# sisl/NeRFSafetyValidation

Measured on AMD Instinct MI355X. Metric: rendered_samples_per_sec, higher is better.
Workload: dtype f16; 1 GPU; Stonehenge 800x800 synthetic, hashgrid L=16 F=2 T=2^19 + ffmlp(64,2)/(64,3), fp16, occupancy-grid ray marching (run_cuda eval path, BASELINE configs[1]); rays_per_frame=640000, bound=2, cascade=2, frames_in_flight=3, fused_reference_rounding=True, parallelism=single GPU, rccl_ranks=1

## Files before the change

### include/ngp_hip.h

```cpp
#ifndef NGP_HIP_H
#define NGP_HIP_H

#include <stddef.h>
#include <stdint.h>

#ifdef __cplusplus
extern "C" {
#endif

#define NGP_OK 0
#define NGP_EINVAL (-1)
#define NGP_ELAUNCH (-2)
#define NGP_EWORKSPACE (-3)
#define NGP_ENODEVICE (-4)

#define NGP_F32 0
#define NGP_F16 1

typedef void* ngp_stream_t;

#if defined(NGP_BUILD)
#define NGP_API __attribute__((visibility("default")))
#else
#define NGP_API
#endif

NGP_API const char* ngp_last_error(void);
NGP_API int ngp_version(void);
NGP_API int ngp_device_count(void);


NGP_API int ngp_near_far_from_aabb(const float* rays_o, const float* rays_d, const float* aabb, uint32_t N, float min_near,
                           float* nears, float* fars, ngp_stream_t stream);
NGP_API int ngp_finish_rays(float* image, float* depth, const float* weights_sum, const float* nears, const float* fars,
                    const float* bg_color3_host, uint32_t N, ngp_stream_t stream);
NGP_API int ngp_sph_from_ray(const float* rays_o, const float* rays_d, float radius, uint32_t N, float* coords,
                     ngp_stream_t stream);
NGP_API int ngp_morton3D(const int32_t* coords, uint32_t N, int32_t* indices, ngp_stream_t stream);
NGP_API int ngp_morton3D_invert(const int32_t* indices, uint32_t N, int32_t* coords, ngp_stream_t stream);
NGP_API int ngp_packbits(const float* grid, uint32_t N, float density_thresh, uint8_t* bitfield, ngp_stream_t stream);

NGP_API size_t ngp_march_rays_train_workspace(uint32_t N);
NGP_API int ngp_march_rays_train(const float* rays_o, const float* rays_d, const uint8_t* grid, float bound, float dt_gamma,
                         uint32_t max_steps, uint32_t N, uint32_t C, uint32_t H, uint32_t M, const float* nears,
                         const float* fars, float* xyzs, float* dirs, float* deltas, int32_t* rays, int32_t* counter,
                         uint32_t perturb, void* workspace, size_t workspace_bytes, ngp_stream_t stream);
NGP_API int ngp_composite_rays_train_forward(const float* sigmas, const float* rgbs, const float* deltas, const int32_t* rays,
                                     uint32_t M, uint32_t N, float* weights_sum, float* depth, float* image,
                                     ngp_stream_t stream);
NGP_API int ngp_composite_rays_train_backward(const float* grad_weights_sum, const float* grad_image, const float* sigmas,
                                      const float* rgbs, const float* deltas, const int32_t* rays,
                                      const float* weights_sum, const float* image, uint32_t M, uint32_t N,
                                      float* grad_sigmas, float* grad_rgbs, ngp_stream_t stream);
NGP_API int ngp_march_rays(uint32_t n_alive, uint32_t n_step, const int32_t* rays_alive, const float* rays_t,
                   const float* rays_o, const float* rays_d, float bound, float dt_gamma, uint32_t max_steps,
                   uint32_t C, uint32_t H, const uint8_t* grid, const float* nears, const float* fars, float* xyzs,
                   float* dirs, float* deltas, uint32_t perturb, uint32_t M_padded, ngp_stream_t stream);
NGP_API size_t ngp_occupancy_lin_bytes(uint32_t C, uint32_t H);
NGP_API int ngp_build_occupancy_lin(const uint8_t* grid, uint32_t C, uint32_t H, void* out, size_t out_bytes, ngp_stream_t stream);
NGP_API int ngp_march_rays_lin(uint32_t n_alive, uint32_t n_step, const int32_t* rays_alive, const float* rays_t,
                   const float* rays_o, const float* rays_d, float bound, float dt_gamma, uint32_t max_steps,
                   uint32_t C, uint32_t H, const uint8_t* grid, const float* nears, const float* fars, float* xyzs,
                   float* dirs, float* deltas, uint32_t perturb, uint32_t M_padded, const void* occupancy_lin,
                   ngp_stream_t stream);
NGP_API int ngp_composite_rays(uint32_t n_alive, uint32_t n_step, int32_t* rays_alive, float* rays_t, const float* sigmas,
                       const float* rgbs, const float* deltas, float* weights_sum, float* depth, float* image,
                       ngp_stream_t stream);


NGP_API int ngp_grid_encode_forward(const float* inputs, const void* embeddings, const int32_t* offsets_host, void* outputs,
                            uint32_t B, uint32_t D, uint32_t C, uint32_t L, float S, uint32_t H,
                            int calc_grad_inputs, void* dy_dx, uint32_t gridtype, int align_corners, int dtype,
                            const void* cell_tables, uint32_t cell_levels, ngp_stream_t stream);
NGP_API int ngp_grid_encode_backward(const void* grad, const float* inputs, const void* embeddings,
                             const int32_t* offsets_host, void* grad_embeddings, uint32_t B, uint32_t D, uint32_t C,
                             uint32_t L, float S, uint32_t H, int calc_grad_inputs, const void* dy_dx,
                             void* grad_inputs, uint32_t gridtype, int align_corners, int dtype, void* workspace,
                             size_t workspace_bytes, ngp_stream_t stream);
NGP_API int ngp_grid_encode_forward_strided(const float* inputs, const void* embeddings, const int32_t* offsets_host, void* outputs,
                                    uint32_t B, uint32_t D, uint32_t C, uint32_t L, float S, uint32_t H,
                                    int calc_grad_inputs, void* dy_dx, uint32_t gridtype, int align_corners, int dtype,
                                    const void* cell_tables, uint32_t cell_levels, uint32_t level_stride, uint32_t point_stride,
                                    ngp_stream_t stream);
NGP_API int ngp_grid_encode_backward_strided(const void* grad, const float* inputs, const void* embeddings,
                                     const int32_t* offsets_host, void* grad_embeddings, uint32_t B, uint32_t D, uint32_t C,
                                     uint32_t L, float S, uint32_t H, int calc_grad_inputs, const void* dy_dx,
                                     void* grad_inputs, uint32_t gridtype, int align_corners, int dtype, void* workspace,
                                     size_t workspace_bytes, uint32_t level_stride, uint32_t point_stride, ngp_stream_t stream);
NGP_API size_t ngp_grid_encode_backward_workspace(uint32_t B, uint32_t D, uint32_t C, uint32_t L, int dtype);


NGP_API int ngp_sh_encode_forward(const float* inputs, float* outputs, uint32_t B, uint32_t D, uint32_t C,
                          int calc_grad_inputs, float* dy_dx, ngp_stream_t stream);
NGP_API int ngp_sh_encode_backward(const float* grad, const float* inputs, uint32_t B, uint32_t D, uint32_t C,
                           const float* dy_dx, float* grad_inputs, ngp_stream_t stream);


NGP_API int ngp_freq_encode_forward(const float* inputs, float* outputs, uint32_t B, uint32_t D, uint32_t deg, ngp_stream_t stream);
NGP_API int ngp_freq_encode_backward(const float* grad, const float* inputs, uint32_t B, uint32_t D, uint32_t deg, float* grad_inputs,
                             ngp_stream_t stream);

NGP_API int ngp_ff_sigma_color_input(const uint16_t* h, const float* dirs, uint32_t B, uint32_t B_pad, float* sigma, uint16_t* color_input,
                             ngp_stream_t stream);
NGP_API int ngp_ff_sigma_color_input_backward(const uint16_t* h, const float* grad_sigma, const uint16_t* grad_color_input, uint32_t B,
                                      uint32_t B_pad, uint16_t* grad_h, ngp_stream_t stream);
NGP_API int ngp_ff_rgb(const uint16_t* outputs16, uint32_t B, uint16_t* rgb, ngp_stream_t stream);
NGP_API int ngp_ff_rgb_backward(const uint16_t* grad_rgb, const uint16_t* rgb, uint32_t B, uint32_t B_pad, uint16_t* grad_outputs16,
                        ngp_stream_t stream);


NGP_API int ngp_ffmlp_forward(const uint16_t* inputs, const uint16_t* weights, uint32_t B, uint32_t input_dim,
                      uint32_t output_dim, uint32_t hidden_dim, uint32_t num_layers, uint32_t activation,
                      uint32_t output_activation, uint16_t* forward_buffer, uint16_t* outputs, ngp_stream_t stream);
NGP_API int ngp_ffmlp_forward_planes(const uint16_t* inputs, const uint16_t* weights, uint32_t B, uint32_t input_dim,
                             uint32_t output_dim, uint32_t hidden_dim, uint32_t num_layers, uint32_t activation,
                             uint32_t output_activation, uint16_t* forward_buffer, uint16_t* outputs, ngp_stream_t stream);
NGP_API int ngp_ffmlp_backward_planes(const uint16_t* grad, const uint16_t* inputs, const uint16_t* weights, const uint16_t* forward_buffer,
                              uint32_t B, uint32_t input_dim, uint32_t output_dim, uint32_t hidden_dim, uint32_t num_layers,
                              uint32_t activation, uint32_t output_activation, int calc_grad_inputs, uint16_t* backward_buffer,
                              uint16_t* grad_inputs, uint16_t* grad_weights, void* workspace, size_t workspace_bytes,
                              ngp_stream_t stream);
NGP_API int ngp_ffmlp_backward_recomputes(uint32_t input_dim, uint32_t hidden_dim, uint32_t num_layers);
NGP_API int ngp_ffmlp_inference(const uint16_t* inputs, const uint16_t* weights, uint32_t B, uint32_t input_dim,
                        uint32_t output_dim, uint32_t hidden_dim, uint32_t num_layers, uint32_t activation,
                        uint32_t output_activation, uint16_t* inference_buffer, uint16_t* outputs,
                        ngp_stream_t stream);
NGP_API int ngp_ffmlp_backward(const uint16_t* grad, const uint16_t* inputs, const uint16_t* weights,
                       const uint16_t* forward_buffer, uint32_t B, uint32_t input_dim, uint32_t output_dim,
                       uint32_t hidden_dim, uint32_t num_layers, uint32_t activation, uint32_t output_activation,
                       int calc_grad_inputs, uint16_t* backward_buffer, uint16_t* grad_inputs,
                       uint16_t* grad_weights, void* workspace, size_t workspace_bytes, ngp_stream_t stream);
NGP_API size_t ngp_ffmlp_backward_workspace(uint32_t B, uint32_t input_dim, uint32_t hidden_dim, uint32_t num_layers);
NGP_API size_t ngp_ffmlp_backward_buffer_bytes(uint32_t B, uint32_t input_dim, uint32_t hidden_dim, uint32_t num_layers);
NGP_API int ngp_ffmlp_allocate_splitk(size_t n);
NGP_API int ngp_ffmlp_free_splitk(void);


NGP_API int ngp_get_rays(const float* poses, uint32_t Bc, float fx, float fy, float cx, float cy, uint32_t H, uint32_t W,
                 const int32_t* pixel_inds, uint32_t n_pix, float* rays_o, float* rays_d, ngp_stream_t stream);
NGP_API int ngp_get_rays_backward(const float* grad_rays_o, const float* grad_rays_d, uint32_t Bc, float fx, float fy, float cx, float cy,
                          uint32_t H, uint32_t W, const int32_t* pixel_inds, uint32_t n_pix, float* grad_poses,
                          ngp_stream_t stream);


typedef struct ngp_model {
    const uint16_t* embeddings;
    const int32_t* offsets_host;
    uint32_t L;
    float S;
    uint32_t H_base;
    uint32_t gridtype;
    int align_corners;
    const uint16_t* sigma_weights;
    uint32_t sigma_hidden_mm;
    const uint16_t* color_weights;
    uint32_t color_hidden_mm;
    float bound;
    float density_scale;
    const uint8_t* density_bitfield;
    uint32_t cascade;
    uint32_t grid_size;
    const void* cell_tables;
    uint32_t cell_levels;
    const void* packed_weights;
    uint32_t precision;
} ngp_model;
#define NGP_PREC_F16 0u
#define NGP_PREC_F32 1u
#define NGP_PREC_F16_REF 2u

NGP_API size_t ngp_packed_weights_bytes(void);
NGP_API int ngp_pack_weights(const ngp_model* model, void* out, ngp_stream_t stream);

NGP_API size_t ngp_cell_tables_bytes(const ngp_model* model, uint32_t n_levels);
NGP_API int ngp_build_cell_tables(const ngp_model* model, uint32_t n_levels, void* out, ngp_stream_t stream);

typedef struct ngp_render_stats {
    uint64_t samples_marched;
    uint64_t samples_slots;
    uint32_t iterations;
    uint32_t rays;
    uint32_t last_n_alive;
    uint32_t last_n_step;
    uint32_t launches;
    uint32_t replayed;
} ngp_render_stats;

typedef struct ngp_render_ctx ngp_render_ctx;

NGP_API int ngp_render_ctx_create(uint32_t max_rays, ngp_render_ctx** out);
NGP_API int ngp_render_ctx_destroy(ngp_render_ctx* ctx);

NGP_API int ngp_render_ctx_set_frame_width(ngp_render_ctx* ctx, uint32_t width);

NGP_API int ngp_render_rays(ngp_render_ctx* ctx, const ngp_model* model, const float* rays_o, const float* rays_d,
                    const float* nears, const float* fars, uint32_t N, float dt_gamma, uint32_t max_steps,
                    uint32_t perturb, float* weights_sum, float* depth, float* image, float* last_sigmas,
                    float* last_rgbs, const float* pad_value_host, ngp_render_stats* stats_host, int sync,
                    ngp_stream_t stream);

NGP_API int ngp_network_forward(const ngp_model* model, const float* xyzs, const float* dirs, uint32_t M, float* sigmas,
                        float* rgbs, ngp_stream_t stream);

NGP_API int ngp_network_density(const ngp_model* model, const float* xyzs, uint32_t M, float* sigmas, float* geo_feat, ngp_stream_t stream);
NGP_API int ngp_network_density_backward(const ngp_model* model, const void* packed_weights_bwd, const float* xyzs, uint32_t M,
                                 const float* grad_sigmas, const float* grad_geo_feat, float* grad_xyzs, ngp_stream_t stream);

NGP_API int ngp_planner_collision(const ngp_model* model, const float* rot_matrix, const float* pos, const float* body, const float* rot,
                                  uint32_t S, uint32_t B, float* out, ngp_stream_t stream);
NGP_API int ngp_planner_collision_backward(const ngp_model* model, const void* packed_weights_bwd, const float* rot_matrix, const float* pos,
                                           const float* body, const float* rot, uint32_t S, uint32_t B, const float* grad_out,
                                           float* grad_pos, float* grad_rot_matrix, ngp_stream_t stream);

NGP_API int ngp_cell_max_density(const ngp_model* model, const float* start_host, float granularity, uint32_t X, uint32_t Y, uint32_t Z,
                                 uint32_t s, const float* rot_host, float* out_max_sigma, ngp_stream_t stream);

#define NGP_EDT_INF 0x7fffffff
NGP_API size_t ngp_edt_sq_workspace(uint32_t X, uint32_t Y, uint32_t Z);
NGP_API int ngp_edt_sq(const uint8_t* occupied, uint32_t X, uint32_t Y, uint32_t Z, int32_t* d2, void* workspace, size_t workspace_bytes,
                       ngp_stream_t stream);

NGP_API size_t ngp_isosurface_workspace(uint32_t X, uint32_t Y, uint32_t Z);
NGP_API int ngp_isosurface_count(const float* u, uint32_t X, uint32_t Y, uint32_t Z, float threshold, void* workspace, size_t workspace_bytes,
                                 uint64_t* totals, ngp_stream_t stream);
NGP_API int ngp_isosurface_emit(const float* u, uint32_t X, uint32_t Y, uint32_t Z, float threshold, const void* workspace,
                                size_t workspace_bytes, uint64_t V, uint64_t F, float* vertices, int32_t* faces, ngp_stream_t stream);

typedef struct ngp_raycast_grid {
    float lo[3], cell[3], inv_cell[3], grow[3];
    float reach;
    uint32_t n[3];
} ngp_raycast_grid;
NGP_API int ngp_raycast_bin_count(const float* tri_data, uint32_t F, const ngp_raycast_grid* grid, int32_t* counts, ngp_stream_t stream);
NGP_API int ngp_raycast_bin_emit(const float* tri_data, uint32_t F, const ngp_raycast_grid* grid, const int64_t* offsets, uint64_t P,
                                 int32_t* pair_cell, int32_t* pair_tri, ngp_stream_t stream);
NGP_API int ngp_raycast(const float* rays_o, const float* rays_d, uint64_t N, const ngp_raycast_grid* grid, const int32_t* cell_start,
                        const int32_t* pair_tri, uint64_t P, const float* tri_data, uint32_t F, float t_min, float t_max,
                        uint32_t frame_width, float* t, int32_t* prim, float* u, float* v, ngp_stream_t stream);
NGP_API int ngp_raycast_shade(const float* rays_d, const int32_t* prim, const float* u, const float* v, uint64_t N, const float* tri_data,
                              const int32_t* faces, uint32_t F, const float* colors, uint32_t V, float ambient,
                              const float* bg_color3_host, float* image, uint8_t* image_u8, ngp_stream_t stream);

typedef struct ngp_voxel_box {
    double start[3];
    double granularity;
    uint32_t shape[3];
    int32_t axis[3], sign[3];
} ngp_voxel_box;
NGP_API int ngp_voxelize_count(const float* vertices, uint32_t V, const int32_t* faces, uint32_t F, const ngp_voxel_box* box, uint8_t* map,
                               int32_t* counts, ngp_stream_t stream);
NGP_API int ngp_voxelize_mark(const float* vertices, uint32_t V, const int32_t* faces, uint32_t F, const ngp_voxel_box* box,
                              const int64_t* ends, uint64_t pair_base, uint64_t n_pairs, uint8_t* map, ngp_stream_t stream);

NGP_API int ngp_overlay_cast(const float* rays_o, const float* rays_d, uint64_t N, const float* prims_host, const float* prims, uint32_t P,
                             float t_min, const float* t_max, uint32_t frame_width, float* t, int32_t* prim, float* normal,
                             ngp_stream_t stream);
NGP_API int ngp_overlay_shade(const float* rays_d, const int32_t* prim, const float* normal, uint64_t N, const float* colors, uint32_t P,
                              float ambient, float* image, uint8_t* image_u8, ngp_stream_t stream);

#define NGP_DISTANCE_STATS_MAX_THRESHOLDS 8
NGP_API int ngp_closest_point(const float* points, uint64_t N, const ngp_raycast_grid* grid, const int32_t* cell_start,
                              const int32_t* pair_tri, uint64_t P, const float* tri_verts, uint32_t F, float max_distance, float* distance,
                              int32_t* prim, float* point, uint32_t* tested, ngp_stream_t stream);
NGP_API size_t ngp_distance_stats_state_bytes(void);
NGP_API size_t ngp_distance_stats_workspace(uint64_t n);
NGP_API int ngp_distance_stats(const float* distance, uint64_t n, uint64_t seen, const float* thresholds_host, uint32_t K, void* state,
                               double* stats, void* workspace, size_t workspace_bytes, ngp_stream_t stream);

NGP_API int ngp_render_uniform(const ngp_model* model, const float* rays_o, const float* rays_d, const float* nears,
                       const float* fars, uint32_t N, uint32_t T, const float* lin, float* weights_sum, float* depth,
                       float* image, float* aggregated_density, uint32_t dump_begin, float* sigmas, float* rgbs,
                       uint32_t frame_width, ngp_stream_t stream);

NGP_API int ngp_render_upsample(const ngp_model* model, const float* rays_o, const float* rays_d, const float* nears,
                        const float* fars, uint32_t N, uint32_t T, uint32_t U, const float* lin, const float* u,
                        float* weights_sum, float* depth, float* image, float* aggregated_density, uint32_t dump_begin,
                        float* sigmas, float* rgbs, uint32_t frame_width, void* workspace, size_t workspace_bytes,
                        ngp_stream_t stream);
NGP_API size_t ngp_render_upsample_workspace(uint32_t N, uint32_t T, uint32_t U);

NGP_API size_t ngp_packed_weights_bwd_bytes(void);
NGP_API int ngp_pack_weights_bwd(const ngp_model* model, void* out, ngp_stream_t stream);
NGP_API size_t ngp_render_uniform_backward_lds(const ngp_model* model, uint32_t T);
NGP_API int ngp_render_uniform_backward(const ngp_model* model, const void* packed_weights_bwd, const float* rays_o, const float* rays_d,
                                const float* nears, const float* fars, uint32_t N, uint32_t T, const float* lin, const float* grad_image,
                                const float* grad_depth, const float* grad_weights_sum, const float* grad_aggregated_density,
                                float* grad_rays_o, float* grad_rays_d, ngp_stream_t stream);


NGP_API int ngp_uniform_samples(const float* rays_o, const float* rays_d, const float* nears, const float* fars, uint32_t N, uint32_t T,
                        uint32_t steps_for_dist, const float* lin, const float* noise, const float* z_in, const float* aabb_host,
                        float* z_vals, float* xyzs, ngp_stream_t stream);
NGP_API int ngp_uniform_samples_backward(const float* grad_xyzs, const float* rays_o, const float* rays_d, const float* z_vals, uint32_t N,
                                 uint32_t T, const float* aabb_host, float* grad_rays_o, float* grad_rays_d, ngp_stream_t stream);
NGP_API int ngp_transmittance_weights(const float* z_vals, const float* sigmas, const float* sample_dist, uint32_t N, uint32_t T,
                              float density_scale, float* weights, ngp_stream_t stream);
NGP_API int ngp_transmittance_weights_backward(const float* grad_weights, const float* z_vals, const float* sigmas, const float* sample_dist,
                                       uint32_t N, uint32_t T, float density_scale, float* grad_sigmas, ngp_stream_t stream);
NGP_API int ngp_sample_pdf(const float* bins, const float* weights, uint32_t N, uint32_t n_bins, const float* u, int u_per_ray,
                   uint32_t n_samples, float* samples, ngp_stream_t stream);
NGP_API int ngp_merge_sorted(const float* z_a, const float* z_b, uint32_t N, uint32_t Ta, uint32_t Tb, float* z, int64_t* index,
                     ngp_stream_t stream);


NGP_API int ngp_mark_untrained_grid(const float* poses, uint32_t n_cams, float fx, float fy, float cx, float cy, float bound, uint32_t cascade,
                            uint32_t H, float* density_grid, void* workspace, size_t workspace_bytes, ngp_stream_t stream);
NGP_API int ngp_density_grid_points(const int32_t* coords, uint32_t n, uint32_t H, float cascade_bound, const float* noise, float* xyzs,
                            int32_t* indices, ngp_stream_t stream);
NGP_API size_t ngp_density_grid_workspace(uint32_t cascade, uint32_t H);
NGP_API int ngp_density_grid_update(float* density_grid, uint32_t cascade, uint32_t H, uint32_t cas, const int32_t* indices, const float* sigmas,
                            uint32_t n, float density_scale, float decay, void* workspace, size_t workspace_bytes, ngp_stream_t stream);
NGP_API int ngp_density_grid_finish(const float* density_grid, uint32_t cascade, uint32_t H, float density_thresh, float* mean_thresh,
                            uint8_t* bitfield, void* workspace, size_t workspace_bytes, ngp_stream_t stream);


NGP_API size_t ngp_uq_stats_workspace(void);
NGP_API int ngp_uq_stats(const void* c, int c_dtype, const float* d, uint64_t n, const float* r, uint64_t m, double* stats,
                 void* workspace, size_t workspace_bytes, ngp_stream_t stream);


NGP_API size_t ngp_sigma_fit_workspace(uint32_t n, uint32_t max_workgroups);
NGP_API int ngp_sigma_fit_eval(const float* features, const float* y, uint32_t n, const float* theta, float prior_mean, double prior_var,
                       int mode, uint32_t max_workgroups, void* workspace, size_t workspace_bytes, double* loss, float* grad,
                       ngp_stream_t stream);
NGP_API int ngp_sigma_fit_step(const float* features, const float* y, uint32_t n, float* theta, float prior_mean, double prior_var, int mode,
                       uint32_t max_workgroups, void* workspace, size_t workspace_bytes, float* grad, float* exp_avg, float* exp_avg_sq,
                       float lr, uint32_t step, float* min_loss, int32_t* improved, float* history, uint32_t history_index,
                       ngp_stream_t stream);


NGP_API int ngp_adam_step(float* param, const float* grad, float* exp_avg, float* exp_avg_sq, uint64_t n, float lr, float beta1,
                  float beta2, float eps, uint32_t step, float grad_scale, ngp_stream_t stream);

NGP_API int ngp_adam_advance_step(float* step_dev, const float* found_inf_dev, ngp_stream_t stream);
NGP_API int ngp_adam_step_dev(float* param, const float* grad, float* exp_avg, float* exp_avg_sq, uint64_t n, float lr, float beta1,
                      float beta2, float eps, const float* step_dev, const float* grad_scale_dev, const float* found_inf_dev,
                      ngp_stream_t stream);


NGP_API int ngp_train_targets(const void* store, int store_dtype, uint32_t C, uint64_t frame_base, uint32_t n_pix, const int64_t* inds,
                      uint32_t N, const float* bg, const float* table, int round_half, float* gt_rgb, ngp_stream_t stream);

NGP_API size_t ngp_photo_loss_workspace(uint32_t N);
NGP_API int ngp_photo_loss_forward(const void* pred, int pred_dtype, const float* gt, uint32_t N, float* per_ray, float* mean, float* error_row,
                           uint32_t map_len, const int64_t* inds_coarse, void* workspace, size_t workspace_bytes, ngp_stream_t stream);
NGP_API int ngp_photo_loss_backward(const void* pred, int pred_dtype, const float* gt, uint32_t N, const float* g, void* grad_pred,
// ... 59 lines not shown
```

### nerfsafetyvalidation_amd/_fused.py

```python
import ctypes as C
import os
import threading

import numpy as np
import torch

from . import _lib


CACHE_LOCK = threading.Lock()


class RunUniform(torch.autograd.Function):

    @staticmethod
    def forward(ctx, fm, rays_o, rays_d, nears, fars, num_steps, dump_begin, frame_width=0, bg=None):
        rays_o, rays_d = rays_o.float().contiguous(), rays_d.float().contiguous()
        ws, depth, image, agg, sigmas, rgbs = fm.render_uniform(rays_o, rays_d, nears, fars, num_steps, dump_begin, frame_width)
        ctx.fm, ctx.num_steps = fm, num_steps
        ctx.bg = None
        if bg is not None:
            ctx.bg = torch.tensor(bg, dtype=torch.float32, device=image.device) if isinstance(bg, (tuple, list)) else float(bg)
            image = image + (1 - ws).unsqueeze(-1) * ctx.bg
        ctx.save_for_backward(rays_o, rays_d, nears, fars)
# ... 126 lines not shown
            raise RuntimeError("fused renderer needs 64-wide MLPs and geo_feat_dim == 15")
        watched = [net.encoder.embeddings] + [l.weight for l in net.sigma_net] + [l.weight for l in net.color_net]
        if f32 and (len(net.sigma_net) - 2 > 1 or len(net.color_net) - 2 > 2):
            raise RuntimeError("fp32 fused model: at most 3 sigma and 4 colour layers (the backward kernels keep that many activations)")
        return cls(net, blob(net.sigma_net, 32), len(net.sigma_net) - 2, blob(net.color_net, 32), len(net.color_net) - 2, watched, f32=f32)

    def valid_for(self, net):
        return (_versions(self._watched) == self._snapshot and self.density_scale == float(net.density_scale)
                and self.bound == float(net.bound) and self.emb16.device == net.encoder.embeddings.device
                and (self.f32 or self.ref_rounding == bool(getattr(net, "fused_reference_rounding", False))))

    def _struct(self, bitfield):
        m = _lib.ModelStruct()
        m.embeddings = _lib.ptr(self.emb16)
        m.offsets_host = C.cast(self.offsets_host, C.c_void_p)
        m.L, m.S, m.H_base, m.gridtype, m.align_corners = 16, self.S, self.H_base, self.gridtype, self.align_corners
        m.sigma_weights, m.sigma_hidden_mm = _lib.ptr(self.sigma_blob), self.sigma_mm
        m.color_weights, m.color_hidden_mm = _lib.ptr(self.color_blob), self.color_mm
        m.bound, m.density_scale = self.bound, self.density_scale
        m.density_bitfield = _lib.ptr(bitfield) if bitfield is not None else None
        m.cascade, m.grid_size = self.cascade, self.grid_size
        m.cell_tables = _lib.ptr(self._cells) if self._cells is not None else None
        m.cell_levels = self._cell_levels
        m.packed_weights = _lib.ptr(self._packed) if self._packed is not None else None
        m.precision = _lib.NGP_PREC_F32 if self.f32 else (_lib.NGP_PREC_F16_REF if self.ref_rounding else _lib.NGP_PREC_F16)
        return m

    def _ensure_packed(self):
        if self._packed is not None:
            return
        with self._ctx_lock:
            if self._packed is not None:
                return
            lib = _lib.lib()
            m = self._struct(None)
            packed = torch.empty(lib.ngp_packed_weights_bytes(), dtype=torch.uint8, device=self.device)
            _lib.check(lib.ngp_pack_weights(C.byref(m), _lib.ptr(packed), _lib.stream()), "pack_weights")
            torch.cuda.current_stream(self.device).synchronize()
            self._packed = packed

    def _ensure_cells(self):
        self._ensure_packed()
        if self._tables is not None:
            self._tables.table_for_current_stream()
        if self._cells_ready:
            return
        if self.cell_table_gb > 0 and not self.f32:
            self._cells, self._cell_levels = self._tables.ensure_cells(self.offsets_host, self.S, self.H_base, self.gridtype, self.align_corners,
                                                                       self.cell_table_gb)
        self._cells_ready = True

    def network_forward(self, xyzs, dirs):
        xyzs, dirs = xyzs.float().contiguous(), dirs.float().contiguous()
        self._ensure_cells()
        M = xyzs.shape[0]
        sigmas = torch.empty(M, dtype=torch.float32, device=xyzs.device)
        rgbs = torch.empty(M, 3, dtype=torch.float32, device=xyzs.device)
        m = self._struct(None)
        lib = _lib.lib()
        _lib.check(lib.ngp_network_forward(C.byref(m), _lib.ptr(xyzs), _lib.ptr(dirs), M, _lib.ptr(sigmas), _lib.ptr(rgbs), _lib.stream()),
                   "network_forward")
        return sigmas, rgbs

    def network_density(self, xyzs, want_geo=False):
        xyzs = xyzs.float().contiguous()
        self._ensure_packed()
        M = xyzs.shape[0]
        sigmas = torch.empty(M, dtype=torch.float32, device=xyzs.device)
        geo = torch.empty(M, 15, dtype=torch.float32, device=xyzs.device) if want_geo else None
        m = self._struct(None)
        _lib.check(_lib.lib().ngp_network_density(C.byref(m), _lib.ptr(xyzs), M, _lib.ptr(sigmas), _lib.ptr(geo), _lib.stream()), "network_density")
        return (sigmas, geo) if want_geo else sigmas

    def cell_max_density(self, start, granularity, shape, samples_per_axis, rot):
        self._ensure_packed()
        X, Y, Z = (int(n) for n in shape)
        out = torch.empty(X, Y, Z, dtype=torch.float32, device=self.device)
        st = (C.c_float * 3)(*[float(v) for v in start])
        r = (C.c_float * 9)(*[float(v) for v in torch.as_tensor(rot, dtype=torch.float32).reshape(9).tolist()])
        _lib.check(_lib.lib().ngp_cell_max_density(C.byref(self._struct(None)), st, float(granularity), X, Y, Z, int(samples_per_axis), r,
                                                   _lib.ptr(out), _lib.stream()), "cell_max_density")
        return out

    def _ensure_packed_bwd(self):
        if self._packed_bwd is None:
            lib = _lib.lib()
            with self._ctx_lock:
                if self._packed_bwd is None:
                    buf = torch.empty(lib.ngp_packed_weights_bwd_bytes(), dtype=torch.uint8, device=self.device)
                    _lib.check(lib.ngp_pack_weights_bwd(C.byref(self._struct(None)), _lib.ptr(buf), _lib.stream()), "pack_weights_bwd")
                    torch.cuda.current_stream(self.device).synchronize()
                    self._packed_bwd = buf
        return self._packed_bwd

    def network_density_backward(self, xyzs, g_sigma=None, g_geo=None):
        self._ensure_packed()
        packed_bwd = self._ensure_packed_bwd()
        xyzs = xyzs.float().contiguous()
        M = xyzs.shape[0]
        f32 = lambda t: None if t is None else t.float().contiguous()
        gx = torch.empty(M, 3, dtype=torch.float32, device=xyzs.device)
        m = self._struct(None)
        _lib.check(_lib.lib().ngp_network_density_backward(C.byref(m), _lib.ptr(packed_bwd), _lib.ptr(xyzs), M, _lib.ptr(f32(g_sigma)),
                                                           _lib.ptr(f32(g_geo)), _lib.ptr(gx), _lib.stream()), "network_density_backward")
        return gx

    def planner_collision(self, rot_matrix, pos, body, rot):
        self._ensure_packed()
        S, B = rot_matrix.shape[0], body.shape[0]
        out = torch.empty(S, dtype=torch.float32, device=rot_matrix.device)
        _lib.check(_lib.lib().ngp_planner_collision(C.byref(self._struct(None)), _lib.ptr(rot_matrix), _lib.ptr(pos), _lib.ptr(body),
                                                    _lib.ptr(rot), S, B, _lib.ptr(out), _lib.stream()), "planner_collision")
        return out

    def planner_collision_backward(self, rot_matrix, pos, body, rot, g):
        self._ensure_packed()
        packed_bwd = self._ensure_packed_bwd()
        S, B = rot_matrix.shape[0], body.shape[0]
        g = g.float().contiguous()
        g_pos = torch.empty(S, 3, dtype=torch.float32, device=rot_matrix.device)
        g_rot = torch.empty(S, 3, 3, dtype=torch.float32, device=rot_matrix.device)
        _lib.check(_lib.lib().ngp_planner_collision_backward(C.byref(self._struct(None)), _lib.ptr(packed_bwd), _lib.ptr(rot_matrix), _lib.ptr(pos),
                                                             _lib.ptr(body), _lib.ptr(rot), S, B, _lib.ptr(g), _lib.ptr(g_pos), _lib.ptr(g_rot),
                                                             _lib.stream()), "planner_collision_backward")
        return g_pos, g_rot

    def _pad_value(self):
        if self._pad is None:
            z = torch.zeros(16, 3, device=self.device)
            s, c = self.network_forward(z, z)
            sig = np.float32(float(s[0])) * np.float32(self.density_scale)
            self._pad = (C.c_float * 4)(float(sig), float(c[0, 0]), float(c[0, 1]), float(c[0, 2]))
        return self._pad

    @property
    def last_stats(self):
        return getattr(self._tls, "stats", None)

    def _context(self, N):
        lib = _lib.lib()
        key = threading.get_ident()
        with self._ctx_lock:
            ent = self._ctxs.get(key)
        if ent is None or ent[1] < N:
            if ent is not None:
                lib.ngp_render_ctx_destroy(ent[0])
            h = C.c_void_p()
            _lib.check(lib.ngp_render_ctx_create(N, C.byref(h)), "render_ctx_create")
            ent = [h, N]
            with self._ctx_lock:
                self._ctxs[key] = ent
        return ent[0]

    def render(self, net_bitfield_owner, rays_o, rays_d, nears, fars, dt_gamma, max_steps, perturb, want_last=True, want_stats=True,
               frame_width=0):
        bitfield = net_bitfield_owner.density_bitfield
        self._ensure_cells()
        N = rays_o.shape[0]
        dev = rays_o.device
        weights_sum = torch.empty(N, dtype=torch.float32, device=dev)
        depth = torch.empty(N, dtype=torch.float32, device=dev)
        image = torch.empty(N, 3, dtype=torch.float32, device=dev)
        last_s = torch.empty(N + 128, dtype=torch.float32, device=dev) if want_last else None
        last_c = torch.empty(N + 128, 3, dtype=torch.float32, device=dev) if want_last else None
        stats = _lib.RenderStats()
        m = self._struct(bitfield)
        lib = _lib.lib()
        ctx = self._context(N)
        need_stats = want_stats or want_last
        _lib.check(lib.ngp_render_ctx_set_frame_width(ctx, int(frame_width or 0)), "render_ctx_set_frame_width")
        if self.debug is not None:
            flags, stamps, hashes = self.debug
            _lib.check(lib.ngp_render_ctx_set_debug(ctx, 1, int(flags), _lib.ptr(stamps), _lib.ptr(hashes)), "render_ctx_set_debug")
        _lib.check(lib.ngp_render_rays(ctx, C.byref(m), _lib.ptr(rays_o), _lib.ptr(rays_d), _lib.ptr(nears.contiguous()),
                                       _lib.ptr(fars.contiguous()), N, float(dt_gamma), int(max_steps), int(perturb), _lib.ptr(weights_sum),
                                       _lib.ptr(depth), _lib.ptr(image), _lib.ptr(last_s), _lib.ptr(last_c),
                                       self._pad_value() if want_last else None, C.byref(stats) if need_stats else None, 0, _lib.stream()),
                   "render_rays")
        sigmas = rgbs = None
        if need_stats:
            self._tls.stats = {"samples_marched": int(stats.samples_marched), "samples_slots": int(stats.samples_slots),
                               "iterations": int(stats.iterations), "rays": int(stats.rays), "launches": int(stats.launches),
                               "replayed": int(stats.replayed)}
        if want_last and stats.iterations > 0:
            M = stats.last_n_alive * stats.last_n_step
            M += 128 - (M % 128)
            sigmas, rgbs = last_s[:M], last_c[:M]
        return weights_sum, depth, image, sigmas, rgbs

    def render_uniform(self, rays_o, rays_d, nears, fars, num_steps, dump_begin, frame_width=0):
        self._ensure_cells()
        N, T, dev = rays_o.shape[0], int(num_steps), rays_o.device
        lin = self._linspace(0.0, 1.0, T)
        out = [torch.empty(N, dtype=torch.float32, device=dev), torch.empty(N, dtype=torch.float32, device=dev),
               torch.empty(N, 3, dtype=torch.float32, device=dev), torch.empty(N, dtype=torch.float32, device=dev)]
        n_dump = N - dump_begin
        sigmas = torch.empty(n_dump * T, 1, dtype=torch.float32, device=dev)
        rgbs = torch.empty(n_dump, T, 3, dtype=torch.float32, device=dev)
        m = self._struct(None)
        lib = _lib.lib()
        _lib.check(lib.ngp_render_uniform(C.byref(m), _lib.ptr(rays_o), _lib.ptr(rays_d), _lib.ptr(nears.contiguous()), _lib.ptr(fars.contiguous()),
                                          N, T, _lib.ptr(lin), _lib.ptr(out[0]), _lib.ptr(out[1]), _lib.ptr(out[2]), _lib.ptr(out[3]),
                                          dump_begin, _lib.ptr(sigmas), _lib.ptr(rgbs), int(frame_width or 0), _lib.stream()), "render_uniform")
        return out[0], out[1], out[2], out[3], sigmas, rgbs

    def _linspace(self, lo, hi, n):
        key = (float(lo), float(hi), int(n))
        t = self._lin_cache.get(key)
        if t is None:
            t = torch.linspace(lo, hi, n, device=self.device)
            torch.cuda.current_stream(self.device).synchronize()
            self._lin_cache[key] = t
        return t

    def upsample_fits(self, num_steps, upsample_steps):
        if self.f32:
            return False
        weights = 2 * ((2048 + self.sigma_mm * 4096 + 1024) + (2048 + self.color_mm * 4096 + 1024))
        return num_steps >= 3 and upsample_steps >= 1 and weights + 2048 + 4 * (5 * num_steps + 4 * upsample_steps) <= 159 * 1024

    def render_upsample(self, rays_o, rays_d, nears, fars, num_steps, upsample_steps, dump_begin, frame_width=0):
        self._ensure_cells()
        N, T, U, dev = rays_o.shape[0], int(num_steps), int(upsample_steps), rays_o.device
        lin = self._linspace(0.0, 1.0, T)
        u = self._linspace(0.0 + 0.5 / U, 1.0 - 0.5 / U, U)
        out = [torch.empty(N, dtype=torch.float32, device=dev), torch.empty(N, dtype=torch.float32, device=dev),
               torch.empty(N, 3, dtype=torch.float32, device=dev), torch.empty(N, dtype=torch.float32, device=dev)]
        n_dump = N - dump_begin
        sigmas = torch.empty(n_dump * (T + U), 1, dtype=torch.float32, device=dev)
        rgbs = torch.empty(n_dump, T + U, 3, dtype=torch.float32, device=dev)
        m = self._struct(None)
        lib = _lib.lib()
        wbytes = lib.ngp_render_upsample_workspace(N, T, U)
        work = torch.empty((wbytes + 3) // 4, dtype=torch.float32, device=dev) if wbytes else None
        _lib.check(lib.ngp_render_upsample(C.byref(m), _lib.ptr(rays_o), _lib.ptr(rays_d), _lib.ptr(nears.contiguous()), _lib.ptr(fars.contiguous()),
                                           N, T, U, _lib.ptr(lin), _lib.ptr(u), _lib.ptr(out[0]), _lib.ptr(out[1]), _lib.ptr(out[2]),
                                           _lib.ptr(out[3]), dump_begin, _lib.ptr(sigmas), _lib.ptr(rgbs), int(frame_width or 0), _lib.ptr(work), wbytes,
                                           _lib.stream()), "render_upsample")
        return out[0], out[1], out[2], out[3], sigmas, rgbs

    def render_uniform_backward(self, rays_o, rays_d, nears, fars, num_steps, g_image, g_depth=None, g_ws=None, g_agg=None):
        self._ensure_cells()
        lib = _lib.lib()
        self._ensure_packed_bwd()
        N, T, dev = rays_o.shape[0], int(num_steps), rays_o.device
        lin = self._linspace(0.0, 1.0, T)
        f32 = lambda t: None if t is None else t.float().contiguous()
        go = torch.empty(N, 3, dtype=torch.float32, device=dev)
        gd = torch.empty(N, 3, dtype=torch.float32, device=dev)
        m = self._struct(None)
        _lib.check(lib.ngp_render_uniform_backward(C.byref(m), _lib.ptr(self._packed_bwd), _lib.ptr(rays_o), _lib.ptr(rays_d), _lib.ptr(nears.contiguous()),
                                                   _lib.ptr(fars.contiguous()), N, T, _lib.ptr(lin), _lib.ptr(f32(g_image)), _lib.ptr(f32(g_depth)),
                                                   _lib.ptr(f32(g_ws)), _lib.ptr(f32(g_agg)), _lib.ptr(go), _lib.ptr(gd), _lib.stream()),
                   "render_uniform_backward")
        return go, gd

    def uniform_backward_fits(self, num_steps):
        need = _lib.lib().ngp_render_uniform_backward_lds(C.byref(self._struct(None)), int(num_steps))
        return num_steps <= 1024 and need <= 160 * 1024

    def __del__(self):
        try:
            for ent in self._ctxs.values():
                _lib.lib().ngp_render_ctx_destroy(ent[0])
        except Exception:
            pass
```

### nerfsafetyvalidation_amd/_lib.py

```python
import ctypes as C
import os

import torch

_HERE = os.path.dirname(os.path.abspath(__file__))
SO_PATH = os.environ.get("NGP_HIP_LIB", os.path.join(_HERE, "libngp_hip.so"))

NGP_F32, NGP_F16 = 0, 1
NGP_PREC_F16, NGP_PREC_F32, NGP_PREC_F16_REF = 0, 1, 2
NGP_DBG_NO_BLOCK_JUMP, NGP_DBG_NO_COARSE, NGP_DBG_NO_SLOW_SORT, NGP_DBG_NO_LIN = 1 << 0, 1 << 1, 1 << 2, 1 << 3
NGP_DBG_ONE_ITER_PER_LAUNCH, NGP_DBG_NO_TILES = 1 << 8, 1 << 13
NGP_DBG_NO_PRE_VERDICT, NGP_DBG_WIDE_ITEMS, NGP_DBG_REPLAY_ONE_ITER = 1 << 14, 1 << 15, 1 << 16
NGP_DBG_LANE_MARCH, NGP_DBG_PROBE_PER_SAMPLE = 1 << 17, 1 << 18
NGP_EDT_INF = 0x7FFFFFFF

_vp, _u32, _f32, _int, _sz = C.c_void_p, C.c_uint32, C.c_float, C.c_int, C.c_size_t


class ModelStruct(C.Structure):
    _fields_ = [
        ("embeddings", _vp), ("offsets_host", _vp), ("L", _u32), ("S", _f32), ("H_base", _u32), ("gridtype", _u32),
        ("align_corners", _int), ("sigma_weights", _vp), ("sigma_hidden_mm", _u32), ("color_weights", _vp),
        ("color_hidden_mm", _u32), ("bound", _f32), ("density_scale", _f32), ("density_bitfield", _vp),
        ("cascade", _u32), ("grid_size", _u32), ("cell_tables", _vp), ("cell_levels", _u32), ("packed_weights", _vp),
        ("precision", _u32),
    ]


class RenderStats(C.Structure):
    _fields_ = [("samples_marched", C.c_uint64), ("samples_slots", C.c_uint64), ("iterations", _u32), ("rays", _u32),
                ("last_n_alive", _u32), ("last_n_step", _u32), ("launches", _u32), ("replayed", _u32)]


class RaycastGrid(C.Structure):
    _fields_ = [("lo", _f32 * 3), ("cell", _f32 * 3), ("inv_cell", _f32 * 3), ("grow", _f32 * 3), ("reach", _f32), ("n", _u32 * 3)]


class VoxelBox(C.Structure):
    _fields_ = [("start", C.c_double * 3), ("granularity", C.c_double), ("shape", _u32 * 3), ("axis", C.c_int32 * 3), ("sign", C.c_int32 * 3)]


SIGNATURES = {
    "ngp_last_error": [],
    "ngp_version": [],
    "ngp_device_count": [],
    "ngp_finish_rays": [_vp, _vp, _vp, _vp, _vp, C.POINTER(C.c_float), _u32, _vp],
    "ngp_near_far_from_aabb": [_vp, _vp, _vp, _u32, _f32, _vp, _vp, _vp],
    "ngp_sph_from_ray": [_vp, _vp, _f32, _u32, _vp, _vp],
    "ngp_morton3D": [_vp, _u32, _vp, _vp],
    "ngp_morton3D_invert": [_vp, _u32, _vp, _vp],
    "ngp_packbits": [_vp, _u32, _f32, _vp, _vp],
    "ngp_march_rays_train_workspace": [_u32],
    "ngp_march_rays_train": [_vp, _vp, _vp, _f32, _f32, _u32, _u32, _u32, _u32, _u32, _vp, _vp, _vp, _vp, _vp, _vp, _vp,
                             _u32, _vp, _sz, _vp],
    "ngp_composite_rays_train_forward": [_vp, _vp, _vp, _vp, _u32, _u32, _vp, _vp, _vp, _vp],
    "ngp_composite_rays_train_backward": [_vp, _vp, _vp, _vp, _vp, _vp, _vp, _vp, _u32, _u32, _vp, _vp, _vp],
    "ngp_march_rays": [_u32, _u32, _vp, _vp, _vp, _vp, _f32, _f32, _u32, _u32, _u32, _vp, _vp, _vp, _vp, _vp, _vp, _u32,
                       _u32, _vp],
    "ngp_occupancy_lin_bytes": [_u32, _u32],
    "ngp_build_occupancy_lin": [_vp, _u32, _u32, _vp, _sz, _vp],
    "ngp_march_rays_lin": [_u32, _u32, _vp, _vp, _vp, _vp, _f32, _f32, _u32, _u32, _u32, _vp, _vp, _vp, _vp, _vp, _vp, _u32,
                           _u32, _vp, _vp],
    "ngp_composite_rays": [_u32, _u32, _vp, _vp, _vp, _vp, _vp, _vp, _vp, _vp, _vp],
    "ngp_grid_encode_forward": [_vp, _vp, _vp, _vp, _u32, _u32, _u32, _u32, _f32, _u32, _int, _vp, _u32, _int, _int, _vp, _u32, _vp],
    "ngp_grid_encode_backward": [_vp, _vp, _vp, _vp, _vp, _u32, _u32, _u32, _u32, _f32, _u32, _int, _vp, _vp, _u32, _int,
                                 _int, _vp, _sz, _vp],
    "ngp_grid_encode_forward_strided": [_vp, _vp, _vp, _vp, _u32, _u32, _u32, _u32, _f32, _u32, _int, _vp, _u32, _int, _int, _vp, _u32,
                                        _u32, _u32, _vp],
    "ngp_grid_encode_backward_strided": [_vp, _vp, _vp, _vp, _vp, _u32, _u32, _u32, _u32, _f32, _u32, _int, _vp, _vp, _u32, _int,
                                         _int, _vp, _sz, _u32, _u32, _vp],
    "ngp_grid_encode_backward_workspace": [_u32, _u32, _u32, _u32, _int],
    "ngp_sh_encode_forward": [_vp, _vp, _u32, _u32, _u32, _int, _vp, _vp],
    "ngp_sh_encode_backward": [_vp, _vp, _u32, _u32, _u32, _vp, _vp, _vp],
    "ngp_freq_encode_forward": [_vp, _vp, _u32, _u32, _u32, _vp],
    "ngp_freq_encode_backward": [_vp, _vp, _u32, _u32, _u32, _vp, _vp],
    "ngp_ff_sigma_color_input": [_vp, _vp, _u32, _u32, _vp, _vp, _vp],
    "ngp_ff_sigma_color_input_backward": [_vp, _vp, _vp, _u32, _u32, _vp, _vp],
    "ngp_ff_rgb": [_vp, _u32, _vp, _vp],
    "ngp_ff_rgb_backward": [_vp, _vp, _u32, _u32, _vp, _vp],
    "ngp_ffmlp_forward": [_vp, _vp, _u32, _u32, _u32, _u32, _u32, _u32, _u32, _vp, _vp, _vp],
    "ngp_ffmlp_inference": [_vp, _vp, _u32, _u32, _u32, _u32, _u32, _u32, _u32, _vp, _vp, _vp],
    "ngp_ffmlp_backward": [_vp, _vp, _vp, _vp, _u32, _u32, _u32, _u32, _u32, _u32, _u32, _int, _vp, _vp, _vp, _vp, _sz, _vp],
    "ngp_ffmlp_forward_planes": [_vp, _vp, _u32, _u32, _u32, _u32, _u32, _u32, _u32, _vp, _vp, _vp],
    "ngp_ffmlp_backward_planes": [_vp, _vp, _vp, _vp, _u32, _u32, _u32, _u32, _u32, _u32, _u32, _int, _vp, _vp, _vp, _vp, _sz, _vp],
    "ngp_ffmlp_backward_recomputes": [_u32, _u32, _u32],
    "ngp_ffmlp_backward_workspace": [_u32, _u32, _u32, _u32],
    "ngp_ffmlp_backward_buffer_bytes": [_u32, _u32, _u32, _u32],
    "ngp_ffmlp_allocate_splitk": [_sz],
    "ngp_ffmlp_free_splitk": [],
    "ngp_get_rays": [_vp, _u32, _f32, _f32, _f32, _f32, _u32, _u32, _vp, _u32, _vp, _vp, _vp],
    "ngp_get_rays_backward": [_vp, _vp, _u32, _f32, _f32, _f32, _f32, _u32, _u32, _vp, _u32, _vp, _vp],
    "ngp_uq_stats_workspace": [],
    "ngp_uq_stats": [_vp, _int, _vp, C.c_uint64, _vp, C.c_uint64, _vp, _vp, _sz, _vp],
    "ngp_sigma_fit_workspace": [_u32, _u32],
    "ngp_sigma_fit_eval": [_vp, _vp, _u32, _vp, _f32, C.c_double, _int, _u32, _vp, _sz, _vp, _vp, _vp],
    "ngp_sigma_fit_step": [_vp, _vp, _u32, _vp, _f32, C.c_double, _int, _u32, _vp, _sz, _vp, _vp, _vp, _f32, _u32, _vp, _vp, _vp, _u32, _vp],
    "ngp_adam_step": [_vp, _vp, _vp, _vp, C.c_uint64, _f32, _f32, _f32, _f32, _u32, _f32, _vp],
    "ngp_adam_advance_step": [_vp, _vp, _vp],
    "ngp_adam_step_dev": [_vp, _vp, _vp, _vp, C.c_uint64, _f32, _f32, _f32, _f32, _vp, _vp, _vp, _vp],
    "ngp_train_targets": [_vp, _int, _u32, C.c_uint64, _u32, _vp, _u32, _vp, _vp, _int, _vp, _vp],
    "ngp_photo_loss_workspace": [_u32],
    "ngp_photo_loss_forward": [_vp, _int, _vp, _u32, _vp, _vp, _vp, _u32, _vp, _vp, _sz, _vp],
    "ngp_photo_loss_backward": [_vp, _int, _vp, _u32, _vp, _vp, _vp],
    "ngp_distortion_workspace": [_u32],
    "ngp_distortion_train_forward": [_vp, _vp, _vp, _vp, _u32, _u32, _vp, _vp, _vp, _vp, _sz, _vp],
    "ngp_distortion_train_backward": [_vp, _vp, _vp, _vp, _vp, _vp, _u32, _u32, _vp, _vp],
    "ngp_distortion_forward": [_vp, _vp, _vp, _f32, _vp, _u32, _u32, _vp, _vp, _vp, _vp, _sz, _vp],
    "ngp_distortion_backward": [_vp, _vp, _vp, _vp, _f32, _vp, _vp, _u32, _u32, _vp, _vp],
    "ngp_image_quality_workspace": [_u32, _u32, _u32],
    "ngp_image_quality": [_vp, _vp, _vp, _u32, _u32, _u32, C.c_int64, C.c_int64, C.c_int64, C.c_int64, _f32, _vp, _vp, _vp, _sz, _vp],
    "ngp_cell_tables_bytes": [C.POINTER(ModelStruct), _u32],
    "ngp_build_cell_tables": [C.POINTER(ModelStruct), _u32, _vp, _vp],
    "ngp_packed_weights_bytes": [],
    "ngp_pack_weights": [C.POINTER(ModelStruct), _vp, _vp],
    "ngp_render_ctx_create": [_u32, C.POINTER(_vp)],
    "ngp_render_ctx_destroy": [_vp],
    "ngp_render_ctx_set_frame_width": [_vp, _u32],
    "ngp_render_rays": [_vp, C.POINTER(ModelStruct), _vp, _vp, _vp, _vp, _u32, _f32, _u32, _u32, _vp, _vp, _vp, _vp, _vp,
                        C.POINTER(C.c_float), C.POINTER(RenderStats), _int, _vp],
    "ngp_network_forward": [C.POINTER(ModelStruct), _vp, _vp, _u32, _vp, _vp, _vp],
    "ngp_network_density": [C.POINTER(ModelStruct), _vp, _u32, _vp, _vp, _vp],
    "ngp_network_density_backward": [C.POINTER(ModelStruct), _vp, _vp, _u32, _vp, _vp, _vp, _vp],
    "ngp_planner_collision": [C.POINTER(ModelStruct), _vp, _vp, _vp, _vp, _u32, _u32, _vp, _vp],
    "ngp_planner_collision_backward": [C.POINTER(ModelStruct), _vp, _vp, _vp, _vp, _vp, _u32, _u32, _vp, _vp, _vp, _vp],
    "ngp_cell_max_density": [C.POINTER(ModelStruct), _vp, C.c_float, _u32, _u32, _u32, _u32, _vp, _vp, _vp],
    "ngp_edt_sq_workspace": [_u32, _u32, _u32],
    "ngp_edt_sq": [_vp, _u32, _u32, _u32, _vp, _vp, _sz, _vp],
    "ngp_isosurface_workspace": [_u32, _u32, _u32],
    "ngp_isosurface_count": [_vp, _u32, _u32, _u32, _f32, _vp, _sz, _vp, _vp],
    "ngp_isosurface_emit": [_vp, _u32, _u32, _u32, _f32, _vp, _sz, C.c_uint64, C.c_uint64, _vp, _vp, _vp],
    "ngp_raycast_bin_count": [_vp, _u32, C.POINTER(RaycastGrid), _vp, _vp],
    "ngp_raycast_bin_emit": [_vp, _u32, C.POINTER(RaycastGrid), _vp, C.c_uint64, _vp, _vp, _vp],
    "ngp_raycast": [_vp, _vp, C.c_uint64, C.POINTER(RaycastGrid), _vp, _vp, C.c_uint64, _vp, _u32, _f32, _f32, _u32, _vp, _vp, _vp, _vp, _vp],
    "ngp_raycast_shade": [_vp, _vp, _vp, _vp, C.c_uint64, _vp, _vp, _u32, _vp, _u32, _f32, C.POINTER(C.c_float), _vp, _vp, _vp],
    "ngp_voxelize_count": [_vp, _u32, _vp, _u32, C.POINTER(VoxelBox), _vp, _vp, _vp],
    "ngp_voxelize_mark": [_vp, _u32, _vp, _u32, C.POINTER(VoxelBox), _vp, C.c_uint64, C.c_uint64, _vp, _vp],
    "ngp_overlay_cast": [_vp, _vp, C.c_uint64, _vp, _vp, _u32, _f32, _vp, _u32, _vp, _vp, _vp, _vp],
    "ngp_overlay_shade": [_vp, _vp, _vp, C.c_uint64, _vp, _u32, _f32, _vp, _vp, _vp],
    "ngp_closest_point": [_vp, C.c_uint64, C.POINTER(RaycastGrid), _vp, _vp, C.c_uint64, _vp, _u32, _f32, _vp, _vp, _vp, _vp, _vp],
    "ngp_distance_stats_state_bytes": [],
    "ngp_distance_stats_workspace": [C.c_uint64],
    "ngp_distance_stats": [_vp, C.c_uint64, C.c_uint64, C.POINTER(C.c_float), _u32, _vp, _vp, _vp, _sz, _vp],
    "ngp_sift_workspace": [_u32, _u32],
    "ngp_sift_layer_offset": [_u32, _u32, _int, _int],
    "ngp_sift_octaves": [_u32, _u32],
    "ngp_sift_interest_mask": [_vp, _u32, _u32, _u32, _u32, _vp, _vp, _vp, _vp, _sz, _vp],
    "ngp_render_uniform_backward_lds": [C.POINTER(ModelStruct), _u32],
    "ngp_packed_weights_bwd_bytes": [],
    "ngp_pack_weights_bwd": [C.POINTER(ModelStruct), _vp, _vp],
    "ngp_render_uniform_backward": [C.POINTER(ModelStruct), _vp, _vp, _vp, _vp, _vp, _u32, _u32, _vp, _vp, _vp, _vp, _vp, _vp, _vp, _vp],
    "ngp_uniform_samples": [_vp, _vp, _vp, _vp, _u32, _u32, _u32, _vp, _vp, _vp, C.POINTER(C.c_float), _vp, _vp, _vp],
    "ngp_uniform_samples_backward": [_vp, _vp, _vp, _vp, _u32, _u32, C.POINTER(C.c_float), _vp, _vp, _vp],
    "ngp_transmittance_weights": [_vp, _vp, _vp, _u32, _u32, _f32, _vp, _vp],
    "ngp_transmittance_weights_backward": [_vp, _vp, _vp, _vp, _u32, _u32, _f32, _vp, _vp],
    "ngp_sample_pdf": [_vp, _vp, _u32, _u32, _vp, _int, _u32, _vp, _vp],
    "ngp_merge_sorted": [_vp, _vp, _u32, _u32, _u32, _vp, _vp, _vp],
    "ngp_mark_untrained_grid": [_vp, _u32, _f32, _f32, _f32, _f32, _f32, _u32, _u32, _vp, _vp, _sz, _vp],
    "ngp_density_grid_points": [_vp, _u32, _u32, _f32, _vp, _vp, _vp, _vp],
    "ngp_density_grid_workspace": [_u32, _u32],
    "ngp_density_grid_update": [_vp, _u32, _u32, _u32, _vp, _vp, _u32, _f32, _f32, _vp, _sz, _vp],
    "ngp_density_grid_finish": [_vp, _u32, _u32, _f32, _vp, _vp, _vp, _sz, _vp],
    "ngp_render_uniform": [C.POINTER(ModelStruct), _vp, _vp, _vp, _vp, _u32, _u32, _vp, _vp, _vp, _vp, _vp, _u32, _vp, _vp, _u32, _vp],
    "ngp_render_upsample": [C.POINTER(ModelStruct), _vp, _vp, _vp, _vp, _u32, _u32, _u32, _vp, _vp, _vp, _vp, _vp, _vp, _u32, _vp, _vp, _u32, _vp, _sz, _vp],
    "ngp_render_upsample_workspace": [_u32, _u32, _u32],
    "ngp_debug_set_stamps": [_vp],
    "ngp_debug_set_sample_hash": [_vp],
    "ngp_debug_disable_march_queue": [_int],
    "ngp_render_ctx_set_debug": [_vp, _int, _int, _vp, _vp],
    "ngp_debug_set_grad_dump": [_vp],
    "ngp_debug_fused_features": [C.POINTER(ModelStruct), _vp, _u32, _int, _vp, _vp],
    "ngp_prof_enable": [_int],
    "ngp_prof_reset": [],
    "ngp_prof_read": [C.c_char_p, C.POINTER(C.c_double), C.POINTER(C.c_uint64), C.POINTER(C.c_double)],
}
_RESTYPES = {"ngp_render_uniform_backward_lds": _sz, "ngp_cell_tables_bytes": _sz, "ngp_packed_weights_bytes": _sz, "ngp_packed_weights_bwd_bytes": _sz, "ngp_grid_encode_backward_workspace": _sz,
             "ngp_ffmlp_backward_workspace": _sz, "ngp_ffmlp_backward_buffer_bytes": _sz, "ngp_render_upsample_workspace": _sz, "ngp_density_grid_workspace": _sz, "ngp_last_error": C.c_char_p, "ngp_march_rays_train_workspace": _sz, "ngp_uq_stats_workspace": _sz, "ngp_sigma_fit_workspace": _sz, "ngp_occupancy_lin_bytes": _sz, "ngp_edt_sq_workspace": _sz, "ngp_isosurface_workspace": _sz, "ngp_sift_workspace": _sz, "ngp_sift_layer_offset": _sz, "ngp_photo_loss_workspace": _sz, "ngp_image_quality_workspace": _sz, "ngp_distortion_workspace": _sz, "ngp_distance_stats_state_bytes": _sz, "ngp_distance_stats_workspace": _sz}

_lib = None


def lib():
    global _lib
    if _lib is None:
        if not os.path.exists(SO_PATH):
            raise RuntimeError(
                f"{SO_PATH} not found: build it with `python -c 'import __graft_entry__ as g; g.build()'` "
                "(hipcc --offload-arch=gfx950).  There is no fallback implementation.")
        handle = C.CDLL(SO_PATH)
        for name, argtypes in SIGNATURES.items():
            fn = getattr(handle, name)
            fn.argtypes = argtypes
            fn.restype = _RESTYPES.get(name, C.c_int)
        _lib = handle
    return _lib


def check(rc, what=""):
    if rc != 0:
        msg = lib().ngp_last_error()
        raise RuntimeError(f"libngp_hip {what} failed (code {rc}): {msg.decode() if msg else ''}")


def ptr(t):
    if t is None:
        return None
    if not t.is_cuda:
        raise RuntimeError("libngp_hip operators need tensors on a HIP device; got a CPU tensor (no CPU fallback)")
    if not t.is_contiguous():
        raise RuntimeError("libngp_hip operators need contiguous tensors")
    return t.data_ptr()


_raw_stream = getattr(torch._C, "_cuda_getCurrentRawStream", None)


def stream():
    if _raw_stream is not None:
        return _raw_stream(torch.cuda.current_device())
    return torch.cuda.current_stream().cuda_stream


def dtype_code(t):
    if t.dtype == torch.float32:
        return NGP_F32
    if t.dtype == torch.float16:
        return NGP_F16
    raise RuntimeError(f"unsupported dtype {t.dtype}: the grid encoder supports float32 and float16")


def host_i32(t):
    cached = getattr(t, "_ngp_host_i32", None)
    if cached is not None and cached[0] == t._version and cached[1] == t.data_ptr():
        return cached[2]
    vals = t.detach().to("cpu", torch.int32).tolist()
    arr = (C.c_int32 * len(vals))(*vals)
    try:
        t._ngp_host_i32 = (t._version, t.data_ptr(), arr)
    except AttributeError:
        pass
    return arr
```

### nerfsafetyvalidation_amd/csrc/capi.hip

```cpp
#include <math.h>
#include <stdarg.h>
#include <stdlib.h>
#include <string.h>

#include <mutex>
#include <vector>

#include "ngp_common.hpp"
#include "wave_ops.hpp"

namespace ngp {

static thread_local char g_err[512] = "";

void set_error(const char* fmt, ...) {
    va_list ap;
    va_start(ap, fmt);
    vsnprintf(g_err, sizeof(g_err), fmt, ap);
    va_end(ap);
}

int check_launch(const char* what) {
    const hipError_t e = hipGetLastError();
    if (e != hipSuccess) {
        set_error("%s: %s", what, hipGetErrorString(e));
        return NGP_ELAUNCH;
    }
    return NGP_OK;
}

bool env_set(const char* name) { return getenv(name) != nullptr; }
uint32_t env_u32(const char* name, uint32_t dflt) {
    const char* e = getenv(name);
    return e ? (uint32_t)atoll(e) : dflt;
}

static std::mutex g_attr_mu;
static std::vector<std::pair<int, const void*>> g_attr_done;

void ensure_dynamic_lds(const void* func, int bytes) {
    int dev = 0;
    (void)hipGetDevice(&dev);
    std::lock_guard<std::mutex> lk(g_attr_mu);
    for (const auto& e : g_attr_done)
        if (e.first == dev && e.second == func) return;
    (void)hipFuncSetAttribute(func, hipFuncAttributeMaxDynamicSharedMemorySize, bytes);
    g_attr_done.emplace_back(dev, func);
}

struct ProfEntry {
    std::string name;
    std::vector<std::pair<hipEvent_t, hipEvent_t>> events;
    double total_ms = 0;
    uint64_t launches = 0;
    double units = 0;
};
static bool g_prof_on = false;
static std::mutex g_prof_mu;
static std::vector<ProfEntry> g_prof;

static int prof_slot(const char* name) {
    for (size_t i = 0; i < g_prof.size(); i++)
        if (g_prof[i].name == name) return (int)i;
    g_prof.emplace_back();
    g_prof.back().name = name;
    return (int)g_prof.size() - 1;
}

ProfScope::ProfScope(const char* name, hipStream_t s, double units) : slot(-1), stream(s) {
    if (!g_prof_on) return;
    std::lock_guard<std::mutex> lk(g_prof_mu);
    slot = prof_slot(name);
    hipEvent_t a, b;
    (void)hipEventCreate(&a);
    (void)hipEventCreate(&b);
    (void)hipEventRecord(a, s);
    g_prof[slot].events.emplace_back(a, b);
    g_prof[slot].units += units;
}
ProfScope::~ProfScope() {
    if (slot < 0) return;
    std::lock_guard<std::mutex> lk(g_prof_mu);
    (void)hipEventRecord(g_prof[slot].events.back().second, stream);
}

bool prof_enabled() { return g_prof_on; }
void prof_add_units(const char* name, double units) {
    if (!g_prof_on) return;
    std::lock_guard<std::mutex> lk(g_prof_mu);
    g_prof[prof_slot(name)].units += units;
}

static void prof_collect(ProfEntry& e) {
    for (auto& p : e.events) {
        (void)hipEventSynchronize(p.second);
        float ms = 0;
        if (hipEventElapsedTime(&ms, p.first, p.second) == hipSuccess) {
            e.total_ms += ms;
            e.launches++;
        }
        (void)hipEventDestroy(p.first);
        (void)hipEventDestroy(p.second);
    }
    e.events.clear();
}

constexpr uint32_t kUqBlocks = 512, kUqThreads = 256;

template <typename CT>
__global__ void __launch_bounds__(kUqThreads) k_uq_partial(const CT* __restrict__ c, const float* __restrict__ d, uint64_t n,
                                                           const float* __restrict__ r, uint64_t m, double* __restrict__ partial) {
    __shared__ double red[5][kUqThreads / 64];
    double acc[5] = {0, 0, 0, 0, 0};
    const uint64_t stride = (uint64_t)gridDim.x * kUqThreads, t0 = (uint64_t)blockIdx.x * kUqThreads + threadIdx.x;
    for (uint64_t i = t0; i < n; i += stride) {
        const double dv = (double)d[i];
        double sc = 0, sc2 = 0;
#pragma unroll
        for (int k = 0; k < 3; k++) {
            const double cv = (double)(float)c[i * 3 + k];
            sc += cv;
            sc2 += cv * cv;
        }
        acc[0] += sc2 * dv * dv;
        acc[1] += sc * dv;
        acc[3] += dv;
        acc[4] += dv * dv;
    }
    for (uint64_t i = t0; i < m; i += stride) acc[2] += (double)r[i];
#pragma unroll
    for (int k = 0; k < 5; k++) {
        const double v = wave_sum_lane0(acc[k]);
        if ((threadIdx.x & 63) == 0) red[k][threadIdx.x >> 6] = v;
    }
    __syncthreads();
    if (threadIdx.x < 5) {
        double v = 0;
        for (uint32_t w = 0; w < kUqThreads / 64; w++) v += red[threadIdx.x][w];
        partial[(size_t)blockIdx.x * 5 + threadIdx.x] = v;
    }
}

__global__ void k_uq_final(const double* __restrict__ partial, uint32_t blocks, uint64_t n, uint64_t m, double* __restrict__ stats) {
    const uint32_t k = threadIdx.x;
    if (k >= 5) return;
    double v = 0;
    for (uint32_t b = 0; b < blocks; b++) v += partial[(size_t)b * 5 + k];
    const int slot[5] = {0, 1, 2, 4, 5};
    stats[slot[k]] = v;
    if (k == 0) {
        stats[3] = (double)m;
        stats[6] = (double)n;
        stats[7] = 0;
    }
}

__global__ void __launch_bounds__(256) k_adam_step(float* __restrict__ p, const float* __restrict__ g, float* __restrict__ m,
                                                   float* __restrict__ v, uint64_t n, float beta1, float beta2, float eps, float step_size,
                                                   float rsqrt_bc2_inv, float grad_scale_inv) {
    const uint64_t i0 = ((uint64_t)blockIdx.x * 256 + threadIdx.x) * 4;
    if (i0 >= n) return;
    const bool vec = i0 + 4 <= n && (((uintptr_t)p | (uintptr_t)g | (uintptr_t)m | (uintptr_t)v) & 15) == 0;
    float pv[4], gv[4], mv[4], vv[4];
    const uint32_t cnt = (uint32_t)(n - i0 < 4 ? n - i0 : 4);
    if (vec) {
        *reinterpret_cast<float4*>(pv) = *reinterpret_cast<const float4*>(p + i0);
        *reinterpret_cast<float4*>(gv) = *reinterpret_cast<const float4*>(g + i0);
        *reinterpret_cast<float4*>(mv) = *reinterpret_cast<const float4*>(m + i0);
        *reinterpret_cast<float4*>(vv) = *reinterpret_cast<const float4*>(v + i0);
    } else {
        for (uint32_t k = 0; k < cnt; k++) { pv[k] = p[i0 + k]; gv[k] = g[i0 + k]; mv[k] = m[i0 + k]; vv[k] = v[i0 + k]; }
    }
#pragma unroll
    for (uint32_t k = 0; k < 4; k++) {
        if (k < cnt) {
            const float gr = gv[k] * grad_scale_inv;
            mv[k] = mv[k] + (1.0f - beta1) * (gr - mv[k]);
            vv[k] = beta2 * vv[k] + (1.0f - beta2) * gr * gr;
            const float denom = sqrtf(vv[k]) / rsqrt_bc2_inv + eps;
            pv[k] = pv[k] - step_size * (mv[k] / denom);
        }
    }
    if (vec) {
        *reinterpret_cast<float4*>(p + i0) = *reinterpret_cast<float4*>(pv);
        *reinterpret_cast<float4*>(m + i0) = *reinterpret_cast<float4*>(mv);
        *reinterpret_cast<float4*>(v + i0) = *reinterpret_cast<float4*>(vv);
    } else {
        for (uint32_t k = 0; k < cnt; k++) { p[i0 + k] = pv[k]; m[i0 + k] = mv[k]; v[i0 + k] = vv[k]; }
    }
}

__global__ void k_adam_advance(float* __restrict__ step, const float* __restrict__ found_inf) {
    if (threadIdx.x == 0 && blockIdx.x == 0 && !(found_inf && *found_inf != 0.0f)) *step += 1.0f;
}
__global__ void __launch_bounds__(256) k_adam_step_dev(float* __restrict__ p, const float* __restrict__ g, float* __restrict__ m,
                                                       float* __restrict__ v, uint64_t n, float beta1, float beta2, float eps, float lr,
                                                       const float* __restrict__ step, const float* __restrict__ grad_scale,
                                                       const float* __restrict__ found_inf) {
    if (found_inf && *found_inf != 0.0f) return;
    __shared__ float s_step_size, s_sqrt_bc2, s_inv;
    if (threadIdx.x == 0) {
        const double st = (double)*step;
        const double bc1 = 1.0 - pow((double)beta1, st), bc2 = 1.0 - pow((double)beta2, st);
        s_step_size = (float)((double)lr / bc1);
        s_sqrt_bc2 = (float)sqrt(bc2);
        s_inv = grad_scale ? 1.0f / *grad_scale : 1.0f;
    }
    __syncthreads();
    const float step_size = s_step_size, rsqrt_bc2_inv = s_sqrt_bc2, grad_scale_inv = s_inv;
    const uint64_t i0 = ((uint64_t)blockIdx.x * 256 + threadIdx.x) * 4;
    if (i0 >= n) return;
    const bool vec = i0 + 4 <= n && (((uintptr_t)p | (uintptr_t)g | (uintptr_t)m | (uintptr_t)v) & 15) == 0;
    float pv[4], gv[4], mv[4], vv[4];
    const uint32_t cnt = (uint32_t)(n - i0 < 4 ? n - i0 : 4);
    if (vec) {
        *reinterpret_cast<float4*>(pv) = *reinterpret_cast<const float4*>(p + i0);
        *reinterpret_cast<float4*>(gv) = *reinterpret_cast<const float4*>(g + i0);
        *reinterpret_cast<float4*>(mv) = *reinterpret_cast<const float4*>(m + i0);
        *reinterpret_cast<float4*>(vv) = *reinterpret_cast<const float4*>(v + i0);
    } else {
        for (uint32_t k = 0; k < cnt; k++) { pv[k] = p[i0 + k]; gv[k] = g[i0 + k]; mv[k] = m[i0 + k]; vv[k] = v[i0 + k]; }
    }
#pragma unroll
    for (uint32_t k = 0; k < 4; k++) {
        if (k < cnt) {
            const float gr = gv[k] * grad_scale_inv;
            mv[k] = mv[k] + (1.0f - beta1) * (gr - mv[k]);
            vv[k] = beta2 * vv[k] + (1.0f - beta2) * gr * gr;
            const float denom = sqrtf(vv[k]) / rsqrt_bc2_inv + eps;
            pv[k] = pv[k] - step_size * (mv[k] / denom);
        }
    }
    if (vec) {
        *reinterpret_cast<float4*>(p + i0) = *reinterpret_cast<float4*>(pv);
        *reinterpret_cast<float4*>(m + i0) = *reinterpret_cast<float4*>(mv);
        *reinterpret_cast<float4*>(v + i0) = *reinterpret_cast<float4*>(vv);
    } else {
        for (uint32_t k = 0; k < cnt; k++) { p[i0 + k] = pv[k]; m[i0 + k] = mv[k]; v[i0 + k] = vv[k]; }
    }
}

}

using namespace ngp;

extern "C" {

const char* ngp_last_error(void) { return g_err; }
int ngp_version(void) { return 100; }

int ngp_device_count(void) {
    int n = 0;
    if (hipGetDeviceCount(&n) != hipSuccess) return 0;
    return n;
}

size_t ngp_uq_stats_workspace(void) { return (size_t)kUqBlocks * 5 * sizeof(double); }

int ngp_uq_stats(const void* c, int c_dtype, const float* d, uint64_t n, const float* r, uint64_t m, double* stats, void* workspace,
                 size_t workspace_bytes, ngp_stream_t stream) {
    NGP_REQUIRE(stats && workspace, "uq_stats: null pointer");
    NGP_REQUIRE((c && d) || n == 0, "uq_stats: null sample buffers");
    NGP_REQUIRE(r || m == 0, "uq_stats: null rendered-colour buffer");
    NGP_REQUIRE(workspace_bytes >= ngp_uq_stats_workspace(), "uq_stats: workspace too small (%zu < %zu bytes)", workspace_bytes,
                ngp_uq_stats_workspace());
    NGP_REQUIRE(c_dtype == 0 || c_dtype == 1, "uq_stats: colour dtype must be 0 (f32) or 1 (f16)");
    hipStream_t s = (hipStream_t)stream;
    const uint64_t work = n > m ? n : m;
    uint32_t blocks = (uint32_t)((work + kUqThreads - 1) / kUqThreads);
    blocks = blocks < 1 ? 1 : blocks > kUqBlocks ? kUqBlocks : blocks;
    ProfScope prof("uq_stats", s, (double)work);
    if (c_dtype == 0)
        k_uq_partial<float><<<blocks, kUqThreads, 0, s>>>((const float*)c, d, n, r, m, (double*)workspace);
    else
        k_uq_partial<_Float16><<<blocks, kUqThreads, 0, s>>>((const _Float16*)c, d, n, r, m, (double*)workspace);
    int rc = check_launch("uq_stats");
    if (rc) return rc;
    k_uq_final<<<1, 64, 0, s>>>((const double*)workspace, blocks, n, m, stats);
    return check_launch("uq_stats (final)");
}

int ngp_adam_step(float* param, const float* grad, float* exp_avg, float* exp_avg_sq, uint64_t n, float lr, float beta1, float beta2, float eps,
                  uint32_t step, float grad_scale, ngp_stream_t stream) {
    if (n == 0) return NGP_OK;
    NGP_REQUIRE(param && grad && exp_avg && exp_avg_sq, "adam_step: null pointer");
    NGP_REQUIRE(step >= 1, "adam_step: step counts from 1");
    NGP_REQUIRE(grad_scale != 0.0f, "adam_step: grad_scale must be non-zero");
    const double bc1 = 1.0 - pow((double)beta1, (double)step), bc2 = 1.0 - pow((double)beta2, (double)step);
    const float step_size = (float)((double)lr / bc1);
    const float sqrt_bc2 = (float)sqrt(bc2);
    const uint64_t quads = (n + 3) / 4;
    ProfScope prof("adam_step", (hipStream_t)stream, (double)n);
    k_adam_step<<<(uint32_t)((quads + 255) / 256), 256, 0, (hipStream_t)stream>>>(param, grad, exp_avg, exp_avg_sq, n, beta1, beta2, eps, step_size,
                                                                                   sqrt_bc2, 1.0f / grad_scale);
    return check_launch("adam_step");
}

int ngp_adam_advance_step(float* step_dev, const float* found_inf_dev, ngp_stream_t stream) {
    NGP_REQUIRE(step_dev, "adam_advance_step: null pointer");
    k_adam_advance<<<1, 64, 0, (hipStream_t)stream>>>(step_dev, found_inf_dev);
    return check_launch("adam_advance_step");
}

int ngp_adam_step_dev(float* param, const float* grad, float* exp_avg, float* exp_avg_sq, uint64_t n, float lr, float beta1, float beta2,
                      float eps, const float* step_dev, const float* grad_scale_dev, const float* found_inf_dev, ngp_stream_t stream) {
    if (n == 0) return NGP_OK;
    NGP_REQUIRE(param && grad && exp_avg && exp_avg_sq && step_dev, "adam_step_dev: null pointer");
    const uint64_t quads = (n + 3) / 4;
    ProfScope prof("adam_step", (hipStream_t)stream, (double)n);
    k_adam_step_dev<<<(uint32_t)((quads + 255) / 256), 256, 0, (hipStream_t)stream>>>(param, grad, exp_avg, exp_avg_sq, n, beta1, beta2, eps, lr,
                                                                                       step_dev, grad_scale_dev, found_inf_dev);
    return check_launch("adam_step_dev");
}

int ngp_prof_enable(int on) {
    g_prof_on = on != 0;
    return NGP_OK;
}

int ngp_prof_reset(void) {
    std::lock_guard<std::mutex> lk(g_prof_mu);
    for (auto& e : g_prof) {
        prof_collect(e);
        e.total_ms = 0;
        e.launches = 0;
        e.units = 0;
    }
    return NGP_OK;
}

int ngp_prof_read(const char* name, double* total_ms, uint64_t* launches, double* units) {
    std::lock_guard<std::mutex> lk(g_prof_mu);
    for (auto& e : g_prof) {
        if (e.name == name) {
            prof_collect(e);
            if (total_ms) *total_ms = e.total_ms;
            if (launches) *launches = e.launches;
            if (units) *units = e.units;
            return NGP_OK;
        }
    }
    set_error("prof_read: no kernel named '%s' was recorded", name);
    return NGP_EINVAL;
}

}
```

### nerfsafetyvalidation_amd/csrc/density_grid.hip

```cpp
#include "ngp_common.hpp"
#include "wave_ops.hpp"

namespace ngp {

constexpr int kDgBlock = 256;
constexpr uint32_t kMaxCams = 2048;

__device__ __forceinline__ float cell_unit(uint32_t c, float Hm1) { return (2.0f * (float)c) / Hm1 - 1.0f; }

__global__ void __launch_bounds__(kDgBlock) k_mark_untrained(const float* __restrict__ poses, uint32_t n_cams, float kx, float ky, float bound,
                                                              uint32_t cascade, uint32_t H, float* __restrict__ grid,
                                                              uint32_t* __restrict__ seen_any, uint32_t first_batch, uint32_t last_batch) {
    extern __shared__ float cam[];
    for (uint32_t i = threadIdx.x; i < n_cams * 12; i += kDgBlock) {
        const uint32_t c = i / 12, e = i % 12;
        cam[i] = e < 9 ? poses[(size_t)c * 16 + (e / 3) * 4 + (e % 3)] : poses[(size_t)c * 16 + (e - 9) * 4 + 3];
    }
    __syncthreads();
    const uint32_t H3 = H * H * H;
    const uint32_t g = blockIdx.x * kDgBlock + threadIdx.x;
    if (g >= cascade * H3) return;
    const uint32_t cas = g / H3, cell = g % H3;
    const uint32_t x = cell / (H * H), y = (cell / H) % H, z = cell % H;
    const uint32_t m = morton3D_cell(x, y, z);
// ... 24 lines not shown
    uint32_t c[3];
    if (coords) { c[0] = (uint32_t)coords[(size_t)i * 3]; c[1] = (uint32_t)coords[(size_t)i * 3 + 1]; c[2] = (uint32_t)coords[(size_t)i * 3 + 2]; }
    else { c[0] = i / (H * H); c[1] = (i / H) % H; c[2] = i % H; }
    indices[i] = (int32_t)morton3D(c[0], c[1], c[2]);
    const float Hm1 = (float)(H - 1);
#pragma unroll
    for (int d = 0; d < 3; d++) {
        float v = cell_unit(c[d], Hm1) * span;
        if (noise) v = v + (noise[(size_t)i * 3 + d] * 2.0f - 1.0f) * hgs;
        xyzs[(size_t)i * 3 + d] = v;
    }
}

__global__ void __launch_bounds__(kDgBlock) k_grid_scatter(const int32_t* __restrict__ indices, const float* __restrict__ sigmas, uint32_t n,
                                                            float density_scale, unsigned long long* __restrict__ tmp, uint32_t H3) {
    const uint32_t i = blockIdx.x * kDgBlock + threadIdx.x;
    if (i >= n) return;
    const uint32_t cell = (uint32_t)indices[i];
    if (cell >= H3) return;
    const float v = sigmas[i] * density_scale;
    atomicMax(tmp + cell, ((unsigned long long)(i + 1) << 32) | (unsigned long long)__float_as_uint(v));
}

__global__ void __launch_bounds__(kDgBlock) k_grid_ema(float* __restrict__ grid, const unsigned long long* __restrict__ tmp, uint32_t H3, float decay) {
    const uint32_t i = blockIdx.x * kDgBlock + threadIdx.x;
    if (i >= H3) return;
    const unsigned long long t = tmp[i];
    if (t == 0ull) return;
    const float g = grid[i], v = __uint_as_float((uint32_t)t);
    if (g >= 0.0f && v >= 0.0f) grid[i] = fmaxf(g * decay, v);
}

__global__ void __launch_bounds__(kDgBlock) k_grid_possum(const float* __restrict__ grid, uint32_t n, double* __restrict__ partial) {
    __shared__ double wsum[kDgBlock / 64];
    const uint32_t i = blockIdx.x * kDgBlock + threadIdx.x;
    double pos = 0.0;
    if (i < n) { const float g = grid[i]; pos = g > 0.0f ? (double)g : 0.0; }
    pos = wave_sum_lane0(pos);
    if ((threadIdx.x & 63) == 0) wsum[threadIdx.x >> 6] = pos;
    __syncthreads();
    if (threadIdx.x == 0) partial[blockIdx.x] = wsum[0] + wsum[1] + wsum[2] + wsum[3];
}

__global__ void __launch_bounds__(1024) k_grid_mean_thresh(const double* __restrict__ partial, uint32_t n_partial, double n_cells, float density_thresh,
                                                            float* __restrict__ out) {
    __shared__ double s[1024];
    double a = 0.0;
    for (uint32_t i = threadIdx.x; i < n_partial; i += 1024) a += partial[i];
    s[threadIdx.x] = a;
    __syncthreads();
    for (uint32_t st = 512; st > 0; st >>= 1) {
        if (threadIdx.x < st) s[threadIdx.x] += s[threadIdx.x + st];
        __syncthreads();
    }
    if (threadIdx.x == 0) {
        const float mean = (float)(s[0] / n_cells);
        out[0] = mean;
        out[1] = fminf(mean, density_thresh);
    }
}

__global__ void __launch_bounds__(kDgBlock) k_packbits_dev(const float* __restrict__ grid, uint32_t n_bytes, const float* __restrict__ thresh_p,
                                                            uint8_t* __restrict__ bitfield) {
    const uint32_t w = blockIdx.x * kDgBlock + threadIdx.x;
    const uint32_t n0 = w * 4;
    if (n0 >= n_bytes) return;
    const float thresh = *thresh_p;
    for (uint32_t n = n0; n < n_bytes && n < n0 + 4; n++) {
        const float4 lo = reinterpret_cast<const float4*>(grid)[(size_t)n * 2], hi = reinterpret_cast<const float4*>(grid)[(size_t)n * 2 + 1];
        const uint32_t b = (lo.x > thresh ? 1u : 0u) | (lo.y > thresh ? 2u : 0u) | (lo.z > thresh ? 4u : 0u) | (lo.w > thresh ? 8u : 0u) |
                           (hi.x > thresh ? 16u : 0u) | (hi.y > thresh ? 32u : 0u) | (hi.z > thresh ? 64u : 0u) | (hi.w > thresh ? 128u : 0u);
        bitfield[n] = (uint8_t)b;
    }
}

static bool grid_dims_ok(uint32_t cascade, uint32_t H) {
    return cascade >= 1 && cascade <= 8 && H >= 2 && H <= 1024 && (H * H * H) % 8 == 0;
}

}

using namespace ngp;

extern "C" {

int ngp_mark_untrained_grid(const float* poses, uint32_t n_cams, float fx, float fy, float cx, float cy, float bound, uint32_t cascade, uint32_t H,
                            float* density_grid, void* workspace, size_t workspace_bytes, ngp_stream_t stream) {
    NGP_REQUIRE(density_grid && (poses || n_cams == 0), "mark_untrained_grid: null pointer");
    NGP_REQUIRE(grid_dims_ok(cascade, H), "mark_untrained_grid: unsupported cascade / grid size (%u, %u)", cascade, H);
    hipStream_t s = (hipStream_t)stream;
    const uint32_t H3 = H * H * H, cells = cascade * H3;
    const float kx = (float)((double)cx / (double)fx), ky = (float)((double)cy / (double)fy);
    const uint32_t n_batches = n_cams ? div_up(n_cams, kMaxCams) : 1;
    uint32_t* seen = nullptr;
    if (n_batches > 1) {
        NGP_REQUIRE(workspace && workspace_bytes >= (size_t)cells * 4, "mark_untrained_grid: %u cameras need a workspace of %zu bytes", n_cams,
                    (size_t)cells * 4);
        seen = reinterpret_cast<uint32_t*>(workspace);
    }
    ensure_dynamic_lds((const void*)k_mark_untrained, (int)(kMaxCams * 12 * sizeof(float)));
    for (uint32_t b = 0; b < n_batches; b++) {
        const uint32_t c0 = b * kMaxCams, nc = n_cams - c0 < kMaxCams ? n_cams - c0 : kMaxCams;
        k_mark_untrained<<<div_up(cells, kDgBlock), kDgBlock, (size_t)(nc ? nc : 1) * 12 * sizeof(float), s>>>(
            poses + (size_t)c0 * 16, n_cams ? nc : 0, kx, ky, bound, cascade, H, density_grid, seen, b == 0, b + 1 == n_batches);
    }
    return check_launch("mark_untrained_grid");
}

int ngp_density_grid_points(const int32_t* coords, uint32_t n, uint32_t H, float cascade_bound, const float* noise, float* xyzs, int32_t* indices,
                            ngp_stream_t stream) {
    if (n == 0) return NGP_OK;
    NGP_REQUIRE(xyzs && indices, "density_grid_points: null pointer");
    NGP_REQUIRE(H >= 2 && H <= 1024, "density_grid_points: unsupported grid size %u", H);
    NGP_REQUIRE(coords || n <= H * H * H, "density_grid_points: a full sweep has at most H^3 samples");
    const double hgs = (double)cascade_bound / (double)H;
    k_grid_points<<<div_up(n, kDgBlock), kDgBlock, 0, (hipStream_t)stream>>>(coords, n, H, (float)((double)cascade_bound - hgs), (float)hgs, noise, xyzs,
                                                                             indices);
    return check_launch("density_grid_points");
}

size_t ngp_density_grid_workspace(uint32_t cascade, uint32_t H) {
    const size_t H3 = (size_t)H * H * H;
    return H3 * 8 + (size_t)div_up((uint32_t)(cascade * H3), kDgBlock) * 8 + 64;
}

int ngp_density_grid_update(float* density_grid, uint32_t cascade, uint32_t H, uint32_t cas, const int32_t* indices, const float* sigmas, uint32_t n,
                            float density_scale, float decay, void* workspace, size_t workspace_bytes, ngp_stream_t stream) {
    NGP_REQUIRE(density_grid && workspace && (n == 0 || (indices && sigmas)), "density_grid_update: null pointer");
    NGP_REQUIRE(grid_dims_ok(cascade, H) && cas < cascade, "density_grid_update: unsupported cascade / grid size");
    NGP_REQUIRE(workspace_bytes >= ngp_density_grid_workspace(cascade, H) && ((uintptr_t)workspace & 7) == 0,
                "density_grid_update: workspace too small or misaligned (%zu < %zu bytes)", workspace_bytes, ngp_density_grid_workspace(cascade, H));
    hipStream_t s = (hipStream_t)stream;
    const uint32_t H3 = H * H * H;
    unsigned long long* tmp = reinterpret_cast<unsigned long long*>(workspace);
    if (hipMemsetAsync(tmp, 0, (size_t)H3 * 8, s) != hipSuccess) return check_launch("density_grid_update (memset)");
    if (n) k_grid_scatter<<<div_up(n, kDgBlock), kDgBlock, 0, s>>>(indices, sigmas, n, density_scale, tmp, H3);
    k_grid_ema<<<div_up(H3, kDgBlock), kDgBlock, 0, s>>>(density_grid + (size_t)cas * H3, tmp, H3, decay);
    return check_launch("density_grid_update");
}

int ngp_density_grid_finish(const float* density_grid, uint32_t cascade, uint32_t H, float density_thresh, float* mean_thresh, uint8_t* bitfield,
                            void* workspace, size_t workspace_bytes, ngp_stream_t stream) {
    NGP_REQUIRE(density_grid && mean_thresh && bitfield && workspace, "density_grid_finish: null pointer");
    NGP_REQUIRE(grid_dims_ok(cascade, H), "density_grid_finish: unsupported cascade / grid size");
    NGP_REQUIRE(workspace_bytes >= ngp_density_grid_workspace(cascade, H) && ((uintptr_t)workspace & 7) == 0, "density_grid_finish: workspace too small or misaligned");
    NGP_REQUIRE(((uintptr_t)density_grid & 15) == 0, "density_grid_finish: the density grid must be 16-byte aligned");
    hipStream_t s = (hipStream_t)stream;
    const uint32_t H3 = H * H * H, cells = cascade * H3;
    double* partial = reinterpret_cast<double*>(reinterpret_cast<unsigned long long*>(workspace) + H3);
    const uint32_t per = div_up(H3, kDgBlock);
    for (uint32_t c = 0; c < cascade; c++) k_grid_possum<<<per, kDgBlock, 0, s>>>(density_grid + (size_t)c * H3, H3, partial + (size_t)c * per);
    k_grid_mean_thresh<<<1, 1024, 0, s>>>(partial, cascade * per, (double)cells, density_thresh, mean_thresh);
    k_packbits_dev<<<div_up(div_up(cells / 8, 4), kDgBlock), kDgBlock, 0, s>>>(density_grid, cells / 8, mean_thresh + 1, bitfield);
    return check_launch("density_grid_finish");
}

}
```

### nerfsafetyvalidation_amd/csrc/ngp_common.hpp

```cpp
#pragma once
#include <hip/hip_runtime.h>
#include <stdint.h>
#include <stdio.h>
#include <string>

#include "../../include/ngp_hip.h"

namespace ngp {

void set_error(const char* fmt, ...);
int check_launch(const char* what);

#define NGP_REQUIRE(cond, ...)                 \
    do {                                       \
        if (!(cond)) {                         \
            ngp::set_error(__VA_ARGS__);       \
            return NGP_EINVAL;                 \
        }                                      \
    } while (0)

bool env_set(const char* name);
uint32_t env_u32(const char* name, uint32_t dflt);

struct ProfScope {
    ProfScope(const char* name, hipStream_t s, double units);
    ~ProfScope();
    int slot;
    hipStream_t stream;
};
bool prof_enabled();
void prof_add_units(const char* name, double units);

static inline uint32_t div_up(uint32_t a, uint32_t b) { return (a + b - 1) / b; }

constexpr uint32_t kMeanOneBlockRays = 16384;
constexpr uint32_t kMeanOneBlockThreads = 1024;
constexpr uint32_t kMeanGroupThreads = 256;
static inline size_t mean_workspace(uint32_t N) { return N <= kMeanOneBlockRays ? 0 : (size_t)div_up(N, 64) * sizeof(float); }
int mean_of_rays(const float* values, uint32_t N, float* mean, void* workspace, size_t workspace_bytes, hipStream_t s, const char* what);
int mean_of_groups(const float* groups, uint32_t N, float* mean, hipStream_t s, const char* what);

void ensure_dynamic_lds(const void* func, int bytes);

constexpr int kMaxLevels = 32;
struct GridLevels {
    float scale[kMaxLevels];
    uint32_t resolution[kMaxLevels];
    uint32_t offset[kMaxLevels + 1];
    uint32_t mul1[kMaxLevels], mul2[kMaxLevels];
    uint8_t hashed[kMaxLevels], mode[kMaxLevels];
};
void fill_levels(GridLevels& lv, const int32_t* offsets_host, uint32_t L, float S, uint32_t H, uint32_t D, uint32_t gridtype,
                 bool align_corners);

__device__ __forceinline__ _Float16 mul_round_f16(float w, _Float16 g) {
    float p = w * (float)g;
    asm volatile("" : "+v"(p));
    return (_Float16)p;
}
__device__ __forceinline__ float clampf(float x, float lo, float hi) { return fminf(hi, fmaxf(lo, x)); }
__device__ __forceinline__ float signf(float x) { return copysignf(1.0f, x); }

__device__ __forceinline__ uint32_t expand_bits(uint32_t v) {
    v = (v * 0x00010001u) & 0xFF0000FFu;
    v = (v * 0x00000101u) & 0x0F00F00Fu;
    v = (v * 0x00000011u) & 0xC30C30C3u;
    v = (v * 0x00000005u) & 0x49249249u;
    return v;
}
__device__ __forceinline__ uint32_t morton3D(uint32_t x, uint32_t y, uint32_t z) {
    return expand_bits(x) | (expand_bits(y) << 1) | (expand_bits(z) << 2);
}
__device__ __forceinline__ uint32_t expand_bits10(uint32_t v) {
    v = (v | (v << 16)) & 0xFF0000FFu;
    v = (v | (v << 8)) & 0x0F00F00Fu;
    v = (v | (v << 4)) & 0xC30C30C3u;
    v = (v | (v << 2)) & 0x49249249u;
    return v;
}
__device__ __forceinline__ uint32_t morton3D_cell(uint32_t x, uint32_t y, uint32_t z) {
    return expand_bits10(x) | (expand_bits10(y) << 1) | (expand_bits10(z) << 2);
}

}
```

### nerfsafetyvalidation_amd/csrc/raymarching.hip

```cpp
#include "occupancy.hpp"

namespace ngp {

constexpr int kBlock = 256;
typedef float f4u __attribute__((ext_vector_type(4), aligned(4)));

__global__ void __launch_bounds__(kBlock) k_near_far_from_aabb(const float* __restrict__ rays_o, const float* __restrict__ rays_d,
                                                               const float* __restrict__ aabb, uint32_t N, float min_near,
                                                               float* __restrict__ nears, float* __restrict__ fars) {
    const uint32_t n = blockIdx.x * kBlock + threadIdx.x;
    if (n >= N) return;
    const float ox = rays_o[n * 3], oy = rays_o[n * 3 + 1], oz = rays_o[n * 3 + 2];
    const float rdx = 1 / rays_d[n * 3], rdy = 1 / rays_d[n * 3 + 1], rdz = 1 / rays_d[n * 3 + 2];
    const float a0 = aabb[0], a1 = aabb[1], a2 = aabb[2], a3 = aabb[3], a4 = aabb[4], a5 = aabb[5];
    float near = (a0 - ox) * rdx, far = (a3 - ox) * rdx;
    if (near > far) { float c = near; near = far; far = c; }
    float near_y = (a1 - oy) * rdy, far_y = (a4 - oy) * rdy;
    if (near_y > far_y) { float c = near_y; near_y = far_y; far_y = c; }
    const float FMAX = 3.402823466e+38f;
    if (near > far_y || near_y > far) { nears[n] = fars[n] = FMAX; return; }
    if (near_y > near) near = near_y;
    if (far_y < far) far = far_y;
    float near_z = (a2 - oz) * rdz, far_z = (a5 - oz) * rdz;
    if (near_z > far_z) { float c = near_z; near_z = far_z; far_z = c; }
// ... 502 lines not shown
                                                           float* __restrict__ weights_sum, float* __restrict__ depth,
                                                           float* __restrict__ image) {
    const uint32_t n = blockIdx.x * kBlock + threadIdx.x;
    if (n >= n_alive) return;
    const int32_t index = rays_alive[n];
    const float* sg = sigmas + (size_t)n * n_step;
    const float* rg = rgbs + (size_t)n * n_step * 3;
    const float* dl = deltas + (size_t)n * n_step * 2;
    float t = rays_t[index];
    float weight_sum = weights_sum[index], d = depth[index];
    float r = image[index * 3], g = image[index * 3 + 1], b = image[index * 3 + 2];
    uint32_t step = 0;
    while (step < n_step) {
        if (dl[0] == 0) break;
        const float alpha = 1.0f - expf(-sg[0] * dl[0]);
        const float T = 1 - weight_sum;
        const float weight = alpha * T;
        weight_sum += weight;
        t += dl[1];
        d = fmaf(weight, t, d);
        r = fmaf(weight, rg[0], r); g = fmaf(weight, rg[1], g); b = fmaf(weight, rg[2], b);
        if ((double)T < 1e-4) break;
        sg++; rg += 3; dl += 2; step++;
    }
    if (step < n_step) rays_alive[n] = -1; else rays_t[index] = t;
    weights_sum[index] = weight_sum; depth[index] = d;
    image[index * 3] = r; image[index * 3 + 1] = g; image[index * 3 + 2] = b;
}

__global__ void __launch_bounds__(kBlock) k_get_rays(const float* __restrict__ poses, uint32_t Bc, float fx, float fy, float cx, float cy,
                                                     uint32_t H, uint32_t W, const int32_t* __restrict__ pixel_inds, uint32_t n_pix,
                                                     float* __restrict__ rays_o, float* __restrict__ rays_d) {
    const uint32_t p = blockIdx.x * kBlock + threadIdx.x;
    const uint32_t cam = blockIdx.y;
    if (p >= n_pix || cam >= Bc) return;
    const uint32_t pix = pixel_inds ? (uint32_t)pixel_inds[p] : p;
    const float* P = poses + (size_t)cam * 16;
    const float i = (float)(pix % W) + 0.5f, j = (float)(pix / W) + 0.5f;
    const float xs = (i - cx) / fx, ys = (j - cy) / fy, zs = 1.0f;
    const float nrm = sqrtf(xs * xs + ys * ys + zs * zs);
    const float ux = xs / nrm, uy = ys / nrm, uz = zs / nrm;
    const size_t o = ((size_t)cam * n_pix + p) * 3;
    rays_d[o + 0] = ux * P[0] + uy * P[1] + uz * P[2];
    rays_d[o + 1] = ux * P[4] + uy * P[5] + uz * P[6];
    rays_d[o + 2] = ux * P[8] + uy * P[9] + uz * P[10];
    rays_o[o + 0] = P[3];
    rays_o[o + 1] = P[7];
    rays_o[o + 2] = P[11];
}

__global__ void __launch_bounds__(1024) k_get_rays_backward(const float* __restrict__ grad_rays_o, const float* __restrict__ grad_rays_d,
                                                            float fx, float fy, float cx, float cy, uint32_t W,
                                                            const int32_t* __restrict__ pixel_inds, uint32_t n_pix,
                                                            float* __restrict__ grad_poses) {
    __shared__ float red[12][1024 / 64];
    const uint32_t cam = blockIdx.x;
    float acc[12];
#pragma unroll
    for (int k = 0; k < 12; k++) acc[k] = 0.0f;
    for (uint32_t p = threadIdx.x; p < n_pix; p += 1024) {
        const uint32_t pix = pixel_inds ? (uint32_t)pixel_inds[p] : p;
        const float i = (float)(pix % W) + 0.5f, j = (float)(pix / W) + 0.5f;
        const float xs = (i - cx) / fx, ys = (j - cy) / fy, zs = 1.0f;
        const float nrm = sqrtf(xs * xs + ys * ys + zs * zs);
        const float u[3] = {xs / nrm, ys / nrm, zs / nrm};
        const size_t o = ((size_t)cam * n_pix + p) * 3;
#pragma unroll
        for (int k = 0; k < 3; k++) {
            const float gd = grad_rays_d ? grad_rays_d[o + k] : 0.0f;
#pragma unroll
            for (int m = 0; m < 3; m++) acc[k * 4 + m] += gd * u[m];
            acc[k * 4 + 3] += grad_rays_o ? grad_rays_o[o + k] : 0.0f;
        }
    }
#pragma unroll
    for (int k = 0; k < 12; k++) {
        const float v = wave_sum_lane0(acc[k]);
        if ((threadIdx.x & 63) == 0) red[k][threadIdx.x >> 6] = v;
    }
    __syncthreads();
    if (threadIdx.x < 16) {
        float v = 0.0f;
        if (threadIdx.x < 12)
            for (int w = 0; w < 1024 / 64; w++) v += red[threadIdx.x][w];
        grad_poses[(size_t)cam * 16 + threadIdx.x] = v;
    }
}

}

using namespace ngp;

__global__ void __launch_bounds__(kBlock) k_finish_rays(float* __restrict__ image, float* __restrict__ depth, const float* __restrict__ weights_sum,
                                                        const float* __restrict__ nears, const float* __restrict__ fars, float bg_r, float bg_g,
                                                        float bg_b, uint32_t N) {
    const uint32_t n = blockIdx.x * kBlock + threadIdx.x;
    if (n >= N) return;
    const float t = 1.0f - weights_sum[n];
    image[(size_t)n * 3] = image[(size_t)n * 3] + t * bg_r;
    image[(size_t)n * 3 + 1] = image[(size_t)n * 3 + 1] + t * bg_g;
    image[(size_t)n * 3 + 2] = image[(size_t)n * 3 + 2] + t * bg_b;
    const float d = depth[n] - nears[n];
    depth[n] = (d != d ? d : fmaxf(d, 0.0f)) / (fars[n] - nears[n]);
}

extern "C" {

int ngp_finish_rays(float* image, float* depth, const float* weights_sum, const float* nears, const float* fars, const float* bg_color3,
                    uint32_t N, ngp_stream_t stream) {
    if (N == 0) return NGP_OK;
    NGP_REQUIRE(image && depth && weights_sum && nears && fars && bg_color3, "finish_rays: null pointer");
    k_finish_rays<<<div_up(N, kBlock), kBlock, 0, (hipStream_t)stream>>>(image, depth, weights_sum, nears, fars, bg_color3[0], bg_color3[1],
                                                                          bg_color3[2], N);
    return check_launch("finish_rays");
}

int ngp_near_far_from_aabb(const float* rays_o, const float* rays_d, const float* aabb, uint32_t N, float min_near, float* nears,
                           float* fars, ngp_stream_t stream) {
    if (N == 0) return NGP_OK;
    NGP_REQUIRE(rays_o && rays_d && aabb && nears && fars, "near_far_from_aabb: null pointer");
    hipStream_t s = (hipStream_t)stream;
    ProfScope prof("near_far_from_aabb", s, N);
    k_near_far_from_aabb<<<div_up(N, kBlock), kBlock, 0, s>>>(rays_o, rays_d, aabb, N, min_near, nears, fars);
    return check_launch("near_far_from_aabb");
}

int ngp_sph_from_ray(const float* rays_o, const float* rays_d, float radius, uint32_t N, float* coords, ngp_stream_t stream) {
    if (N == 0) return NGP_OK;
    NGP_REQUIRE(rays_o && rays_d && coords, "sph_from_ray: null pointer");
    k_sph_from_ray<<<div_up(N, kBlock), kBlock, 0, (hipStream_t)stream>>>(rays_o, rays_d, radius, N, coords);
    return check_launch("sph_from_ray");
}

int ngp_morton3D(const int32_t* coords, uint32_t N, int32_t* indices, ngp_stream_t stream) {
    if (N == 0) return NGP_OK;
    NGP_REQUIRE(coords && indices, "morton3D: null pointer");
    k_morton3D<<<div_up(N, kBlock), kBlock, 0, (hipStream_t)stream>>>(coords, N, indices);
    return check_launch("morton3D");
}

int ngp_morton3D_invert(const int32_t* indices, uint32_t N, int32_t* coords, ngp_stream_t stream) {
    if (N == 0) return NGP_OK;
    NGP_REQUIRE(coords && indices, "morton3D_invert: null pointer");
    k_morton3D_invert<<<div_up(N, kBlock), kBlock, 0, (hipStream_t)stream>>>(indices, N, coords);
    return check_launch("morton3D_invert");
}

int ngp_packbits(const float* grid, uint32_t N, float density_thresh, uint8_t* bitfield, ngp_stream_t stream) {
    if (N == 0) return NGP_OK;
    NGP_REQUIRE(grid && bitfield, "packbits: null pointer");
    hipStream_t s = (hipStream_t)stream;
    ProfScope prof("packbits", s, N);
    k_packbits<<<div_up(div_up(N, 4), kBlock), kBlock, 0, s>>>(grid, N, density_thresh, bitfield);
    return check_launch("packbits");
}

static size_t train_counts_bytes(uint32_t N) {
    const size_t nblocks = div_up(N ? N : 1, kBlock);
    return (((size_t)(N + nblocks + 4) * sizeof(uint32_t)) + 15) & ~(size_t)15;
}

constexpr uint32_t kTraceMaxRays = 16384, kTraceMaxSteps = 1024;
static size_t train_trace_bytes(uint32_t N) { return N <= kTraceMaxRays ? (size_t)N * kTraceMaxSteps * sizeof(float2) : 0; }

size_t ngp_march_rays_train_workspace(uint32_t N) {
    return train_counts_bytes(N) + kTrainLinBytes + kCoarseMaxBytes + train_trace_bytes(N);
}

int ngp_march_rays_train(const float* rays_o, const float* rays_d, const uint8_t* grid, float bound, float dt_gamma, uint32_t max_steps,
                         uint32_t N, uint32_t C, uint32_t H, uint32_t M, const float* nears, const float* fars, float* xyzs, float* dirs,
                         float* deltas, int32_t* rays, int32_t* counter, uint32_t perturb, void* workspace, size_t workspace_bytes,
                         ngp_stream_t stream) {
    if (N == 0) return NGP_OK;
    NGP_REQUIRE(rays_o && rays_d && grid && nears && fars && xyzs && dirs && deltas && rays && counter, "march_rays_train: null pointer");
    NGP_REQUIRE(C >= 1 && C <= 8 && H >= 2 && H <= 1024, "march_rays_train: unsupported cascade/grid size C=%u H=%u", C, H);
    if (!workspace || workspace_bytes < ngp_march_rays_train_workspace(N)) {
        set_error("march_rays_train: workspace of %zu bytes needed, %zu given", ngp_march_rays_train_workspace(N), workspace_bytes);
        return NGP_EWORKSPACE;
    }
    hipStream_t s = (hipStream_t)stream;
    const uint32_t nblocks = div_up(N, kBlock);
    uint32_t* counts = (uint32_t*)workspace;
    uint32_t* block_sums = counts + N;
    uint32_t* base = block_sums + nblocks;
    Pcg32 rng;
    rng.seed(42u);
    ProfScope prof("march_rays_train", s, N);
    OccupancyLin tl = {};
    const bool lin = N >= 1024 && occupancy_lin_fits(C, H, grid, kTrainLinBytes, kCoarseMaxBytes);
    char* extra = (char*)workspace + train_counts_bytes(N);
    float2* trace = nullptr;
    if (lin && train_trace_bytes(N) && max_steps <= kTraceMaxSteps) trace = (float2*)(extra + kTrainLinBytes + kCoarseMaxBytes);
    enum { kWave, kTraced, kLin, kPlain } const form = !lin ? kPlain : (!trace ? kLin : (dt_gamma == 0.0f ? kWave : kTraced));
    if (lin) tl = build_occupancy_lin(grid, C, H, extra, extra + kTrainLinBytes, s);
#define NGP_COUNT(LIN_, TRACE_)                                                                                                                   \
    k_march_train_count<LIN_, TRACE_><<<nblocks, kBlock, 0, s>>>(rays_o, rays_d, grid, bound, dt_gamma, max_steps, N, C, H, nears, fars, perturb, rng, \
                                                                 counts, block_sums, tl, trace)
#define NGP_WRITE(LIN_, TRACE_)                                                                                                                      \
    k_march_train_write<LIN_, TRACE_><<<nblocks, kBlock, 0, s>>>(rays_o, rays_d, grid, bound, dt_gamma, max_steps, N, C, H, M, nears, fars, perturb, rng, \
                                                                 counts, block_sums, base, xyzs, dirs, deltas, rays, tl, trace)
    switch (form) {
        case kWave:
            (void)hipMemsetAsync(block_sums, 0, (size_t)nblocks * sizeof(uint32_t), s);
            k_march_train_count_wave<<<div_up(N, kBlock / 64), kBlock, 0, s>>>(rays_o, rays_d, grid, bound, max_steps, N, C, H, nears, fars, perturb,
                                                                              rng, counts, block_sums, tl, trace);
            break;
        case kTraced: NGP_COUNT(true, true); break;
        case kLin: NGP_COUNT(true, false); break;
        case kPlain: NGP_COUNT(false, false); break;
    }
    k_march_train_scan<<<1, 1024, 0, s>>>(block_sums, nblocks, N, counter, base);
    switch (form) {
        case kWave:
            k_march_train_write_wave<<<div_up(N, kBlock / 64), kBlock, 0, s>>>(rays_o, rays_d, bound, max_steps, N, M, nears, perturb, rng, counts,
                                                                              block_sums, base, xyzs, dirs, deltas, rays, trace);
            break;
        case kTraced: NGP_WRITE(true, true); break;
        case kLin: NGP_WRITE(true, false); break;
        case kPlain: NGP_WRITE(false, false); break;
    }
#undef NGP_COUNT
#undef NGP_WRITE
    return check_launch("march_rays_train");
}

int ngp_composite_rays_train_forward(const float* sigmas, const float* rgbs, const float* deltas, const int32_t* rays, uint32_t M,
                                     uint32_t N, float* weights_sum, float* depth, float* image, ngp_stream_t stream) {
    if (N == 0) return NGP_OK;
    NGP_REQUIRE(sigmas && rgbs && deltas && rays && weights_sum && depth && image, "composite_rays_train_forward: null pointer");
    hipStream_t s = (hipStream_t)stream;
    ProfScope prof("composite_rays_train_forward", s, M);
    k_composite_train_fwd<<<div_up(N, kBlock), kBlock, 0, s>>>(sigmas, rgbs, deltas, rays, M, N, weights_sum, depth, image);
    return check_launch("composite_rays_train_forward");
}

int ngp_composite_rays_train_backward(const float* grad_weights_sum, const float* grad_image, const float* sigmas, const float* rgbs,
                                      const float* deltas, const int32_t* rays, const float* weights_sum, const float* image, uint32_t M,
                                      uint32_t N, float* grad_sigmas, float* grad_rgbs, ngp_stream_t stream) {
    if (N == 0) return NGP_OK;
    NGP_REQUIRE(grad_weights_sum && grad_image && sigmas && rgbs && deltas && rays && weights_sum && image && grad_sigmas && grad_rgbs,
                "composite_rays_train_backward: null pointer");
    ProfScope prof("composite_rays_train_backward", (hipStream_t)stream, M);
    k_composite_train_bwd<<<div_up(N, kBlock), kBlock, 0, (hipStream_t)stream>>>(grad_weights_sum, grad_image, sigmas, rgbs, deltas, rays,
                                                                                 weights_sum, image, M, N, grad_sigmas, grad_rgbs);
    return check_launch("composite_rays_train_backward");
}

static size_t lin_coarse_offset(uint32_t C, uint32_t H) { return ((size_t)C * H * H * H / 8 + 255) / 256 * 256; }
size_t ngp_occupancy_lin_bytes(uint32_t C, uint32_t H) {
    if (!occupancy_lin_fits(C, H, nullptr, kTrainLinBytes, kCoarseMaxBytes)) return 0;
    return lin_coarse_offset(C, H) + (size_t)C * H * H * H / 512;
}
int ngp_build_occupancy_lin(const uint8_t* grid, uint32_t C, uint32_t H, void* out, size_t out_bytes, ngp_stream_t stream) {
    NGP_REQUIRE(grid && out, "build_occupancy_lin: null pointer");
    const size_t need = ngp_occupancy_lin_bytes(C, H);
    NGP_REQUIRE(need && out_bytes >= need, "build_occupancy_lin: C=%u H=%u needs %zu bytes (0 = not supported), %zu given", C, H, need, out_bytes);
    NGP_REQUIRE(((uintptr_t)grid & 7) == 0 && ((uintptr_t)out & 255) == 0, "build_occupancy_lin: grid must be 8-byte aligned, out 256-byte aligned");
    build_occupancy_lin(grid, C, H, out, (char*)out + lin_coarse_offset(C, H), (hipStream_t)stream);
    return check_launch("build_occupancy_lin");
}

static int march_rays_impl(uint32_t n_alive, uint32_t n_step, const int32_t* rays_alive, const float* rays_t, const float* rays_o,
                           const float* rays_d, float bound, float dt_gamma, uint32_t max_steps, uint32_t C, uint32_t H, const uint8_t* grid,
                           const float* fars, float* xyzs, float* dirs, float* deltas, uint32_t perturb, uint32_t M_padded,
                           const void* occupancy_lin, ngp_stream_t stream) {
    if (M_padded == 0 || n_step == 0) return NGP_OK;
    NGP_REQUIRE(rays_alive && rays_t && rays_o && rays_d && grid && fars && xyzs && dirs && deltas, "march_rays: null pointer");
    NGP_REQUIRE((uint64_t)n_alive * n_step <= M_padded, "march_rays: M_padded=%u smaller than n_alive*n_step", M_padded);
    NGP_REQUIRE(C >= 1 && C <= 8 && H >= 2 && H <= 1024, "march_rays: unsupported cascade/grid size C=%u H=%u", C, H);
    hipStream_t s = (hipStream_t)stream;
    Pcg32 rng;
    rng.seed((uint64_t)perturb);
    const uint32_t n_rows = div_up(M_padded, n_step);
    ProfScope prof("march_rays", s, (double)n_alive * n_step);
    OccupancyLin tl = {};
    if (occupancy_lin) {
        NGP_REQUIRE(occupancy_lin_fits(C, H, nullptr, kTrainLinBytes, kCoarseMaxBytes), "march_rays_lin: C=%u H=%u has no derived occupancy copies (ngp_occupancy_lin_bytes is 0)", C, H);
        tl = occupancy_lin_view(C, H, occupancy_lin, (const char*)occupancy_lin + lin_coarse_offset(C, H));
        k_march_rays<true><<<div_up(n_rows, kBlock), kBlock, 0, s>>>(n_alive, n_step, rays_alive, rays_t, rays_o, rays_d, bound, dt_gamma, max_steps,
                                                                     C, H, grid, fars, xyzs, dirs, deltas, perturb, rng, n_rows, M_padded, tl);
    } else {
        k_march_rays<false><<<div_up(n_rows, kBlock), kBlock, 0, s>>>(n_alive, n_step, rays_alive, rays_t, rays_o, rays_d, bound, dt_gamma, max_steps,
                                                                      C, H, grid, fars, xyzs, dirs, deltas, perturb, rng, n_rows, M_padded, tl);
    }
    return check_launch("march_rays");
}

int ngp_march_rays_lin(uint32_t n_alive, uint32_t n_step, const int32_t* rays_alive, const float* rays_t, const float* rays_o,
                       const float* rays_d, float bound, float dt_gamma, uint32_t max_steps, uint32_t C, uint32_t H, const uint8_t* grid,
                       const float* nears, const float* fars, float* xyzs, float* dirs, float* deltas, uint32_t perturb, uint32_t M_padded,
                       const void* occupancy_lin, ngp_stream_t stream) {
    (void)nears;
    NGP_REQUIRE(occupancy_lin, "march_rays_lin: occupancy_lin is NULL (ngp_build_occupancy_lin fills it; ngp_march_rays needs none)");
    return march_rays_impl(n_alive, n_step, rays_alive, rays_t, rays_o, rays_d, bound, dt_gamma, max_steps, C, H, grid, fars, xyzs, dirs, deltas,
                           perturb, M_padded, occupancy_lin, stream);
}

int ngp_march_rays(uint32_t n_alive, uint32_t n_step, const int32_t* rays_alive, const float* rays_t, const float* rays_o,
                   const float* rays_d, float bound, float dt_gamma, uint32_t max_steps, uint32_t C, uint32_t H, const uint8_t* grid,
                   const float* nears, const float* fars, float* xyzs, float* dirs, float* deltas, uint32_t perturb, uint32_t M_padded,
                   ngp_stream_t stream) {
    (void)nears;
    return march_rays_impl(n_alive, n_step, rays_alive, rays_t, rays_o, rays_d, bound, dt_gamma, max_steps, C, H, grid, fars, xyzs, dirs, deltas,
                           perturb, M_padded, nullptr, stream);
}

// ... 34 lines not shown
```

### nerfsafetyvalidation_amd/csrc/render_fused.hip

```cpp
#include <hip/hip_fp16.h>
#include <math.h>
#include <string.h>

#include <atomic>

#include "fused_net.hpp"
#include "occupancy.hpp"

namespace ngp {

constexpr int kWaves = 8;
constexpr int kThreads = kWaves * 64;
constexpr int kWavesPerSimd = 4;
constexpr int kCh = 2;
constexpr int kSlots = 64 * kCh;
constexpr size_t kLinMaxBytes = 4u << 20;
constexpr int kLookahead = 4;
constexpr int kRing = 8;

struct Ctl {
    uint32_t n_alive, n_step, step, done;
    uint32_t iters, last_n_alive, last_n_step, pad;
    unsigned long long samples_marched, samples_slots;
    uint32_t spec, rollbacks, backoff, rsv;
};

constexpr uint32_t kSpecK = 8;
constexpr uint32_t kSpecMarginDiv = 16;
constexpr uint32_t kSpecMaxQ = 8;
constexpr uint32_t kSpecMaxSamples = 32;
constexpr uint32_t kSpecMidSamples = 8;
constexpr uint32_t kSpecSafetyX2 = 1;
constexpr int kDeathShards = 64;
constexpr uint32_t kDeathWords = 2u * kDeathShards * kSpecK;
struct QueueHeads { uint32_t head[8][32]; };

constexpr int kStatShards = 64;

struct RenderArgs {
    const float *rays_o, *rays_d, *fars;
    float* rays_t;
    float *weights_sum, *depth, *image;
    float *last_sigmas, *last_rgbs;
    float pad_sigma, pad_r, pad_g, pad_b;
    float4* dump_rec;
    uint32_t* dump_iter;
    const int32_t* alive_in;
    int32_t* staging;
    uint32_t* chunk_count;
    uint32_t sort_slow;
    Ctl* ctl;
    QueueHeads* heads;
    unsigned long long* stat_shards;
    uint32_t* death_shards;
    float4* backup;
    const uint8_t* bitfield;
    uint32_t cascade, grid_size, max_steps, perturb;
    float dt_gamma;
    Pcg32 rng;
    OccupancyLin occ;
    uint32_t block_jump;
    uint32_t* sample_hash;
    unsigned long long* stamps;
    float2* march_samples;
    uint8_t* march_counts;
    uint32_t wave_slots;
    uint32_t n_rays;
    uint32_t pre_verdict;
    uint32_t wave_march_max;
    uint32_t cell_runs;
};

__host__ __device__ __forceinline__ uint32_t item_width(uint32_t n_alive, uint32_t wave_slots) {
    return n_alive >= 64u * wave_slots ? 64u : (n_alive >= 32u * wave_slots ? 32u : 16u);
}
__device__ __forceinline__ void truncate_launch(Ctl& c, const uint32_t* exhausted, uint32_t N) {
    if (!c.spec) return;
    const uint32_t q = c.spec, K = c.n_step / q;
    uint32_t alive = c.n_alive, ok = K;
    for (uint32_t j = 0; j < K; j++) {
        if (alive == 0) break;
        const uint32_t want_q = N / alive;
        if (j > 0 && (want_q < 1 ? 1u : (want_q > 8 ? 8u : want_q)) != q) { ok = j; break; }
        alive -= exhausted[j] < alive ? exhausted[j] : alive;
    }
    if (ok < K) {
        if (ok <= 1) { c.spec = 0; c.n_step = q; }
        else c.n_step = ok * q;
        c.rsv += 1;
    }
}
static uint32_t items_bound(uint32_t ub, uint32_t wave_slots) {
    const uint32_t by64 = div_up(ub ? ub : 1, 64), narrow = div_up(ub ? ub : 1, 16);
    const uint32_t cap = 2u * wave_slots + 1u;
    return by64 > (narrow < cap ? narrow : cap) ? by64 : (narrow < cap ? narrow : cap);
}

struct WaveSlab {
    float t[kSlots], dt[kSlots], sig[kSlots];
    uint32_t rg[kSlots], b[kSlots];
    uint16_t list[kSlots];
    float od[64][6];
};

__device__ __forceinline__ void dump_row(const RenderArgs& ra, uint32_t entry, int32_t ray, uint32_t n_step, uint32_t k, float sg, float r,
                                         float g, float b) {
    if (ra.dump_rec) {
        ra.dump_rec[(size_t)ray * 8 + k] = make_float4(sg, r, g, b);
    } else {
        const size_t row = (size_t)entry * n_step + k;
        ra.last_sigmas[row] = sg;
        ra.last_rgbs[row * 3] = r; ra.last_rgbs[row * 3 + 1] = g; ra.last_rgbs[row * 3 + 2] = b;
    }
}

__device__ __forceinline__ void march_ahead_wave(const RenderArgs& ra, float bound, const Ctl& ctl, const uint32_t* coarse) {
    const uint32_t lane = threadIdx.x & 63u;
    const uint32_t entry = blockIdx.x * 4u + (threadIdx.x >> 6);
    if (entry >= ctl.n_alive) return;
    const uint32_t n_step = ctl.n_step, spec = ctl.spec;
    const int32_t ray = ra.alive_in[entry];
    Dda dda;
    const float t_c = ra.rays_t[ray], far = ra.fars[ray];
    float t_march = dda.start(ra.rays_o + (size_t)ray * 3, ra.rays_d + (size_t)ray * 3, ra.bitfield, bound, 0.0f, ra.max_steps, ra.cascade,
                              ra.grid_size, &ra.occ, ra.block_jump != 0, t_c, ra.perturb, ra.rng, entry);
    float last_m = t_march, geo_tc = t_c;
    uint32_t emitted = 0, rounds = 0;
    float2* out = ra.march_samples + ((size_t)(entry >> 6) * n_step) * 64 + (entry & 63u);
    while (t_march < far && emitted < n_step) {
        rounds++;
        const LatticeWindow w = probe_window(dda, t_march, far, lane, coarse);
        const uint32_t room = spec ? spec - emitted % spec : n_step - emitted;
        unsigned long long emit = 0ull;
        uint32_t cur = 0, cnt = 0;
        float t_next = t_march;
        for (int guard = 0; guard < 64; guard++) {
            const float to = __uint_as_float((uint32_t)__builtin_amdgcn_readlane((int)__float_as_uint(w.nxt), (int)cur));
            if ((w.omask >> cur) & 1ull) {
                emit |= 1ull << cur;
                const float d1 = to - last_m;
                last_m = to;
                geo_tc += d1;
                if (++cnt == room) { t_next = to; break; }
            }
            const uint32_t jn = (uint32_t)__builtin_amdgcn_readlane((int)w.j, (int)cur);
            if (jn >= 64u || !((w.vmask >> jn) & 1ull)) { t_next = to; break; }
            cur = jn;
        }
        if ((emit >> lane) & 1ull) out[(size_t)(emitted + (uint32_t)__popcll(emit & ((1ull << lane) - 1ull))) * 64] = make_float2(w.p, w.dt);
        emitted += cnt;
        t_march = t_next;
        if (spec && cnt == room) {
            t_march = geo_tc;
            last_m = geo_tc;
        }
    }
    if (lane != 0) return;
    if (ra.stamps) {
        atomicAdd(ra.stamps + 4, (unsigned long long)rounds);
        atomicAdd(ra.stamps + 5, (unsigned long long)rounds * 64ull);
        atomicAdd(ra.stamps + 6, 1ull);
        atomicMax(ra.stamps + 7, (unsigned long long)rounds);
    }
    if (spec && ra.pre_verdict && emitted < n_step)
        atomicAdd(ra.death_shards + (size_t)kDeathShards * kSpecK + (blockIdx.x % kDeathShards) * kSpecK + emitted / spec, 1u);
    bool slow = false;
    if (ra.sort_slow && emitted == n_step) slow = geo_tc < far && dda.coarse_empty_at_lin(geo_tc, coarse);
    ra.march_counts[entry] = (uint8_t)(emitted | (slow ? 128u : 0u));
}

template <bool LIN>
__global__ void __launch_bounds__(256) k_march_ahead(RenderArgs ra, float bound) {
    const Ctl ctl = *ra.ctl;
    if (ctl.done) return;
    const uint32_t n_alive = ctl.n_alive, n_step = ctl.n_step, spec = ctl.spec;
    const bool by_wave = LIN && n_alive <= ra.wave_march_max;
    if (blockIdx.x * (by_wave ? 4u : 256u) >= n_alive) return;
    __shared__ uint32_t coarse_lds[kCoarseMaxBytes / 4];
    stage_coarse(ra.occ, coarse_lds, blockDim.x);
    __syncthreads();
    const uint32_t* coarse = ra.occ.coarse_words ? coarse_lds : nullptr;
    if (LIN && by_wave) {
        march_ahead_wave(ra, bound, ctl, coarse);
        return;
    }
    const uint32_t entry = blockIdx.x * blockDim.x + threadIdx.x;
    if (entry >= n_alive) return;
    const int32_t ray = ra.alive_in[entry];
    Dda dda;
    const float t_c = ra.rays_t[ray], far = ra.fars[ray];
    float t_march = dda.start(ra.rays_o + (size_t)ray * 3, ra.rays_d + (size_t)ray * 3, ra.bitfield, bound, ra.dt_gamma, ra.max_steps, ra.cascade,
                              ra.grid_size, LIN ? &ra.occ : nullptr, ra.block_jump != 0, t_c, ra.perturb, ra.rng, entry);
    float last_m = t_march;
    float geo_tc = t_c;
    uint32_t emitted = 0;
    float2* out = ra.march_samples + ((size_t)(entry >> 6) * n_step) * 64 + (entry & 63u);
    float x, y, z, dt;
    uint32_t probes = 0, probes_coarse_empty = 0, probes_fine_empty = 0;
    const bool run_cells = LIN && dda.const_dt && ra.cell_runs != 0;
    float occ_until = 0.0f;
    while (t_march < far && emitted < n_step) {
        probes++;
        const bool diag_ce = LIN && ra.stamps && dda.coarse_empty_at_lin(t_march, coarse);
        const uint32_t emitted_before = emitted;
        if (LIN ? dda.probe_lin(t_march, x, y, z, dt, coarse, run_cells ? &occ_until : nullptr) : dda.probe(t_march, x, y, z, dt, coarse)) {
            do {
                out[(size_t)emitted * 64] = make_float2(t_march, dt);
                t_march += dt;
                const float d1 = t_march - last_m;
                last_m = t_march;
                geo_tc += d1;
                emitted++;
                if (spec && emitted % spec == 0) {
                    t_march = geo_tc;
                    last_m = geo_tc;
                }
            } while (run_cells && t_march < occ_until && t_march < far && emitted < n_step);
        }
        if (ra.stamps && emitted == emitted_before) { if (diag_ce) probes_coarse_empty++; else probes_fine_empty++; }
    }
    if (ra.stamps) {
        uint32_t mx = probes, sm = probes;
#pragma unroll
        for (int off = 32; off > 0; off >>= 1) {
            const uint32_t o = (uint32_t)__shfl_xor((int)mx, off, 64), p2 = (uint32_t)__shfl_xor((int)sm, off, 64);
            mx = mx > o ? mx : o;
            sm += p2;
        }
        if ((threadIdx.x & 63u) == (uint32_t)__builtin_ctzll(__ballot(true))) {
            atomicAdd(ra.stamps + 4, (unsigned long long)mx);
            atomicAdd(ra.stamps + 5, (unsigned long long)sm);
            atomicAdd(ra.stamps + 6, 1ull);
            atomicMax(ra.stamps + 7, (unsigned long long)mx);
        }
        uint32_t ce = probes_coarse_empty, fe = probes_fine_empty;
        ce = wave_sum(ce);
        fe = wave_sum(fe);
        if ((threadIdx.x & 63u) == (uint32_t)__builtin_ctzll(__ballot(true))) {
            atomicAdd(ra.stamps + 14, (unsigned long long)ce);
            atomicAdd(ra.stamps + 15, (unsigned long long)fe);
        }
    }
    if (spec && ra.pre_verdict) {
        const uint32_t K = n_step / spec, jd = emitted < n_step ? emitted / spec : 0xFFFFFFFFu;
        const unsigned long long act = __ballot(true);
        const bool leader = (threadIdx.x & 63u) == (uint32_t)__builtin_ctzll(act);
        uint32_t* ex = ra.death_shards + (size_t)kDeathShards * kSpecK + (blockIdx.x % kDeathShards) * kSpecK;
        for (uint32_t j = 0; j < K; j++) {
            const unsigned long long b = __ballot(jd == j);
            if (leader && b) atomicAdd(&ex[j], (uint32_t)__popcll(b));
        }
    }
    bool slow = false;
    if (ra.sort_slow && emitted == n_step) slow = geo_tc < far && (LIN ? dda.coarse_empty_at_lin(geo_tc, coarse) : dda.coarse_empty_at(geo_tc, coarse));
    ra.march_counts[entry] = (uint8_t)(emitted | (slow ? 128u : 0u));
}

template <int MODE, bool HACC = false>
__global__ void __launch_bounds__(kThreads, kWavesPerSimd) k_render_iter(NetArgs na, GridLevels lv, RenderArgs ra) {
    Ctl ctl = *ra.ctl;
    if (ctl.done) return;
    const uint32_t n_step_marched = ctl.n_step;
    extern __shared__ __attribute__((aligned(16))) char smem[];
    if (ctl.spec) {
        uint32_t* exhausted = reinterpret_cast<uint32_t*>(smem);
        if (threadIdx.x < kSpecK) {
            uint32_t d = 0;
            for (int sh = 0; sh < kDeathShards; sh++) d += ra.death_shards[(size_t)kDeathShards * kSpecK + sh * kSpecK + threadIdx.x];
            exhausted[threadIdx.x] = d;
        }
        __syncthreads();
        truncate_launch(ctl, exhausted, ra.n_rays);
        __syncthreads();
    }
    const uint32_t n_alive = ctl.n_alive, n_step = ctl.n_step;
    const uint32_t spec = ctl.spec;
    const uint32_t W = item_width(n_alive, ra.wave_slots);
    const uint32_t n_chunks = (n_alive + W - 1) / W;

    const size_t w_bytes = net_w_bytes_f16(na);
    _Float16* Wlds = reinterpret_cast<_Float16*>(smem);
    LevelTab* lt = reinterpret_cast<LevelTab*>(smem + w_bytes);
    WaveSlab* slabs = reinterpret_cast<WaveSlab*>(smem + w_bytes + sizeof(LevelTab));
    stage_block(na, lv, Wlds, lt, w_bytes);

    const uint32_t lane = threadIdx.x & 63, wid = threadIdx.x >> 6, c = lane & 15;
    WaveSlab& S = slabs[wid];
    unsigned long long ts0 = 0, ts1 = 0;
#define NGP_STAMP(idx)                                                                  \
    if (ra.stamps) {                                                                    \
        ts1 = __builtin_amdgcn_s_memtime();                                             \
        if (lane == 0) atomicAdd(ra.stamps + (idx), ts1 - ts0);                         \
        ts0 = ts1;                                                                      \
    }

    const uint32_t n_shards = gridDim.x < 8u ? gridDim.x : 8u;
    const uint32_t shard = blockIdx.x % n_shards;
    unsigned long long wave_total = 0;
    for (;;) {
        uint32_t chunk = 0xFFFFFFFFu;
        {
            uint32_t k = 0;
            if (lane == 0) k = atomicAdd(&ra.heads->head[shard][0], 1u);
            k = __builtin_amdgcn_readfirstlane(k);
            const uint32_t cand = k * n_shards + shard;
            if (cand < n_chunks) chunk = cand;
        }
        if (chunk == 0xFFFFFFFFu) break;
        if (ra.stamps) ts0 = __builtin_amdgcn_s_memtime();

        const uint32_t first_entry = chunk * W, group = first_entry >> 6;
        const uint32_t entry = group * 64 + lane;
        const bool active = entry < n_alive && entry - first_entry < W;
        const int32_t ray = active ? ra.alive_in[entry] : -1;

        float last_t = 0, t_c = 0, t_c0 = 0, t_start = 0;
        float ws = 0, dep = 0, cr = 0, cg = 0, cb = 0;
        uint32_t emitted = 0;
        bool slow_next = false;
        if (active) {
            t_c = ra.rays_t[ray];
            t_c0 = t_c;
            t_start = t_c;
            if (ra.perturb) {
                const float SQRT3 = 1.7320508075688772f;
                Pcg32 rng = ra.rng;
                rng.advance((int64_t)entry);
                t_start += (2 * SQRT3 / (float)ra.max_steps) * rng.next_float();
            }
            last_t = t_start;
            const uint32_t mc = ra.march_counts[entry];
            emitted = mc & 63u;
            slow_next = (mc & 128u) != 0;
            ws = ra.weights_sum[ray]; dep = ra.depth[ray];
            cr = ra.image[(size_t)ray * 3]; cg = ra.image[(size_t)ray * 3 + 1]; cb = ra.image[(size_t)ray * 3 + 2];
#pragma unroll
            for (int d = 0; d < 3; d++) { S.od[lane][d] = ra.rays_o[(size_t)ray * 3 + d]; S.od[lane][3 + d] = ra.rays_d[(size_t)ray * 3 + d]; }
            if (spec) {
                ra.backup[(size_t)ray * 2] = make_float4(t_c, ws, dep, ra.sample_hash ? __uint_as_float(ra.sample_hash[ray]) : 0.0f);
                ra.backup[(size_t)ray * 2 + 1] = make_float4(cr, cg, cb, 0.0f);
            }
        }
        const float2* marched = ra.march_samples + ((size_t)group * n_step_marched) * 64 + lane;
        bool running = active;
        uint32_t steps_done = 0;
        uint32_t wave_samples = 0;

        for (uint32_t s0 = 0; s0 < n_step; s0 += kCh) {
            const uint32_t want = (n_step - s0) < (uint32_t)kCh ? (n_step - s0) : (uint32_t)kCh;
            uint32_t cnt = 0;
            const bool do_march = active && (running || (ra.last_sigmas != nullptr && !spec));
            if (do_march) {
                const uint32_t left = emitted > s0 ? emitted - s0 : 0u;
                cnt = left < want ? left : want;
                for (uint32_t k = 0; k < cnt; k++) {
                    const float2 v = marched[(size_t)(s0 + k) * 64];
                    S.t[lane * kCh + k] = v.x;
                    S.dt[lane * kCh + k] = v.y;
                }
            }
            if (!__any(cnt != 0)) {
                if (running && cnt < want) running = false;
                if (ra.last_sigmas && active && !spec)
                    for (uint32_t k = 0; k < want; k++) dump_row(ra, entry, ray, n_step, s0 + k, ra.pad_sigma, ra.pad_r, ra.pad_g, ra.pad_b);
                if (!ra.last_sigmas && !__any(running)) break;
                continue;
            }
            NGP_STAMP(0)
            uint32_t incl = cnt;
#pragma unroll
            for (int off = 1; off < 64; off <<= 1) {
                const uint32_t o = __shfl_up(incl, off, 64);
                if (lane >= (uint32_t)off) incl += o;
            }
// ... 211 lines not shown
    truncate_launch(c, exhausted, N);
    if (threadIdx.x == 0) {
        uint32_t bad = 0, keep = 0;
        if (c.spec) {
            const uint32_t q = c.spec, K = c.n_step / q;
            uint32_t alive = c.n_alive;
            keep = K;
            for (uint32_t j = 0; j < K; j++) {
                if (alive == 0) break;
                const uint32_t want_q = N / alive;
                if (j > 0 && (want_q < 1 ? 1u : (want_q > 8 ? 8u : want_q)) != q) { bad = 1; keep = j; break; }
                alive -= deaths[j];
                if ((spec_allowed & 2u) && alive == 0) { bad = 1; keep = j; break; }
            }
        }
        verdict_bad = bad;
        verdict_keep = keep;
    }
    __syncthreads();
    if (verdict_bad) {
        for (uint32_t e = first * W + threadIdx.x; e < (first + 8) * W && e < c.n_alive; e += 256) {
            const int32_t ray = alive_in[e];
            const float4 a = backup[(size_t)ray * 2], b = backup[(size_t)ray * 2 + 1];
            rays_t[ray] = a.x; weights_sum[ray] = a.y; depth[ray] = a.z;
            if (sample_hash) sample_hash[ray] = __float_as_uint(a.w);
            image[(size_t)ray * 3] = b.x; image[(size_t)ray * 3 + 1] = b.y; image[(size_t)ray * 3 + 2] = b.z;
            alive_out[e] = ray;
        }
        if (g == n_blocks - 1 && threadIdx.x == 0) {
            Ctl n = c;
            n.rollbacks = c.rollbacks + 1;
            if (verdict_keep >= 2 && !(spec_allowed & 4u)) {
                n.spec = c.spec;
                n.n_step = verdict_keep * c.spec;
                n.backoff = 0;
                for (uint32_t i = 0; i < kDeathWords; i++) death_next[i] = 0;
            } else {
                n.spec = 0;
                const uint32_t ns = c.n_alive ? N / c.n_alive : 8;
                n.n_step = ns < 1 ? 1 : (ns > 8 ? 8 : ns);
                n.backoff = 2;
            }
            for (int i = 0; i < kStatShards; i++) stat_shards_rw[i] = 0ull;
            *nxt = n;
            for (int i = 0; i < 8; i++) nxt_heads->head[i][0] = 0;
            publish_status(host_slot, n, seq, fin_host, call_tag);
        }
        return;
    }
    uint32_t pf = 0, ps = 0, tf = 0;
    for (uint32_t j = threadIdx.x; j < n_chunks; j += 256) {
        const uint32_t v = chunk_count[j];
        tf += v >> 16;
        if (j < first) { pf += v & 0xffffu; ps += v >> 16; }
    }
#pragma unroll
    for (int off = 32; off > 0; off >>= 1) {
        pf += __shfl_down(pf, off, 64);
        ps += __shfl_down(ps, off, 64);
        tf += __shfl_down(tf, off, 64);
    }
    if ((threadIdx.x & 63) == 0) { red[0][threadIdx.x >> 6] = pf; red[1][threadIdx.x >> 6] = ps; red[2][threadIdx.x >> 6] = tf; }
    if (threadIdx.x == 0) {
        uint32_t af = 0, as = 0;
        for (uint32_t i = 0; i < 8; i++) {
            const uint32_t v = (first + i < n_chunks) ? chunk_count[first + i] : 0;
            off_f[i] = af; off_s[i] = as;
            af += v & 0xffffu; as += v >> 16;
        }
        off_f[8] = af; off_s[8] = as;
    }
    __syncthreads();
    const uint32_t prefix_f = red[0][0] + red[0][1] + red[0][2] + red[0][3];
    const uint32_t prefix_s = red[1][0] + red[1][1] + red[1][2] + red[1][3];
    const uint32_t total_s = red[2][0] + red[2][1] + red[2][2] + red[2][3];
    const uint32_t lane = threadIdx.x & 63, w = threadIdx.x >> 6;
#pragma unroll
    for (uint32_t h = 0; h < 2; h++) {
        const uint32_t ci = w * 2 + h;
        const uint32_t nf = off_f[ci + 1] - off_f[ci], ns = off_s[ci + 1] - off_s[ci];
        if (lane < ns) alive_out[prefix_s + off_s[ci] + lane] = staging[(size_t)(first + ci) * W + W - 1 - lane];
        if (lane < nf) alive_out[total_s + prefix_f + off_f[ci] + lane] = staging[(size_t)(first + ci) * W + lane];
    }
    unsigned long long marched = threadIdx.x < (uint32_t)kStatShards ? stat_shards_rw[threadIdx.x] : 0ull;
#pragma unroll
    for (int off = 32; off > 0; off >>= 1) marched += __shfl_down(marched, off, 64);
    if (g == n_blocks - 1 && threadIdx.x == 0) {
        Ctl n = c;
        n.samples_marched = c.samples_marched + marched;
        for (int i = 0; i < kStatShards; i++) stat_shards_rw[i] = 0ull;
        n.n_alive = total_s + prefix_f + off_f[8];
        uint32_t recent = c.n_alive - n.n_alive;
        if (!c.spec) {
            n.last_n_alive = c.n_alive;
            n.last_n_step = c.n_step;
            n.iters = c.iters + 1;
            n.samples_slots = c.samples_slots + (unsigned long long)c.n_alive * c.n_step;
            n.step = c.step + c.n_step;
        } else {
            const uint32_t q = c.spec, K = c.n_step / q;
            uint32_t alive = c.n_alive, d_last = 0, d_prev = 0;
            unsigned long long slots = c.samples_slots;
            uint32_t it = 0;
            for (uint32_t j = 0; j < K; j++) {
                if (alive == 0) break;
                slots += (unsigned long long)alive * q;
                it++;
                n.last_n_alive = alive;
                n.last_n_step = q;
                alive -= deaths[j];
                d_prev = d_last;
                d_last = deaths[j];
            }
            recent = d_last > d_prev ? d_last : d_prev;
            n.iters = c.iters + it;
            n.samples_slots = slots;
            n.step = c.step + it * q;
        }
        uint32_t ns = n.n_alive ? N / n.n_alive : 8;
        n.n_step = ns < 1 ? 1 : (ns > 8 ? 8 : ns);
        n.done = (n.n_alive == 0 || n.step >= max_steps) ? 1 : 0;
        n.spec = 0;
        if (n.backoff) n.backoff--;
        else if (spec_allowed && !n.done && n.n_step <= kSpecMaxQ && (n.n_step == 8 || n.n_alive > N / (n.n_step + 1))) {
            const uint32_t q = n.n_step;
            const bool own_last = (spec_allowed & 2u) != 0;
            uint32_t room = (max_steps - n.step) / q;
            if (own_last && room) room--;
            const uint32_t headroom = n.n_alive - (q == 8 ? 0u : N / (q + 1)) - 1;
            uint32_t sq = 0;
            while ((unsigned long long)(sq + 1) * (sq + 1) <= recent) sq++;
            const unsigned long long rate = (unsigned long long)recent + 4ull * sq + 16ull;
            uint32_t K = (uint32_t)((unsigned long long)headroom * 2u / (kSpecSafetyX2 * rate));
            const uint32_t cap_mid = 8u * q < cap_mid_max ? 8u * q : cap_mid_max;
            const uint32_t cap_samples = q == 1 ? 8u : (q <= 4 ? cap_mid : cap_hi);
            const uint32_t capK = cap_samples / q < kSpecK ? cap_samples / q : kSpecK;
            K = (q == 8 && !own_last) ? capK : (K < capK ? K : capK);
            K = K < room ? K : room;
            if (K >= 2) { n.spec = q; n.n_step = K * q; }
        }
        if (n.spec)
            for (uint32_t i = 0; i < kDeathWords; i++) death_next[i] = 0;
        *nxt = n;
        for (int i = 0; i < 8; i++) nxt_heads->head[i][0] = 0;
        publish_status(host_slot, n, seq, fin_host, call_tag);
    }
}

__global__ void __launch_bounds__(256) k_render_init(uint32_t N, const float* __restrict__ nears, float* __restrict__ rays_t,
                                                      int32_t* __restrict__ alive, float* __restrict__ weights_sum, float* __restrict__ depth,
                                                      float* __restrict__ image, Ctl* __restrict__ ctl, uint32_t max_steps,
                                                      uint32_t* __restrict__ sample_hash, unsigned long long* __restrict__ stat_shards,
                                                      QueueHeads* __restrict__ heads, uint32_t* __restrict__ death_shards, uint32_t spec_allowed,
                                                      uint32_t tile_w) {
    const uint32_t n = blockIdx.x * 256 + threadIdx.x;
    if (n < (uint32_t)kStatShards) stat_shards[n] = 0ull;
    if (n < 2u * kDeathWords) death_shards[n] = 0;
    if (n < 16) heads[n >> 3].head[n & 7][0] = 0;
    if (n < N) {
        if (sample_hash) sample_hash[n] = 2166136261u;
        uint32_t first = n;
        if (tile_w) {
            const uint32_t t = n >> 4, in = n & 15u, per_row = tile_w >> 2;
            first = ((t / per_row) * 4u + (in >> 2)) * tile_w + (t % per_row) * 4u + (in & 3u);
        }
        alive[n] = (int32_t)first;
        rays_t[n] = nears[n];
        weights_sum[n] = 0; depth[n] = 0;
        image[(size_t)n * 3] = 0; image[(size_t)n * 3 + 1] = 0; image[(size_t)n * 3 + 2] = 0;
    }
    if (n == 0) {
        Ctl c = {};
        c.n_alive = N;
        c.n_step = 1;
        c.done = (N == 0 || max_steps == 0) ? 1 : 0;
        const uint32_t room = (spec_allowed & 2u) ? (max_steps ? max_steps - 1 : 0) : max_steps;
        if (spec_allowed && !c.done && N > N / 2 + N / kSpecMarginDiv && room >= 2) {
            c.spec = 1;
            c.n_step = room < kSpecK ? room : kSpecK;
        }
        ctl[0] = c;
        ctl[1] = c;
    }
}

__global__ void __launch_bounds__(256) k_dump_count(const uint32_t* __restrict__ dump_iter, uint32_t N, const Ctl* __restrict__ fin_state,
                                                     uint32_t* __restrict__ block_sums) {
    __shared__ uint32_t ws[4];
    const uint32_t last_iter = fin_state->iters - 1;
    const uint32_t n = blockIdx.x * 256 + threadIdx.x;
    const bool f = n < N && dump_iter[n] == last_iter;
    const uint32_t c = (uint32_t)__popcll(__ballot(f));
    if ((threadIdx.x & 63) == 0) ws[threadIdx.x >> 6] = c;
    __syncthreads();
    if (threadIdx.x == 0) block_sums[blockIdx.x] = ws[0] + ws[1] + ws[2] + ws[3];
}
__global__ void __launch_bounds__(1024) k_dump_scan(uint32_t* __restrict__ block_sums, uint32_t nblocks) {
    scan_in_place_1024(block_sums, nblocks);
}
__global__ void __launch_bounds__(256) k_dump_gather(const uint32_t* __restrict__ dump_iter, const float4* __restrict__ rec, uint32_t N,
                                                      const Ctl* __restrict__ fin_state, const uint32_t* __restrict__ block_off,
                                                      float* __restrict__ last_sigmas, float* __restrict__ last_rgbs, float ps, float pr, float pg,
                                                      float pb) {
    __shared__ uint32_t ws[4];
    const uint32_t n = blockIdx.x * 256 + threadIdx.x;
    const uint32_t lane = threadIdx.x & 63, wid = threadIdx.x >> 6;
    if (fin_state->iters == 0) return;
    const uint32_t last_iter = fin_state->iters - 1, n_alive = fin_state->last_n_alive, n_step = fin_state->last_n_step;
    const bool f = n < N && dump_iter[n] == last_iter;
    const unsigned long long bal = __ballot(f);
    if (lane == 0) ws[wid] = (uint32_t)__popcll(bal);
    __syncthreads();
    uint32_t rank = block_off[blockIdx.x] + (uint32_t)__popcll(bal & ((1ull << lane) - 1ull));
    for (uint32_t w = 0; w < wid; w++) rank += ws[w];
    if (f) {
        for (uint32_t k = 0; k < n_step; k++) {
            const float4 v = rec[(size_t)n * 8 + k];
            const size_t row = (size_t)rank * n_step + k;
            last_sigmas[row] = v.x;
            last_rgbs[row * 3] = v.y; last_rgbs[row * 3 + 1] = v.z; last_rgbs[row * 3 + 2] = v.w;
        }
    }
    if (n < 128) {
        const size_t row = (size_t)n_alive * n_step + n;
        last_sigmas[row] = ps;
        last_rgbs[row * 3] = pr; last_rgbs[row * 3 + 1] = pg; last_rgbs[row * 3 + 2] = pb;
    }
}

}

using namespace ngp;

struct ngp_render_ctx {
    uint32_t max_rays = 0;
    uint32_t frame_width = 0;
    int32_t* alive[2] = {nullptr, nullptr};
    int32_t* staging = nullptr;
    uint32_t* chunk_count = nullptr;
    float* rays_t = nullptr;
    unsigned long long* coarse = nullptr;
    uint32_t* grid_lin = nullptr;
    uint32_t* death_shards = nullptr;
    float4* backup = nullptr;
    float2* march_samples = nullptr;
    uint8_t* march_counts = nullptr;
    float4* dump_rec = nullptr;
    uint32_t* dump_iter = nullptr;
    Ctl* ctl = nullptr;
    unsigned long long* stat_shards = nullptr;
    QueueHeads* heads = nullptr;
    _Float16* packed = nullptr;
    unsigned long long* status = nullptr;
    unsigned long long* status_dev = nullptr;
    unsigned long long* fin = nullptr;
    unsigned long long* fin_dev = nullptr;
    uint32_t calls = 0;
    uint32_t seq_base = 0;
    hipEvent_t ev[kRing];
    int num_cu = 256;
    bool has_debug = false;
    DebugState debug;
    void* owned[20] = {};
    uint32_t n_owned = 0;
};

template <typename T>
static bool ctx_alloc(ngp_render_ctx* c, T** p, size_t bytes) {
    if (c->n_owned == sizeof(c->owned) / sizeof(c->owned[0]) || hipMalloc(p, bytes) != hipSuccess) return false;
    c->owned[c->n_owned++] = *p;
    return true;
}

static DebugState debug_snapshot(const ngp_render_ctx* ctx) { return ctx->has_debug ? ctx->debug : ngp::debug_snapshot(); }

extern "C" {

int ngp_render_ctx_create(uint32_t max_rays, ngp_render_ctx** out) {
    NGP_REQUIRE(out, "render_ctx_create: null out pointer");
    NGP_REQUIRE(max_rays > 0, "render_ctx_create: max_rays must be positive");
    ngp_render_ctx* c = new ngp_render_ctx();
    c->max_rays = max_rays;
    const size_t chunks = div_up(max_rays, 64);
    bool ok = true;
    int dev = 0;
    hipDeviceProp_t prop;
    if (hipGetDevice(&dev) == hipSuccess && hipGetDeviceProperties(&prop, dev) == hipSuccess) c->num_cu = prop.multiProcessorCount;
    const size_t max_items = items_bound(max_rays, (uint32_t)c->num_cu * 16u) + 8;
    ok &= ctx_alloc(c, &c->alive[0], (size_t)max_rays * 4);
    ok &= ctx_alloc(c, &c->alive[1], (size_t)max_rays * 4);
    ok &= ctx_alloc(c, &c->staging, chunks * 64 * 4);
    ok &= ctx_alloc(c, &c->chunk_count, (max_items > (size_t)div_up(max_rays, 256) ? max_items : (size_t)div_up(max_rays, 256)) * 4);
    ok &= ctx_alloc(c, &c->rays_t, (size_t)max_rays * 4);
    ok &= ctx_alloc(c, &c->coarse, kCoarseMaxBytes);
    ok &= ctx_alloc(c, &c->ctl, 2 * sizeof(Ctl));
    ok &= ctx_alloc(c, &c->stat_shards, kStatShards * sizeof(unsigned long long));
    ok &= ctx_alloc(c, &c->death_shards, 2 * (size_t)kDeathWords * sizeof(uint32_t));
    ok &= ctx_alloc(c, &c->backup, (size_t)max_rays * 2 * sizeof(float4));
    ok &= ctx_alloc(c, &c->march_samples, ((size_t)max_rays + 512) * 8 * sizeof(float2));
    ok &= ctx_alloc(c, &c->march_counts, (size_t)max_rays);
    ok &= ctx_alloc(c, &c->heads, 2 * sizeof(QueueHeads));
    ok &= ctx_alloc(c, &c->packed, (size_t)(sig_halfs(2) + sig_halfs(3)) * 2);
    ok &= hipHostMalloc(&c->status, kRing * sizeof(unsigned long long), hipHostMallocMapped | hipHostMallocCoherent) == hipSuccess;
    if (ok) {
        memset(c->status, 0, kRing * sizeof(unsigned long long));
        ok &= hipHostGetDevicePointer((void**)&c->status_dev, c->status, 0) == hipSuccess;
    }
    ok &= hipHostMalloc(&c->fin, 4 * sizeof(unsigned long long), hipHostMallocMapped | hipHostMallocCoherent) == hipSuccess;
    if (ok) {
        memset(c->fin, 0, 4 * sizeof(unsigned long long));
        ok &= hipHostGetDevicePointer((void**)&c->fin_dev, c->fin, 0) == hipSuccess;
    }
    for (int i = 0; i < kRing; i++) ok &= hipEventCreateWithFlags(&c->ev[i], hipEventDisableTiming) == hipSuccess;
    if (!ok) {
        set_error("render_ctx_create: allocation failed: %s", hipGetErrorString(hipGetLastError()));
        ngp_render_ctx_destroy(c);
        return NGP_ENODEVICE;
    }
    *out = c;
    return NGP_OK;
}

int ngp_render_ctx_set_frame_width(ngp_render_ctx* ctx, uint32_t width) {
    NGP_REQUIRE(ctx, "render_ctx_set_frame_width: null context");
    ctx->frame_width = width;
    return NGP_OK;
}

int ngp_render_ctx_destroy(ngp_render_ctx* c) {
    if (!c) return NGP_OK;
    (void)hipDeviceSynchronize();
    for (uint32_t i = 0; i < c->n_owned; i++) (void)hipFree(c->owned[i]);
    if (c->status) (void)hipHostFree(c->status);
    if (c->fin) (void)hipHostFree(c->fin);
    for (int i = 0; i < kRing; i++) (void)hipEventDestroy(c->ev[i]);
    delete c;
    return NGP_OK;
}

static std::atomic<int> g_active_renders{0};
struct ActiveRender {
    ActiveRender() { g_active_renders.fetch_add(1, std::memory_order_relaxed); }
    ~ActiveRender() { g_active_renders.fetch_sub(1, std::memory_order_relaxed); }
};

static bool choose_occupancy(ngp_render_ctx* ctx, const ngp_model* model, const DebugState& dbg, hipStream_t s, RenderArgs& ra) {
    const uint32_t C = model->cascade, H = model->grid_size;
    const size_t cells = (size_t)C * H * H * H;
    bool lin = !dbg.coarse_off() && !dbg.lin_off() && occupancy_lin_fits(C, H, model->density_bitfield, kLinMaxBytes, kCoarseMaxBytes);
    const bool use_coarse = !dbg.coarse_off() && cells % 4096 == 0 && cells / 64 / 8 <= kCoarseMaxBytes && ((uintptr_t)model->density_bitfield & 7) == 0;
    if (lin && !ctx->grid_lin && !ctx_alloc(ctx, &ctx->grid_lin, kLinMaxBytes)) lin = false;
    if (lin) {
        ra.occ = build_occupancy_lin(model->density_bitfield, C, H, ctx->grid_lin, ctx->coarse, s);
        ra.block_jump = dbg.jump_off() ? 0u : 1u;
    } else if (use_coarse) {
        const uint32_t n_words = (uint32_t)(cells / 64);
        k_build_coarse<<<div_up(n_words, 256), 256, 0, s>>>((const unsigned long long*)model->density_bitfield, n_words, ctx->coarse);
        ra.occ.coarse = (const uint32_t*)ctx->coarse;
        ra.occ.coarse_words = n_words / 32;
    } else {
        ra.sort_slow = 0;
    }
    return lin;
}

static void fill_render_args(const ngp_render_ctx* ctx, const ngp_model* model, const DebugState& dbg, uint32_t N, float dt_gamma,
                             uint32_t max_steps, uint32_t perturb, RenderArgs& ra) {
    ra.rays_t = ctx->rays_t;
    ra.staging = ctx->staging; ra.chunk_count = ctx->chunk_count; ra.stat_shards = ctx->stat_shards;
    ra.wave_slots = dbg.narrow_items_off() ? 0u : (uint32_t)ctx->num_cu * 16u;
    ra.pre_verdict = dbg.pre_verdict_off() ? 0u : 1u;
    ra.cell_runs = dbg.cell_runs_off() ? 0u : 1u;
    ra.wave_march_max = (dbg.wave_march_off() || dt_gamma != 0.0f) ? 0u : (uint32_t)ctx->num_cu * 64u;
    ra.backup = ctx->backup;
    ra.march_samples = ctx->march_samples; ra.march_counts = ctx->march_counts;
    ra.bitfield = model->density_bitfield; ra.cascade = model->cascade; ra.grid_size = model->grid_size;
    ra.max_steps = max_steps; ra.perturb = perturb; ra.dt_gamma = dt_gamma;
    ra.n_rays = N;
    ra.rng.seed((uint64_t)perturb);
    ra.stamps = dbg.stamps;
    ra.sort_slow = (perturb == 0 && !dbg.sort_off()) ? 1u : 0u;
    ra.sample_hash = dbg.sample_hash;
}

typedef void (*IterKernel)(NetArgs, GridLevels, RenderArgs);
static IterKernel choose_iter_kernel(const NetArgs& na, const GridLevels& lv) {
    static const IterKernel kIter[2][3] = {{k_render_iter<0, false>, k_render_iter<1, false>, k_render_iter<2, false>},
                                           {k_render_iter<0, true>, k_render_iter<1, true>, k_render_iter<2, true>}};
    return kIter[na.hacc() ? 1 : 0][needs_generic(lv) ? 1 : (na.cells ? 2 : 0)];
}

static void enqueue_launch(ngp_render_ctx* ctx, const NetArgs& na, const GridLevels& lv, RenderArgs& ra, IterKernel iter_kernel, size_t lds,
                           bool lin, uint32_t ub, uint32_t launched, uint32_t spec_allowed, uint32_t call_tag, hipStream_t s) {
    const uint32_t cur = launched & 1;
    const uint32_t chunks = items_bound(ub, ra.wave_slots);
    const uint32_t blocks_per_cu = lds <= 80 * 1024 ? 2 : 1;
    const uint32_t blocks_pct = g_active_renders.load(std::memory_order_relaxed) > 1 ? 62u : 100u;
    const uint32_t max_blocks = (uint32_t)ctx->num_cu * blocks_per_cu * blocks_pct / 100u;
    const uint32_t want_blocks = div_up(chunks, kWaves);
    const uint32_t blocks = want_blocks < max_blocks ? want_blocks : max_blocks;
    ra.alive_in = ctx->alive[cur];
    ra.ctl = ctx->ctl + cur;
    ra.heads = ctx->heads + cur;
    ra.death_shards = ctx->death_shards + (size_t)cur * kDeathWords;
    {
        ProfScope pm("k_march_ahead", s, 0);
        const uint32_t by_wave = div_up(ub < ra.wave_march_max ? ub : ra.wave_march_max, 4);
        const uint32_t by_lane = div_up(ub ? ub : 1, 256);
        if (lin) k_march_ahead<true><<<by_lane > by_wave ? by_lane : by_wave, 256, 0, s>>>(ra, na.bound);
        else k_march_ahead<false><<<div_up(ub ? ub : 1, 256), 256, 0, s>>>(ra, na.bound);
    }
    {
        ProfScope pk("k_render_iter", s, 0);
        iter_kernel<<<blocks, kThreads, lds, s>>>(na, lv, ra);
    }
    k_render_compact<<<div_up(chunks, 8), 256, 0, s>>>(ctx->ctl + cur, ctx->ctl + (cur ^ 1), ctx->staging, ctx->chunk_count,
                                                       ctx->alive[cur ^ 1], ra.n_rays, ra.max_steps, ctx->stat_shards, ctx->heads + (cur ^ 1),
                                                       ctx->status_dev + launched % kRing, ctx->seq_base + launched + 1,
                                                       ctx->death_shards + (size_t)cur * kDeathWords, spec_allowed, ctx->alive[cur],
                                                       ctx->backup, ctx->rays_t, ra.weights_sum, ra.depth, ra.image, ra.sample_hash, ctx->stat_shards,
                                                       ctx->death_shards + (size_t)(cur ^ 1) * kDeathWords, ra.wave_slots, kSpecMidSamples,
                                                       kSpecMaxSamples, ctx->fin_dev, call_tag);
}

static int consume_status(const ngp_render_ctx* ctx, hipStream_t s, uint32_t launched, uint32_t call_tag, bool trace, uint32_t& known,
                          uint32_t& ub, bool& done) {
    while (known < launched) {
        const bool must_wait = launched - known >= (uint32_t)kLookahead;
        volatile unsigned long long* slot = ctx->status + known % kRing;
        const uint32_t want_seq = ctx->seq_base + known + 1;
        unsigned long long w = *slot;
        if ((uint32_t)(w >> 32) != want_seq) {
            if (!must_wait) break;
            uint32_t spins = 0;
            while ((uint32_t)((w = *slot) >> 32) != want_seq) {
                if ((++spins & 0xFFFFFu) == 0) {
                    const hipError_t q = hipStreamQuery(s);
                    if (q != hipSuccess && q != hipErrorNotReady) {
                        set_error("render_rays: %s", hipGetErrorString(q));
                        return NGP_ELAUNCH;
                    }
                    if (q == hipSuccess && (uint32_t)(*slot >> 32) != want_seq) {
                        set_error("render_rays: the device finished without publishing iteration %u", known);
                        return NGP_ELAUNCH;
                    }
                }
                __builtin_ia32_pause();
            }
        }
        known++;
        ub = (uint32_t)w & 0x7FFFFFFFu;
        if (trace) fprintf(stderr, "[ngp] call %u launch %u: n_alive %u%s\n", call_tag, known, ub, ((w >> 31) & 1ull) ? " done" : "");
        if ((w >> 31) & 1ull) { done = true; break; }
    }
    return NGP_OK;
}

static int read_counters(const ngp_render_ctx* ctx, hipStream_t s, const Ctl* last, uint32_t call_tag, uint32_t N, uint32_t launches, int sync,
                         ngp_render_stats* stats_host) {
    bool have_fin = false;
    Ctl fin = {};
    if (stats_host && !sync) {
        volatile unsigned long long* f = ctx->fin;
        unsigned long long w[4] = {0, 0, 0, 0};
        for (uint32_t spin = 0; spin < 200000u && !have_fin; spin++) {
            bool all = true;
            for (int i = 0; i < 4; i++) {
                w[i] = f[i];
                all = all && (w[i] >> 48) == (0x8000u | call_tag);
            }
            have_fin = all;
            if (!have_fin) __builtin_ia32_pause();
        }
        if (have_fin) {
            fin.samples_marched = w[0] & 0xFFFFFFFFFFFFull;
            fin.samples_slots = w[1] & 0xFFFFFFFFFFFFull;
            fin.iters = (uint32_t)((w[2] >> 24) & 0xFFFFFFu);
            fin.rollbacks = (uint32_t)(w[2] & 0xFFFFFFu);
            fin.last_n_alive = (uint32_t)((w[3] >> 8) & 0xFFFFFFFFu);
            fin.last_n_step = (uint32_t)(w[3] & 0xFFu);
        }
    }
    if ((stats_host && !have_fin) || sync) {
        if (hipStreamSynchronize(s) != hipSuccess || hipMemcpy(&fin, last, sizeof(Ctl), hipMemcpyDeviceToHost) != hipSuccess) {
            set_error("render_rays: %s", hipGetErrorString(hipGetLastError()));
            return NGP_ELAUNCH;
        }
        have_fin = true;
    }
    if (have_fin && stats_host) {
        stats_host->samples_marched = fin.samples_marched;
        stats_host->samples_slots = fin.samples_slots;
        stats_host->iterations = fin.iters;
        stats_host->rays = N;
        stats_host->last_n_alive = fin.last_n_alive;
        stats_host->last_n_step = fin.last_n_step;
        stats_host->launches = launches;
        stats_host->replayed = fin.rollbacks;
        prof_add_units("k_render_iter", (double)fin.samples_marched);
    }
    return NGP_OK;
}

int ngp_render_rays(ngp_render_ctx* ctx, const ngp_model* model, const float* rays_o, const float* rays_d, const float* nears,
                    const float* fars, uint32_t N, float dt_gamma, uint32_t max_steps, uint32_t perturb, float* weights_sum, float* depth,
                    float* image, float* last_sigmas, float* last_rgbs, const float* pad_value_host, ngp_render_stats* stats_host, int sync,
                    ngp_stream_t stream) {
    NGP_REQUIRE(ctx, "render_rays: null context");
    NGP_REQUIRE(N <= ctx->max_rays, "render_rays: %u rays exceed the context capacity %u", N, ctx->max_rays);
    NGP_REQUIRE((last_sigmas == nullptr) == (last_rgbs == nullptr), "render_rays: last_sigmas and last_rgbs must both be given or both NULL");
    if (stats_host) *stats_host = ngp_render_stats{};
    if (N == 0) return NGP_OK;
    const ActiveRender active_render;
    NGP_REQUIRE(rays_o && rays_d && nears && fars && weights_sum && depth && image, "render_rays: null pointer");
    NGP_REQUIRE(model && model->density_bitfield, "render_rays: model has no density bitfield");
    NGP_REQUIRE(model->cascade >= 1 && model->cascade <= 8 && model->grid_size >= 2 && model->grid_size <= 1024,
                "render_rays: unsupported cascade/grid size");
    hipStream_t s = (hipStream_t)stream;
    const DebugState dbg = debug_snapshot(ctx);
    NetArgs na;
    GridLevels lv;
    const _Float16* packed = model && model->packed_weights ? (const _Float16*)model->packed_weights : ctx->packed;
    int rc = fill_net(model, packed, na, lv);
    if (rc) return rc;
    NGP_REQUIRE(!na.f32(), "render_rays: the occupancy-grid loop is built for the fp16 network (ngp_model::precision == NGP_PREC_F16)");
    if (!model->packed_weights) {
        const uint32_t n_packed = sig_halfs(na.sig_mm) + sig_halfs(na.col_mm);
        k_pack_weights<<<div_up(n_packed, 256), 256, 0, s>>>((const _Float16*)model->sigma_weights, na.sig_mm,
                                                             (const _Float16*)model->color_weights, na.col_mm, ctx->packed);
    }
    const uint32_t spec_allowed = (!dbg.spec_off() && perturb == 0) ? (1u | (last_sigmas ? 2u : 0u) | (dbg.prefix_replay_off() ? 4u : 0u)) : 0u;
    const uint32_t fw = ctx->frame_width;
    const uint32_t tile_w = (perturb == 0 && !dbg.tile_off() && fw >= 4 && fw % 4 == 0 && N % (4 * fw) == 0) ? fw : 0u;
    const uint32_t init_threads = N > 2u * kDeathWords ? N : 2u * kDeathWords;
    k_render_init<<<div_up(init_threads, 256), 256, 0, s>>>(N, nears, ctx->rays_t, ctx->alive[0], weights_sum, depth, image, ctx->ctl, max_steps,
                                                 dbg.sample_hash, ctx->stat_shards, ctx->heads, ctx->death_shards, spec_allowed, tile_w);

    RenderArgs ra = {};
    ra.rays_o = rays_o; ra.rays_d = rays_d; ra.fars = fars;
    ra.weights_sum = weights_sum; ra.depth = depth; ra.image = image;
    ra.last_sigmas = last_sigmas; ra.last_rgbs = last_rgbs;
    if (pad_value_host) { ra.pad_sigma = pad_value_host[0]; ra.pad_r = pad_value_host[1]; ra.pad_g = pad_value_host[2]; ra.pad_b = pad_value_host[3]; }
    fill_render_args(ctx, model, dbg, N, dt_gamma, max_steps, perturb, ra);
    const bool lin = choose_occupancy(ctx, model, dbg, s, ra);
    if ((ra.sort_slow || tile_w) && last_sigmas) {
        if (!ctx->dump_rec) {
            if (!ctx_alloc(ctx, &ctx->dump_rec, (size_t)ctx->max_rays * 8 * sizeof(float4)) ||
                !ctx_alloc(ctx, &ctx->dump_iter, (size_t)ctx->max_rays * 4)) {
                set_error("render_rays: cannot allocate the per-ray record buffer");
                return NGP_ENODEVICE;
            }
        }
        (void)hipMemsetAsync(ctx->dump_iter, 0xff, (size_t)N * 4, s);
        ra.dump_rec = ctx->dump_rec;
        ra.dump_iter = ctx->dump_iter;
    }
    const size_t lds = weights_bytes(na) + sizeof(LevelTab) + (size_t)kWaves * sizeof(WaveSlab);
    const IterKernel iter_kernel = choose_iter_kernel(na, lv);
    ensure_dynamic_lds(reinterpret_cast<const void*>(iter_kernel), 160 * 1024);
    NGP_REQUIRE(lds <= 160 * 1024, "render_rays: LDS budget exceeded (%zu bytes)", lds);

    const bool trace = env_set("NGP_TRACE_SCHEDULE");
    const uint32_t call_tag = ++ctx->calls & 0x7FFFu;
    uint32_t ub = N;
    uint32_t launched = 0;
    uint32_t known = 0;
    bool done = false;
    while (!done) {
        enqueue_launch(ctx, na, lv, ra, iter_kernel, lds, lin, ub, launched, spec_allowed, call_tag, s);
        launched++;
        rc = consume_status(ctx, s, launched, call_tag, trace, known, ub, done);
        if (rc) return rc;
        if (launched > 2u * max_steps + 16u) {
            set_error("render_rays: iteration bound exceeded");
            return NGP_ELAUNCH;
        }
    }
    ctx->seq_base += launched;
    const Ctl* last = ctx->ctl + (launched & 1);
    if (ra.dump_rec) {
        const uint32_t nb = div_up(N, 256);
        k_dump_count<<<nb, 256, 0, s>>>(ctx->dump_iter, N, last, ctx->chunk_count);
        k_dump_scan<<<1, 1024, 0, s>>>(ctx->chunk_count, nb);
        k_dump_gather<<<nb, 256, 0, s>>>(ctx->dump_iter, ctx->dump_rec, N, last, ctx->chunk_count,
                                         last_sigmas, last_rgbs, ra.pad_sigma, ra.pad_r, ra.pad_g, ra.pad_b);
    }
    rc = check_launch("render_rays");
    if (rc) return rc;
    return read_counters(ctx, s, last, call_tag, N, 2 + 3 * launched, sync, stats_host);
}

int ngp_render_ctx_set_debug(ngp_render_ctx* ctx, int enable, int flags, unsigned long long* stamps, uint32_t* sample_hash) {
    NGP_REQUIRE(ctx, "render_ctx_set_debug: null context");
    if (!debug_flags_valid(flags, "render_ctx_set_debug")) return NGP_EINVAL;
    ctx->has_debug = enable != 0;
    ctx->debug.flags = flags; ctx->debug.stamps = stamps; ctx->debug.sample_hash = sample_hash;
    return NGP_OK;
}

}
```

### nerfsafetyvalidation_amd/raymarching/raymarching.py

```python
import collections
import threading
import weakref

import torch
from torch.autograd import Function
from torch.amp import custom_bwd, custom_fwd

from .. import _lib

__all__ = ["near_far_from_aabb", "sph_from_ray", "morton3D", "morton3D_invert", "packbits", "march_rays_train",
           "composite_rays_train", "distortion_rays_train", "march_rays", "composite_rays"]

USE_OCCUPANCY_LIN = True

_fwd32 = custom_fwd(device_type="cuda", cast_inputs=torch.float32)
_bwd = custom_bwd(device_type="cuda")


def _dev(t):
    return t if t.is_cuda else t.cuda()


def _rays(rays_o, rays_d):
    return _dev(rays_o).contiguous().view(-1, 3), _dev(rays_d).contiguous().view(-1, 3)
# ... 61 lines not shown
morton3D_invert = _morton3D_invert.apply


class _packbits(Function):
    @staticmethod
    @_fwd32
    def forward(ctx, grid, thresh, bitfield=None):
        grid = _dev(grid).contiguous()
        C, H3 = grid.shape[0], grid.shape[1]
        N = C * H3 // 8
        if bitfield is None:
            bitfield = torch.empty(N, dtype=torch.uint8, device=grid.device)
        L = _lib.lib()
        _lib.check(L.ngp_packbits(_lib.ptr(grid), N, thresh, _lib.ptr(bitfield), _lib.stream()), "packbits")
        return bitfield


packbits = _packbits.apply


class _march_rays_train(Function):
    @staticmethod
    @_fwd32
    def forward(ctx, rays_o, rays_d, bound, density_bitfield, C, H, nears, fars, step_counter=None, mean_count=-1,
                perturb=False, align=-1, force_all_rays=False, dt_gamma=0, max_steps=1024):
        rays_o, rays_d = _rays(rays_o, rays_d)
        density_bitfield = _dev(density_bitfield).contiguous()
        N = rays_o.shape[0]
        M = N * max_steps
        if not force_all_rays and mean_count > 0:
            if align > 0:
                mean_count += align - mean_count % align
            M = mean_count
        dev, dt = rays_o.device, rays_o.dtype
        xyzs = torch.zeros(M, 3, dtype=dt, device=dev)
        dirs = torch.zeros(M, 3, dtype=dt, device=dev)
        deltas = torch.zeros(M, 2, dtype=dt, device=dev)
        rays = torch.empty(N, 3, dtype=torch.int32, device=dev)
        if step_counter is None:
            step_counter = torch.zeros(2, dtype=torch.int32, device=dev)
        L = _lib.lib()
        ws_bytes = L.ngp_march_rays_train_workspace(N)
        ws = torch.empty(ws_bytes, dtype=torch.uint8, device=dev)
        _lib.check(L.ngp_march_rays_train(_lib.ptr(rays_o), _lib.ptr(rays_d), _lib.ptr(density_bitfield), bound, dt_gamma,
                                          max_steps, N, C, H, M, _lib.ptr(nears.contiguous()), _lib.ptr(fars.contiguous()),
                                          _lib.ptr(xyzs), _lib.ptr(dirs), _lib.ptr(deltas), _lib.ptr(rays),
                                          _lib.ptr(step_counter), int(perturb), _lib.ptr(ws), ws_bytes, _lib.stream()),
                   "march_rays_train")
        if force_all_rays or mean_count <= 0:
            m = step_counter[0].item()
            if align > 0:
                m += align - m % align
            xyzs, dirs, deltas = xyzs[:m], dirs[:m], deltas[:m]
        return xyzs, dirs, deltas, rays


march_rays_train = _march_rays_train.apply


class _composite_rays_train(Function):
    @staticmethod
    @_fwd32
    def forward(ctx, sigmas, rgbs, deltas, rays):
        sigmas, rgbs, deltas = sigmas.float().contiguous(), rgbs.float().contiguous(), deltas.float().contiguous()
        rays = rays.contiguous()
        M, N = sigmas.shape[0], rays.shape[0]
        weights_sum = torch.empty(N, dtype=sigmas.dtype, device=sigmas.device)
        depth = torch.empty(N, dtype=sigmas.dtype, device=sigmas.device)
        image = torch.empty(N, 3, dtype=sigmas.dtype, device=sigmas.device)
        L = _lib.lib()
        _lib.check(L.ngp_composite_rays_train_forward(_lib.ptr(sigmas), _lib.ptr(rgbs), _lib.ptr(deltas), _lib.ptr(rays), M, N,
                                                      _lib.ptr(weights_sum), _lib.ptr(depth), _lib.ptr(image),
                                                      _lib.stream()), "composite_rays_train_forward")
        ctx.save_for_backward(sigmas, rgbs, deltas, rays, weights_sum, depth, image)
        ctx.dims = [M, N]
        return weights_sum, depth, image

    @staticmethod
    @_bwd
    def backward(ctx, grad_weights_sum, grad_depth, grad_image):
        grad_weights_sum, grad_image = grad_weights_sum.contiguous(), grad_image.contiguous()
        sigmas, rgbs, deltas, rays, weights_sum, depth, image = ctx.saved_tensors
        M, N = ctx.dims
        grad_sigmas, grad_rgbs = torch.zeros_like(sigmas), torch.zeros_like(rgbs)
        L = _lib.lib()
        _lib.check(L.ngp_composite_rays_train_backward(_lib.ptr(grad_weights_sum), _lib.ptr(grad_image), _lib.ptr(sigmas),
                                                       _lib.ptr(rgbs), _lib.ptr(deltas), _lib.ptr(rays),
                                                       _lib.ptr(weights_sum), _lib.ptr(image), M, N, _lib.ptr(grad_sigmas),
                                                       _lib.ptr(grad_rgbs), _lib.stream()),
                   "composite_rays_train_backward")
        return grad_sigmas, grad_rgbs, None, None


composite_rays_train = _composite_rays_train.apply


def _distortion_workspace(L, N, device):
    nbytes = L.ngp_distortion_workspace(N)
    return (torch.empty(nbytes, dtype=torch.uint8, device=device) if nbytes else None), nbytes


class _distortion_rays_train(Function):
    @staticmethod
    @_fwd32
    def forward(ctx, sigmas, deltas, rays, scale):
        sigmas, deltas, rays = sigmas.float().contiguous(), deltas.float().contiguous(), rays.contiguous()
        scale = None if scale is None else scale.float().contiguous()
        M, N = sigmas.shape[0], rays.shape[0]
        loss_rays = torch.zeros(N, dtype=sigmas.dtype, device=sigmas.device)
        totals = torch.zeros(N, 2, dtype=sigmas.dtype, device=sigmas.device)
        loss = torch.zeros((), dtype=sigmas.dtype, device=sigmas.device)
        L = _lib.lib()
        ws, ws_bytes = _distortion_workspace(L, N, sigmas.device)
        _lib.check(L.ngp_distortion_train_forward(_lib.ptr(sigmas), _lib.ptr(deltas), _lib.ptr(rays), _lib.ptr(scale), M, N, _lib.ptr(loss_rays),
                                                  _lib.ptr(totals), _lib.ptr(loss), _lib.ptr(ws), ws_bytes, _lib.stream()),
                   "distortion_train_forward")
        ctx.save_for_backward(sigmas, deltas, rays, scale, totals)
        ctx.dims = [M, N]
        ctx.mark_non_differentiable(loss_rays)
        return loss, loss_rays

    @staticmethod
    @_bwd
    def backward(ctx, grad_loss, _grad_loss_rays):
        sigmas, deltas, rays, scale, totals = ctx.saved_tensors
        M, N = ctx.dims
        grad_sigmas = torch.zeros_like(sigmas)
        _lib.check(_lib.lib().ngp_distortion_train_backward(_lib.ptr(grad_loss.float().contiguous()), _lib.ptr(sigmas), _lib.ptr(deltas),
                                                            _lib.ptr(rays), _lib.ptr(scale), _lib.ptr(totals), M, N, _lib.ptr(grad_sigmas),
                                                            _lib.stream()), "distortion_train_backward")
        return grad_sigmas, None, None, None


def distortion_rays_train(sigmas, deltas, rays, scale=None, return_rays=False):
    if rays.shape[0] == 0:
        loss, loss_rays = sigmas.float().sum() * 0, sigmas.new_zeros(0, dtype=torch.float32)
    else:
        loss, loss_rays = _distortion_rays_train.apply(sigmas, deltas, rays, scale)
    return (loss, loss_rays) if return_rays else loss


_OCC_LIN = collections.OrderedDict()
_OCC_LIN_LOCK = threading.Lock()
_OCC_LIN_MAX = 8


def _occupancy_lin(density_bitfield, C, H):
    L = _lib.lib()
    nbytes = L.ngp_occupancy_lin_bytes(C, H)
    if not nbytes or not density_bitfield.is_cuda or density_bitfield.data_ptr() % 8 or density_bitfield.dtype != torch.uint8:
        return None
    stream = _lib.stream()
    key = (id(density_bitfield), int(stream or 0), C, H)
    with _OCC_LIN_LOCK:
        hit = _OCC_LIN.get(key)
        if hit is not None:
            ref, version, ptr, buf = hit
            if ref() is density_bitfield and version == density_bitfield._version and ptr == density_bitfield.data_ptr():
                _OCC_LIN.move_to_end(key)
                return buf
            del _OCC_LIN[key]
    buf = torch.empty(nbytes, dtype=torch.uint8, device=density_bitfield.device)
    _lib.check(L.ngp_build_occupancy_lin(_lib.ptr(density_bitfield), C, H, _lib.ptr(buf), nbytes, stream), "build_occupancy_lin")
    with _OCC_LIN_LOCK:
        _OCC_LIN[key] = (weakref.ref(density_bitfield), density_bitfield._version, density_bitfield.data_ptr(), buf)
        while len(_OCC_LIN) > _OCC_LIN_MAX:
            _OCC_LIN.popitem(last=False)
    return buf


class _march_rays(Function):
    @staticmethod
    @_fwd32
    def forward(ctx, n_alive, n_step, rays_alive, rays_t, rays_o, rays_d, bound, density_bitfield, C, H, near, far,
                align=-1, perturb=False, dt_gamma=0, max_steps=1024):
        rays_o, rays_d = _rays(rays_o, rays_d)
        M = n_alive * n_step
        if align > 0:
            M += align - (M % align)
        dev, dt = rays_o.device, rays_o.dtype
        xyzs = torch.empty(M, 3, dtype=dt, device=dev)
        dirs = torch.empty(M, 3, dtype=dt, device=dev)
        deltas = torch.empty(M, 2, dtype=dt, device=dev)
        L = _lib.lib()
        occ = _occupancy_lin(density_bitfield, C, H) if USE_OCCUPANCY_LIN else None
        if occ is not None:
            _lib.check(L.ngp_march_rays_lin(n_alive, n_step, _lib.ptr(rays_alive), _lib.ptr(rays_t), _lib.ptr(rays_o),
                                            _lib.ptr(rays_d), bound, dt_gamma, max_steps, C, H, _lib.ptr(density_bitfield),
                                            _lib.ptr(near), _lib.ptr(far), _lib.ptr(xyzs), _lib.ptr(dirs), _lib.ptr(deltas),
                                            int(perturb), M, _lib.ptr(occ), _lib.stream()), "march_rays_lin")
        else:
            _lib.check(L.ngp_march_rays(n_alive, n_step, _lib.ptr(rays_alive), _lib.ptr(rays_t), _lib.ptr(rays_o),
                                        _lib.ptr(rays_d), bound, dt_gamma, max_steps, C, H, _lib.ptr(density_bitfield),
                                        _lib.ptr(near), _lib.ptr(far), _lib.ptr(xyzs), _lib.ptr(dirs), _lib.ptr(deltas),
                                        int(perturb), M, _lib.stream()), "march_rays")
        return xyzs, dirs, deltas


march_rays = _march_rays.apply


class _composite_rays(Function):
    @staticmethod
    @_fwd32
    def forward(ctx, n_alive, n_step, rays_alive, rays_t, sigmas, rgbs, deltas, weights_sum, depth, image):
        sigmas, rgbs = sigmas.float().contiguous(), rgbs.float().contiguous()
        L = _lib.lib()
        _lib.check(L.ngp_composite_rays(n_alive, n_step, _lib.ptr(rays_alive), _lib.ptr(rays_t), _lib.ptr(sigmas),
                                        _lib.ptr(rgbs), _lib.ptr(deltas), _lib.ptr(weights_sum), _lib.ptr(depth),
                                        _lib.ptr(image), _lib.stream()), "composite_rays")
        return tuple()


composite_rays = _composite_rays.apply
```

Before: 7.608 billion samples/s.

## Cache occupancy layouts by bitfield generation and specialize march kernel on diagnostics

Adds a host-side generation counter per density bitfield, bumped whenever packbits or the density-grid finish rewrites it, or when Python sees a tensor version change. The render context then skips rebuilding the linear and coarse occupancy structures while the key is unchanged. The march-ahead kernel gets a compile-time DIAG flag so diagnostic counters are removed from the normal path, and it gains a launch_bounds occupancy hint. The dump_iter memset is folded into the init kernel. The cost is that the cache could go stale if the bitfield is changed by a path that does not touch the generation.

```diff
diff --git a/include/ngp_hip.h b/include/ngp_hip.h
--- a/include/ngp_hip.h
+++ b/include/ngp_hip.h
@@ -39,6 +39,8 @@
 NGP_API int ngp_morton3D(const int32_t* coords, uint32_t N, int32_t* indices, ngp_stream_t stream);
 NGP_API int ngp_morton3D_invert(const int32_t* indices, uint32_t N, int32_t* coords, ngp_stream_t stream);
 NGP_API int ngp_packbits(const float* grid, uint32_t N, float density_thresh, uint8_t* bitfield, ngp_stream_t stream);
+NGP_API unsigned long long ngp_bitfield_generation(const void* bitfield);
+NGP_API int ngp_bitfield_touch(const void* bitfield);
 
 NGP_API size_t ngp_march_rays_train_workspace(uint32_t N);
 NGP_API int ngp_march_rays_train(const float* rays_o, const float* rays_d, const uint8_t* grid, float bound, float dt_gamma,
@@ -192,6 +194,7 @@
 NGP_API int ngp_render_ctx_destroy(ngp_render_ctx* ctx);
 
 NGP_API int ngp_render_ctx_set_frame_width(ngp_render_ctx* ctx, uint32_t width);
+NGP_API int ngp_render_ctx_occupancy_builds(const ngp_render_ctx* ctx, unsigned long long* builds);
 
 NGP_API int ngp_render_rays(ngp_render_ctx* ctx, const ngp_model* model, const float* rays_o, const float* rays_d,
                     const float* nears, const float* fars, uint32_t N, float dt_gamma, uint32_t max_steps,
diff --git a/nerfsafetyvalidation_amd/_fused.py b/nerfsafetyvalidation_amd/_fused.py
--- a/nerfsafetyvalidation_amd/_fused.py
+++ b/nerfsafetyvalidation_amd/_fused.py
@@ -302,6 +302,15 @@
                 self._ctxs[key] = ent
         return ent[0]
 
+    def occupancy_builds(self):
+        with self._ctx_lock:
+            ent = self._ctxs.get(threading.get_ident())
+        if ent is None:
+            return 0
+        n = C.c_ulonglong(0)
+        _lib.check(_lib.lib().ngp_render_ctx_occupancy_builds(ent[0], C.byref(n)), "render_ctx_occupancy_builds")
+        return int(n.value)
+
     def render(self, net_bitfield_owner, rays_o, rays_d, nears, fars, dt_gamma, max_steps, perturb, want_last=True, want_stats=True,
                frame_width=0):
         bitfield = net_bitfield_owner.density_bitfield
@@ -317,6 +326,7 @@
         m = self._struct(bitfield)
         lib = _lib.lib()
         ctx = self._context(N)
+        _lib.bitfield_generation(bitfield)
         need_stats = want_stats or want_last
         _lib.check(lib.ngp_render_ctx_set_frame_width(ctx, int(frame_width or 0)), "render_ctx_set_frame_width")
         if self.debug is not None:
diff --git a/nerfsafetyvalidation_amd/_lib.py b/nerfsafetyvalidation_amd/_lib.py
--- a/nerfsafetyvalidation_amd/_lib.py
+++ b/nerfsafetyvalidation_amd/_lib.py
@@ -1,5 +1,8 @@
+import collections
 import ctypes as C
 import os
+import threading
+import weakref
 
 import torch
 
@@ -116,6 +119,9 @@
     "ngp_render_ctx_create": [_u32, C.POINTER(_vp)],
     "ngp_render_ctx_destroy": [_vp],
     "ngp_render_ctx_set_frame_width": [_vp, _u32],
+    "ngp_render_ctx_occupancy_builds": [_vp, C.POINTER(C.c_ulonglong)],
+    "ngp_bitfield_generation": [_vp],
+    "ngp_bitfield_touch": [_vp],
     "ngp_render_rays": [_vp, C.POINTER(ModelStruct), _vp, _vp, _vp, _vp, _u32, _f32, _u32, _u32, _vp, _vp, _vp, _vp, _vp,
                         C.POINTER(C.c_float), C.POINTER(RenderStats), _int, _vp],
     "ngp_network_forward": [C.POINTER(ModelStruct), _vp, _vp, _u32, _vp, _vp, _vp],
@@ -174,7 +180,7 @@
     "ngp_prof_read": [C.c_char_p, C.POINTER(C.c_double), C.POINTER(C.c_uint64), C.POINTER(C.c_double)],
 }
 _RESTYPES = {"ngp_render_uniform_backward_lds": _sz, "ngp_cell_tables_bytes": _sz, "ngp_packed_weights_bytes": _sz, "ngp_packed_weights_bwd_bytes": _sz, "ngp_grid_encode_backward_workspace": _sz,
-             "ngp_ffmlp_backward_workspace": _sz, "ngp_ffmlp_backward_buffer_bytes": _sz, "ngp_render_upsample_workspace": _sz, "ngp_density_grid_workspace": _sz, "ngp_last_error": C.c_char_p, "ngp_march_rays_train_workspace": _sz, "ngp_uq_stats_workspace": _sz, "ngp_sigma_fit_workspace": _sz, "ngp_occupancy_lin_bytes": _sz, "ngp_edt_sq_workspace": _sz, "ngp_isosurface_workspace": _sz, "ngp_sift_workspace": _sz, "ngp_sift_layer_offset": _sz, "ngp_photo_loss_workspace": _sz, "ngp_image_quality_workspace": _sz, "ngp_distortion_workspace": _sz, "ngp_distance_stats_state_bytes": _sz, "ngp_distance_stats_workspace": _sz}
+             "ngp_ffmlp_backward_workspace": _sz, "ngp_ffmlp_backward_buffer_bytes": _sz, "ngp_render_upsample_workspace": _sz, "ngp_density_grid_workspace": _sz, "ngp_last_error": C.c_char_p, "ngp_march_rays_train_workspace": _sz, "ngp_uq_stats_workspace": _sz, "ngp_sigma_fit_workspace": _sz, "ngp_occupancy_lin_bytes": _sz, "ngp_bitfield_generation": C.c_ulonglong, "ngp_edt_sq_workspace": _sz, "ngp_isosurface_workspace": _sz, "ngp_sift_workspace": _sz, "ngp_sift_layer_offset": _sz, "ngp_photo_loss_workspace": _sz, "ngp_image_quality_workspace": _sz, "ngp_distortion_workspace": _sz, "ngp_distance_stats_state_bytes": _sz, "ngp_distance_stats_workspace": _sz}
 
 _lib = None
 
@@ -228,6 +234,24 @@
     raise RuntimeError(f"unsupported dtype {t.dtype}: the grid encoder supports float32 and float16")
 
 
+_BITFIELD_SEEN = collections.OrderedDict()
+_BITFIELD_LOCK = threading.Lock()
+_BITFIELD_MAX = 64
+
+
+def bitfield_generation(t):
+    L, p = lib(), t.data_ptr()
+    with _BITFIELD_LOCK:
+        seen = _BITFIELD_SEEN.get(p)
+        if seen is None or seen[0]() is not t or seen[1] != t._version:
+            check(L.ngp_bitfield_touch(p), "bitfield_touch")
+            _BITFIELD_SEEN[p] = (weakref.ref(t), t._version)
+        _BITFIELD_SEEN.move_to_end(p)
+        while len(_BITFIELD_SEEN) > _BITFIELD_MAX:
+            _BITFIELD_SEEN.popitem(last=False)
+        return int(L.ngp_bitfield_generation(p))
+
+
 def host_i32(t):
     cached = getattr(t, "_ngp_host_i32", None)
     if cached is not None and cached[0] == t._version and cached[1] == t.data_ptr():
diff --git a/nerfsafetyvalidation_amd/csrc/capi.hip b/nerfsafetyvalidation_amd/csrc/capi.hip
--- a/nerfsafetyvalidation_amd/csrc/capi.hip
+++ b/nerfsafetyvalidation_amd/csrc/capi.hip
@@ -4,6 +4,7 @@
 #include <string.h>
 
 #include <mutex>
+#include <unordered_map>
 #include <vector>
 
 #include "ngp_common.hpp"
@@ -46,6 +47,20 @@
         if (e.first == dev && e.second == func) return;
     (void)hipFuncSetAttribute(func, hipFuncAttributeMaxDynamicSharedMemorySize, bytes);
     g_attr_done.emplace_back(dev, func);
+}
+
+static std::mutex g_bitfield_mu;
+static std::unordered_map<const void*, unsigned long long> g_bitfield_gen;
+static unsigned long long g_bitfield_counter = 0;
+
+unsigned long long bitfield_generation(const void* bitfield) {
+    std::lock_guard<std::mutex> lk(g_bitfield_mu);
+    const auto it = g_bitfield_gen.find(bitfield);
+    return it == g_bitfield_gen.end() ? 0ull : it->second;
+}
+void bitfield_touch(const void* bitfield) {
+    std::lock_guard<std::mutex> lk(g_bitfield_mu);
+    g_bitfield_gen[bitfield] = ++g_bitfield_counter;
 }
 
 struct ProfEntry {
@@ -247,7 +262,14 @@
 extern "C" {
 
 const char* ngp_last_error(void) { return g_err; }
-int ngp_version(void) { return 100; }
+int ngp_version(void) { return 101; }
+
+unsigned long long ngp_bitfield_generation(const void* bitfield) { return bitfield_generation(bitfield); }
+int ngp_bitfield_touch(const void* bitfield) {
+    NGP_REQUIRE(bitfield, "bitfield_touch: null pointer");
+    bitfield_touch(bitfield);
+    return NGP_OK;
+}
 
 int ngp_device_count(void) {
     int n = 0;
diff --git a/nerfsafetyvalidation_amd/csrc/density_grid.hip b/nerfsafetyvalidation_amd/csrc/density_grid.hip
--- a/nerfsafetyvalidation_amd/csrc/density_grid.hip
+++ b/nerfsafetyvalidation_amd/csrc/density_grid.hip
@@ -200,6 +200,7 @@
     for (uint32_t c = 0; c < cascade; c++) k_grid_possum<<<per, kDgBlock, 0, s>>>(density_grid + (size_t)c * H3, H3, partial + (size_t)c * per);
     k_grid_mean_thresh<<<1, 1024, 0, s>>>(partial, cascade * per, (double)cells, density_thresh, mean_thresh);
     k_packbits_dev<<<div_up(div_up(cells / 8, 4), kDgBlock), kDgBlock, 0, s>>>(density_grid, cells / 8, mean_thresh + 1, bitfield);
+    bitfield_touch(bitfield);
     return check_launch("density_grid_finish");
 }
 
diff --git a/nerfsafetyvalidation_amd/csrc/ngp_common.hpp b/nerfsafetyvalidation_amd/csrc/ngp_common.hpp
--- a/nerfsafetyvalidation_amd/csrc/ngp_common.hpp
+++ b/nerfsafetyvalidation_amd/csrc/ngp_common.hpp
@@ -32,6 +32,9 @@
 void prof_add_units(const char* name, double units);
 
 static inline uint32_t div_up(uint32_t a, uint32_t b) { return (a + b - 1) / b; }
+
+unsigned long long bitfield_generation(const void* bitfield);
+void bitfield_touch(const void* bitfield);
 
 constexpr uint32_t kMeanOneBlockRays = 16384;
 constexpr uint32_t kMeanOneBlockThreads = 1024;
diff --git a/nerfsafetyvalidation_amd/csrc/raymarching.hip b/nerfsafetyvalidation_amd/csrc/raymarching.hip
--- a/nerfsafetyvalidation_amd/csrc/raymarching.hip
+++ b/nerfsafetyvalidation_amd/csrc/raymarching.hip
@@ -678,6 +678,7 @@
     hipStream_t s = (hipStream_t)stream;
     ProfScope prof("packbits", s, N);
     k_packbits<<<div_up(div_up(N, 4), kBlock), kBlock, 0, s>>>(grid, N, density_thresh, bitfield);
+    bitfield_touch(bitfield);
     return check_launch("packbits");
 }
 
diff --git a/nerfsafetyvalidation_amd/csrc/render_fused.hip b/nerfsafetyvalidation_amd/csrc/render_fused.hip
--- a/nerfsafetyvalidation_amd/csrc/render_fused.hip
+++ b/nerfsafetyvalidation_amd/csrc/render_fused.hip
@@ -114,6 +114,7 @@
     }
 }
 
+template <bool DIAG>
 __device__ __forceinline__ void march_ahead_wave(const RenderArgs& ra, float bound, const Ctl& ctl, const uint32_t* coarse) {
     const uint32_t lane = threadIdx.x & 63u;
     const uint32_t entry = blockIdx.x * 4u + (threadIdx.x >> 6);
@@ -156,7 +157,7 @@
         }
     }
     if (lane != 0) return;
-    if (ra.stamps) {
+    if (DIAG && ra.stamps) {
         atomicAdd(ra.stamps + 4, (unsigned long long)rounds);
         atomicAdd(ra.stamps + 5, (unsigned long long)rounds * 64ull);
         atomicAdd(ra.stamps + 6, 1ull);
@@ -169,8 +170,8 @@
     ra.march_counts[entry] = (uint8_t)(emitted | (slow ? 128u : 0u));
 }
 
-template <bool LIN>
-__global__ void __launch_bounds__(256) k_march_ahead(RenderArgs ra, float bound) {
+template <bool LIN, bool DIAG>
+__global__ void __launch_bounds__(256, 8) k_march_ahead(RenderArgs ra, float bound) {
     const Ctl ctl = *ra.ctl;
     if (ctl.done) return;
     const uint32_t n_alive = ctl.n_alive, n_step = ctl.n_step, spec = ctl.spec;
@@ -181,7 +182,7 @@
     __syncthreads();
     const uint32_t* coarse = ra.occ.coarse_words ? coarse_lds : nullptr;
     if (LIN && by_wave) {
-        march_ahead_wave(ra, bound, ctl, coarse);
+        march_ahead_wave<DIAG>(ra, bound, ctl, coarse);
         return;
     }
     const uint32_t entry = blockIdx.x * blockDim.x + threadIdx.x;
@@ -200,10 +201,10 @@
     const bool run_cells = LIN && dda.const_dt && ra.cell_runs != 0;
     float occ_until = 0.0f;
     while (t_march < far && emitted < n_step) {
-        probes++;
-        const bool diag_ce = LIN && ra.stamps && dda.coarse_empty_at_lin(t_march, coarse);
+        if (DIAG) probes++;
+        const bool diag_ce = DIAG && LIN && ra.stamps && dda.coarse_empty_at_lin(t_march, coarse);
         const uint32_t emitted_before = emitted;
-        if (LIN ? dda.probe_lin(t_march, x, y, z, dt, coarse, run_cells ? &occ_until : nullptr) : dda.probe(t_march, x, y, z, dt, coarse)) {
+        if (LIN ? dda.probe_lin(t_march, x, y, z, dt, coarse, &occ_until) : dda.probe(t_march, x, y, z, dt, coarse)) {
             do {
                 out[(size_t)emitted * 64] = make_float2(t_march, dt);
                 t_march += dt;
@@ -217,9 +218,9 @@
                 }
             } while (run_cells && t_march < occ_until && t_march < far && emitted < n_step);
         }
-        if (ra.stamps && emitted == emitted_before) { if (diag_ce) probes_coarse_empty++; else probes_fine_empty++; }
-    }
-    if (ra.stamps) {
+        if (DIAG && ra.stamps && emitted == emitted_before) { if (diag_ce) probes_coarse_empty++; else probes_fine_empty++; }
+    }
+    if (DIAG && ra.stamps) {
         uint32_t mx = probes, sm = probes;
 #pragma unroll
         for (int off = 32; off > 0; off >>= 1) {
@@ -737,13 +738,14 @@
                                                       float* __restrict__ image, Ctl* __restrict__ ctl, uint32_t max_steps,
                                                       uint32_t* __restrict__ sample_hash, unsigned long long* __restrict__ stat_shards,
                                                       QueueHeads* __restrict__ heads, uint32_t* __restrict__ death_shards, uint32_t spec_allowed,
-                                                      uint32_t tile_w) {
+                                                      uint32_t tile_w, uint32_t* __restrict__ dump_iter) {
     const uint32_t n = blockIdx.x * 256 + threadIdx.x;
     if (n < (uint32_t)kStatShards) stat_shards[n] = 0ull;
     if (n < 2u * kDeathWords) death_shards[n] = 0;
     if (n < 16) heads[n >> 3].head[n & 7][0] = 0;
     if (n < N) {
         if (sample_hash) sample_hash[n] = 2166136261u;
+        if (dump_iter) dump_iter[n] = 0xFFFFFFFFu;
         uint32_t first = n;
         if (tile_w) {
             const uint32_t t = n >> 4, in = n & 15u, per_row = tile_w >> 2;
@@ -826,6 +828,18 @@
     float* rays_t = nullptr;
     unsigned long long* coarse = nullptr;
     uint32_t* grid_lin = nullptr;
+    struct OccKey {
+        const uint8_t* bitfield = nullptr;
+        unsigned long long generation = 0;
+        uint32_t cascade = 0, grid_size = 0;
+        hipStream_t stream = nullptr;
+        uint32_t layout = 0;
+        bool operator==(const OccKey& o) const {
+            return bitfield == o.bitfield && generation == o.generation && cascade == o.cascade && grid_size == o.grid_size &&
+                   stream == o.stream && layout == o.layout;
+        }
+    } occ_key;
+    unsigned long long occ_builds = 0;
     uint32_t* death_shards = nullptr;
     float4* backup = nullptr;
     float2* march_samples = nullptr;
@@ -912,6 +926,12 @@
     return NGP_OK;
 }
 
+int ngp_render_ctx_occupancy_builds(const ngp_render_ctx* ctx, unsigned long long* builds) {
+    NGP_REQUIRE(ctx && builds, "render_ctx_occupancy_builds: null pointer");
+    *builds = ctx->occ_builds;
+    return NGP_OK;
+}
+
 int ngp_render_ctx_destroy(ngp_render_ctx* c) {
     if (!c) return NGP_OK;
     (void)hipDeviceSynchronize();
@@ -935,12 +955,21 @@
     bool lin = !dbg.coarse_off() && !dbg.lin_off() && occupancy_lin_fits(C, H, model->density_bitfield, kLinMaxBytes, kCoarseMaxBytes);
     const bool use_coarse = !dbg.coarse_off() && cells % 4096 == 0 && cells / 64 / 8 <= kCoarseMaxBytes && ((uintptr_t)model->density_bitfield & 7) == 0;
     if (lin && !ctx->grid_lin && !ctx_alloc(ctx, &ctx->grid_lin, kLinMaxBytes)) lin = false;
+    ngp_render_ctx::OccKey key;
+    key.bitfield = model->density_bitfield; key.generation = bitfield_generation(model->density_bitfield);
+    key.cascade = C; key.grid_size = H; key.stream = s; key.layout = lin ? 1u : (use_coarse ? 2u : 0u);
+    const bool build = key.layout != 0 && !(key == ctx->occ_key);
+    if (build) {
+        ctx->occ_key = key;
+        ctx->occ_builds++;
+    }
     if (lin) {
-        ra.occ = build_occupancy_lin(model->density_bitfield, C, H, ctx->grid_lin, ctx->coarse, s);
+        if (build) build_occupancy_lin(model->density_bitfield, C, H, ctx->grid_lin, ctx->coarse, s);
+        ra.occ = occupancy_lin_view(C, H, ctx->grid_lin, ctx->coarse);
         ra.block_jump = dbg.jump_off() ? 0u : 1u;
     } else if (use_coarse) {
         const uint32_t n_words = (uint32_t)(cells / 64);
-        k_build_coarse<<<div_up(n_words, 256), 256, 0, s>>>((const unsigned long long*)model->density_bitfield, n_words, ctx->coarse);
+        if (build) k_build_coarse<<<div_up(n_words, 256), 256, 0, s>>>((const unsigned long long*)model->density_bitfield, n_words, ctx->coarse);
         ra.occ.coarse = (const uint32_t*)ctx->coarse;
         ra.occ.coarse_words = n_words / 32;
     } else {
@@ -969,6 +998,7 @@
 }
 
 typedef void (*IterKernel)(NetArgs, GridLevels, RenderArgs);
+typedef void (*MarchKernel)(RenderArgs, float);
 static IterKernel choose_iter_kernel(const NetArgs& na, const GridLevels& lv) {
     static const IterKernel kIter[2][3] = {{k_render_iter<0, false>, k_render_iter<1, false>, k_render_iter<2, false>},
                                            {k_render_iter<0, true>, k_render_iter<1, true>, k_render_iter<2, true>}};
@@ -992,8 +1022,10 @@
         ProfScope pm("k_march_ahead", s, 0);
         const uint32_t by_wave = div_up(ub < ra.wave_march_max ? ub : ra.wave_march_max, 4);
         const uint32_t by_lane = div_up(ub ? ub : 1, 256);
-        if (lin) k_march_ahead<true><<<by_lane > by_wave ? by_lane : by_wave, 256, 0, s>>>(ra, na.bound);
-        else k_march_ahead<false><<<div_up(ub ? ub : 1, 256), 256, 0, s>>>(ra, na.bound);
+        const uint32_t march_blocks = lin ? (by_lane > by_wave ? by_lane : by_wave) : by_lane;
+        const MarchKernel march = ra.stamps ? (lin ? k_march_ahead<true, true> : k_march_ahead<false, true>)
+                                            : (lin ? k_march_ahead<true, false> : k_march_ahead<false, false>);
+        march<<<march_blocks, 256, 0, s>>>(ra, na.bound);
     }
     {
         ProfScope pk("k_render_iter", s, 0);
@@ -1117,10 +1149,6 @@
     const uint32_t spec_allowed = (!dbg.spec_off() && perturb == 0) ? (1u | (last_sigmas ? 2u : 0u) | (dbg.prefix_replay_off() ? 4u : 0u)) : 0u;
     const uint32_t fw = ctx->frame_width;
     const uint32_t tile_w = (perturb == 0 && !dbg.tile_off() && fw >= 4 && fw % 4 == 0 && N % (4 * fw) == 0) ? fw : 0u;
-    const uint32_t init_threads = N > 2u * kDeathWords ? N : 2u * kDeathWords;
-    k_render_init<<<div_up(init_threads, 256), 256, 0, s>>>(N, nears, ctx->rays_t, ctx->alive[0], weights_sum, depth, image, ctx->ctl, max_steps,
-                                                 dbg.sample_hash, ctx->stat_shards, ctx->heads, ctx->death_shards, spec_allowed, tile_w);
-
     RenderArgs ra = {};
     ra.rays_o = rays_o; ra.rays_d = rays_d; ra.fars = fars;
     ra.weights_sum = weights_sum; ra.depth = depth; ra.image = image;
@@ -1136,10 +1164,13 @@
                 return NGP_ENODEVICE;
             }
         }
-        (void)hipMemsetAsync(ctx->dump_iter, 0xff, (size_t)N * 4, s);
         ra.dump_rec = ctx->dump_rec;
         ra.dump_iter = ctx->dump_iter;
     }
+    const uint32_t init_threads = N > 2u * kDeathWords ? N : 2u * kDeathWords;
+    k_render_init<<<div_up(init_threads, 256), 256, 0, s>>>(N, nears, ctx->rays_t, ctx->alive[0], weights_sum, depth, image, ctx->ctl, max_steps,
+                                                 dbg.sample_hash, ctx->stat_shards, ctx->heads, ctx->death_shards, spec_allowed, tile_w,
+                                                 ra.dump_iter);
     const size_t lds = weights_bytes(na) + sizeof(LevelTab) + (size_t)kWaves * sizeof(WaveSlab);
     const IterKernel iter_kernel = choose_iter_kernel(na, lv);
     ensure_dynamic_lds(reinterpret_cast<const void*>(iter_kernel), 160 * 1024);
diff --git a/nerfsafetyvalidation_amd/raymarching/raymarching.py b/nerfsafetyvalidation_amd/raymarching/raymarching.py
--- a/nerfsafetyvalidation_amd/raymarching/raymarching.py
+++ b/nerfsafetyvalidation_amd/raymarching/raymarching.py
@@ -237,18 +237,20 @@
         return None
     stream = _lib.stream()
     key = (id(density_bitfield), int(stream or 0), C, H)
+    generation = _lib.bitfield_generation(density_bitfield)
     with _OCC_LIN_LOCK:
         hit = _OCC_LIN.get(key)
         if hit is not None:
-            ref, version, ptr, buf = hit
-            if ref() is density_bitfield and version == density_bitfield._version and ptr == density_bitfield.data_ptr():
+            ref, version, ptr, gen, buf = hit
+            if (ref() is density_bitfield and version == density_bitfield._version and ptr == density_bitfield.data_ptr()
+                    and gen == generation):
                 _OCC_LIN.move_to_end(key)
                 return buf
             del _OCC_LIN[key]
     buf = torch.empty(nbytes, dtype=torch.uint8, device=density_bitfield.device)
     _lib.check(L.ngp_build_occupancy_lin(_lib.ptr(density_bitfield), C, H, _lib.ptr(buf), nbytes, stream), "build_occupancy_lin")
     with _OCC_LIN_LOCK:
-        _OCC_LIN[key] = (weakref.ref(density_bitfield), density_bitfield._version, density_bitfield.data_ptr(), buf)
+        _OCC_LIN[key] = (weakref.ref(density_bitfield), density_bitfield._version, density_bitfield.data_ptr(), generation, buf)
         while len(_OCC_LIN) > _OCC_LIN_MAX:
             _OCC_LIN.popitem(last=False)
     return buf
```

New measurement: 7.791 billion samples/s, median of 6. 2.4% higher.
